# lukashermann/hulc

Hardware: AMD Instinct MI355X
Metric: trajectory-windows/sec (seq_len=32, bs=64/GPU) (higher is better)
Workload: dtype bf16; 1 GPU; HULC training step, vision goal only (use_clip_auxiliary_loss=false), B=64 windows/GPU, seq_len=32, 200x200 static + 84x84 gripper fp32 NCHW frames, fwd+loss+bwd+Adam, dropout 0.1; global_batch=64, seq_len=32, parallelism=dp1

## Files before the change

### hulc_amd/csrc/capi.hip

```cpp
#include <cstdarg>
#include <cstdio>
#include <cstring>
#include <cstdlib>
#include <cmath>
#include <algorithm>
#include <stdexcept>

#include "engine.h"
#include "sbert.h"
#include "store_gather.h"
#include "store_stage.h"

using namespace hulc_bf16;

static thread_local char g_err[1024] = "";
void hulc_set_error(const char* fmt, ...) {
    va_list ap;
    va_start(ap, fmt);
    vsnprintf(g_err, sizeof(g_err), fmt, ap);
    va_end(ap);
}

struct hulc_ctx {
    IEngine* e = nullptr;
// ... 241 lines not shown
    int r = -1, w = -1;
    if (ctx->e->comm->size(&r, &w)) return 1;
    if (rank) *rank = r;
    if (world) *world = w;
    return 0;
}
int hulc_comm_timeline(hulc_ctx* ctx, double* out, int32_t cap_buckets, double* backward_us) {
    if (!ctx || !ctx->e->comm || !out) { hulc_set_error("hulc_comm_timeline: no communicator / null buffer"); return -1; }
    return ctx->e->comm->timeline(out, cap_buckets, backward_us, ctx->e->st);
}
int hulc_allreduce_grads(hulc_ctx* ctx, int32_t bucket_dtype) {
    if (!ctx) { hulc_set_error("hulc_allreduce_grads: null context"); return 1; }
    return ctx->e->allreduce_grads(bucket_dtype);
}
int hulc_backward_allreduce(hulc_ctx* ctx, int32_t bucket_dtype) {
    if (!ctx) { hulc_set_error("hulc_backward_allreduce: null context"); return 1; }
    return ctx->e->backward_allreduce(bucket_dtype);
}
int hulc_scaler_enable(hulc_ctx* ctx, float init_scale, float growth_factor, float backoff_factor, int32_t growth_interval) {
    if (!ctx) { hulc_set_error("hulc_scaler_enable: null context"); return 1; }
    return ctx->e->scaler_enable(init_scale, growth_factor, backoff_factor, growth_interval);
}
int hulc_scaler_get(hulc_ctx* ctx, float* scale, int32_t* growth_tracker, int64_t* skipped_steps, int32_t* last_found_inf, int64_t* taken_steps) {
    if (!ctx) { hulc_set_error("hulc_scaler_get: null context"); return 1; }
    return ctx->e->scaler_get(scale, growth_tracker, skipped_steps, last_found_inf, taken_steps);
}
int hulc_scaler_set(hulc_ctx* ctx, float scale, int32_t growth_tracker, int64_t taken_steps) {
    if (!ctx) { hulc_set_error("hulc_scaler_set: null context"); return 1; }
    return ctx->e->scaler_set(scale, growth_tracker, taken_steps);
}
int hulc_grad_clip_set(hulc_ctx* ctx, int32_t algo, float limit, int32_t track) {
    if (!ctx) { hulc_set_error("hulc_grad_clip_set: null context"); return 1; }
    return ctx->e->grad_clip_set(algo, limit, track);
}
int hulc_grad_norm_get(hulc_ctx* ctx, float* total, float* coef, float* per_tensor_host, int64_t cap) {
    if (!ctx) { hulc_set_error("hulc_grad_norm_get: null context"); return 1; }
    return ctx->e->grad_norm_get(total, coef, per_tensor_host, cap);
}
int hulc_set_kl_beta(hulc_ctx* ctx, float b) { ctx->e->set_kl_beta(b); return 0; }
int hulc_set_dropout(hulc_ctx* ctx, float p) {
    if (!(p >= 0.f && p < 1.f)) { hulc_set_error("hulc_set_dropout: p must be in [0,1)"); return 1; }
    ctx->e->set_dropout(p);
    return 0;
}
int hulc_set_option(hulc_ctx* ctx, const char* name, int64_t value) {
    if (!ctx) { hulc_set_error("hulc_set_option: null context"); return 1; }
    return ctx->e->set_option(name, (long long)value);
}
int hulc_get_option(hulc_ctx* ctx, const char* name, int64_t* value) {
    if (!ctx || !value) { hulc_set_error("hulc_get_option: null argument"); return 1; }
    if (name && !strcmp(name, "stage_tickets")) { *value = HULC_STAGE_TICKETS; return 0; }
    long long v = 0;
    const int rc = ctx->e->get_option(name, &v);
    *value = (int64_t)v;
    return rc;
}
int hulc_timers_enable(hulc_ctx* ctx, int32_t on, const char* only_class) { ctx->e->set_timing(on != 0, only_class); return 0; }
int hulc_timers_read(hulc_ctx* ctx, char* json_out, int64_t cap, int32_t reset) { return ctx->e->timers_read(json_out, cap, reset != 0); }
int hulc_get_tensor(hulc_ctx* ctx, const char* name, float* out, int64_t cap, int64_t* n) { return ctx->e->get_tensor(name, out, cap, n); }
int hulc_get_plan_idx(hulc_ctx* ctx, int32_t* out, int64_t cap) { return ctx->e->get_plan_idx(out, cap); }

int hulc_k_gemm_nt(int32_t dtype, const void* A, const void* B, float* C, int32_t M, int32_t N, int32_t K, int64_t lda, int64_t ldb, int64_t ldc,
                   const float* bias, int32_t relu, void* stream) {
    if (dtype == HULC_DTYPE_F16) return hulc_f16::k_gemm_nt(0, A, B, C, M, N, K, lda, ldb, ldc, bias, relu, stream);
    return hulc_bf16::k_gemm_nt(dtype == HULC_DTYPE_F32, A, B, C, M, N, K, lda, ldb, ldc, bias, relu, stream);
}
#define HULC_K_16BIT(name, call)                                                                                          \
    if (dtype == HULC_DTYPE_F16) return hulc_f16::call;                                                                    \
    if (dtype == HULC_DTYPE_BF16) return hulc_bf16::call;                                                                  \
    hulc_set_error(name ": dtype %d is not a 16-bit type", (int)dtype);                                                    \
    return 1
int hulc_k_spatial_softmax64(int32_t dtype, const void* f, int32_t H, int32_t W, int32_t Nf, void* out, float* stats, const float* dout, void* df, void* stream) {
    HULC_K_16BIT("hulc_k_spatial_softmax64", k_spatial_softmax64(f, H, W, Nf, out, stats, dout, df, stream));
}
int hulc_k_enc_tail_fwd(int32_t dtype, int32_t Nf, int32_t ldemb, const hulc_enc_tail_job* a, const hulc_enc_tail_job* b, void* emb, const float* pos, int32_t S,
                        float drop_p, uint64_t seed, float* xf, void* xt, float* z0, float* z1, void* stream) {
    HULC_K_16BIT("hulc_k_enc_tail_fwd", k_enc_tail_fwd(Nf, ldemb, a, b, emb, pos, S, drop_p, (unsigned long long)seed, xf, xt, z0, z1, stream));
}
int hulc_k_enc_tail_bwd(int32_t dtype, int32_t Nf, int32_t ldemb, const hulc_enc_tail_bwd_job* a, const hulc_enc_tail_bwd_job* b, const float* demb, void* stream) {
    HULC_K_16BIT("hulc_k_enc_tail_bwd", k_enc_tail_bwd(Nf, ldemb, a, b, demb, stream));
}
int hulc_k_tr_layer_fwd(int32_t dtype, const hulc_tr_layer_job* job, int32_t B, int32_t S, int32_t ln_in, float dp, void* stream) {
    HULC_K_16BIT("hulc_k_tr_layer_fwd", k_tr_layer_fwd(job, B, S, ln_in, dp, stream));
}
int hulc_k_tr_ffn_bwd(int32_t dtype, const hulc_tr_ffn_bwd_job* job, int32_t B, int32_t S, int32_t bcast, float bdiv, float dp, void* stream) {
    HULC_K_16BIT("hulc_k_tr_ffn_bwd", k_tr_ffn_bwd(job, B, S, bcast, bdiv, dp, stream));
}
int hulc_k_tr_attn_bwd(int32_t dtype, const hulc_tr_attn_bwd_job* job, int32_t B, int32_t S, int32_t nparts, int64_t part_stride, float dp, void* stream) {
    HULC_K_16BIT("hulc_k_tr_attn_bwd", k_tr_attn_bwd(job, B, S, nparts, (long long)part_stride, dp, stream));
}
int hulc_k_gemm_multi(int32_t dtype, int32_t form, const hulc_gemm_epi_job* jobs, int32_t n, int32_t sh, int32_t* ran, void* stream) {
    HULC_K_16BIT("hulc_k_gemm_multi", k_gemm_multi(form, jobs, n, sh, ran, stream));
}
#undef HULC_K_16BIT
int hulc_k_gemm_epi(int32_t dtype, const hulc_gemm_epi_job* job, int32_t kernel, int32_t* ran, void* stream) {
    if (dtype == HULC_DTYPE_F16) return hulc_f16::k_gemm_epi(1, job, kernel, ran, stream);
    if (dtype != HULC_DTYPE_F32 && dtype != HULC_DTYPE_BF16) { hulc_set_error("hulc_k_gemm_epi: unknown dtype %d", (int)dtype); return 1; }
    return hulc_bf16::k_gemm_epi(dtype == HULC_DTYPE_BF16 ? 1 : 0, job, kernel, ran, stream);
}
int hulc_k_gemm_pick(int32_t dtype, int32_t M, int32_t N, int32_t K, int64_t lda, int64_t ldb, int32_t* pick, int32_t* bk) {
    if (dtype != HULC_DTYPE_F32 && dtype != HULC_DTYPE_BF16 && dtype != HULC_DTYPE_F16) { hulc_set_error("hulc_k_gemm_pick: unknown dtype %d", (int)dtype); return 1; }
    return hulc_bf16::k_gemm_pick(dtype != HULC_DTYPE_F32, M, N, K, (long long)lda, (long long)ldb, pick, bk);
}
int hulc_k_gemm_wgrad_nsplit(int32_t dtype, int32_t M, int32_t N, int32_t K, int32_t* nsplit, int32_t* big) {
    if (dtype != HULC_DTYPE_F32 && dtype != HULC_DTYPE_BF16 && dtype != HULC_DTYPE_F16) { hulc_set_error("hulc_k_gemm_wgrad_nsplit: unknown dtype %d", (int)dtype); return 1; }
    return hulc_bf16::k_gemm_wgrad_nsplit(dtype != HULC_DTYPE_F32, M, N, K, nsplit, big);
}
int hulc_k_logistic_loss(int32_t dtype, int32_t wide, const float* heads, int32_t ldh, const float* actions, const float* robot_obs, int32_t B, int32_t S,
                         int32_t n_mix, int32_t n_dim, int32_t num_classes, float log_scale_min, float gripper_alpha, int32_t gripper_control,
                         int32_t discrete_gripper, float grad_scale, const float* lscale, float* row_loss, float* a_tcp_out, void* dheads, void* stream) {
    if (dtype == HULC_DTYPE_F16)
        return hulc_f16::k_logistic_loss(1, wide, heads, ldh, actions, robot_obs, B, S, n_mix, n_dim, num_classes, log_scale_min, gripper_alpha, gripper_control,
                                         discrete_gripper, grad_scale, lscale, row_loss, a_tcp_out, dheads, stream);
    if (dtype != HULC_DTYPE_F32 && dtype != HULC_DTYPE_BF16) { hulc_set_error("hulc_k_logistic_loss: unknown dtype %d", (int)dtype); return 1; }
    return hulc_bf16::k_logistic_loss(dtype == HULC_DTYPE_BF16, wide, heads, ldh, actions, robot_obs, B, S, n_mix, n_dim, num_classes, log_scale_min, gripper_alpha,
                                      gripper_control, discrete_gripper, grad_scale, lscale, row_loss, a_tcp_out, dheads, stream);
}
#define HULC_K_ANY(name, fn, ...)                                                                                                     \
    if (dtype == HULC_DTYPE_F16) return hulc_f16::fn(1, __VA_ARGS__);                                                                  \
    if (dtype != HULC_DTYPE_F32 && dtype != HULC_DTYPE_BF16) { hulc_set_error(name ": unknown dtype %d", (int)dtype); return 1; }      \
    return hulc_bf16::fn(dtype == HULC_DTYPE_BF16 ? 1 : 0, __VA_ARGS__)
int hulc_k_plan_kl_sample(const float* pr_logits, const float* pp_logits, int32_t B, int32_t NCAT, int32_t NCLS, const int32_t* idx_in, int32_t* idx_out, float* probs,
                          float* kl_cat, float* dpp, float* dpr, float w_pp, float w_pr, uint64_t seed, const float* lscale, void* stream) {
    return hulc_bf16::k_plan_kl_sample(pr_logits, pp_logits, B, NCAT, NCLS, idx_in, idx_out, probs, kl_cat, dpp, dpr, w_pp, w_pr, (unsigned long long)seed, lscale, stream);
}
int hulc_k_st_softmax_bwd(int32_t dtype, const float* probs, const float* dplan, const float* dpr_kl, const float* dpp_kl, int32_t rows, int32_t NCLS, float* out, void* out_t,
                          void* dpp_t, void* stream) {
    HULC_K_ANY("hulc_k_st_softmax_bwd", k_st_softmax_bwd, probs, dplan, dpr_kl, dpp_kl, rows, NCLS, out, out_t, dpp_t, stream);
}
int hulc_k_plan_gather(int32_t dtype, const void* w_t, const int32_t* idx, int32_t B, int32_t NCAT, int32_t NCLS, int32_t H, const float* b1, const float* b2, float* out,
                       const void* emb, void* embg, int32_t S, int32_t W, const void* goal, int32_t G, int32_t grow0, void* cb, void* stream) {
    HULC_K_ANY("hulc_k_plan_gather", k_plan_gather, w_t, idx, B, NCAT, NCLS, H, b1, b2, out, emb, embg, S, W, goal, G, grow0, cb, stream);
}
int hulc_k_plan_scatter_grad(int32_t dtype, int32_t form, const void* dC, const int32_t* idx, int32_t B, int32_t NCAT, int32_t NCLS, int32_t H, int32_t KIN, float* dw,
                             int32_t store, void* stream) {
    HULC_K_ANY("hulc_k_plan_scatter_grad", k_plan_scatter_grad, form, dC, idx, B, NCAT, NCLS, H, KIN, dw, store, stream);
}
int hulc_k_normal_kl_sample(int32_t dtype, const float* pr_state, const float* pp_state, int32_t B, int32_t n, const float* eps_in, float* eps_out, float* plan_f, void* plan_t,
                            float* kl_elem, float* dpp, float* dpr, float w_pp, float w_pr, uint64_t seed, const float* lscale, void* stream) {
    HULC_K_ANY("hulc_k_normal_kl_sample", k_normal_kl_sample, pr_state, pp_state, B, n, eps_in, eps_out, plan_f, plan_t, kl_elem, dpp, dpr, w_pp, w_pr, (unsigned long long)seed, lscale, stream);
}
int hulc_k_normal_rsample_bwd(int32_t dtype, const float* dplan, const float* eps, const float* pr_state, const float* dpr_kl, int32_t B, int32_t n, void* out, void* stream) {
    HULC_K_ANY("hulc_k_normal_rsample_bwd", k_normal_rsample_bwd, dplan, eps, pr_state, dpr_kl, B, n, out, stream);
}
int hulc_k_det_head_loss(int32_t dtype, const void* H1, const void* W, const float* bias, const float* actions, const float* robot_obs, int32_t B, int32_t S,
                         int32_t criterion, int32_t frame, float grad_scale, const float* lscale, float* row_loss, float* pred, float* dpre, void* stream) {
    HULC_K_ANY("hulc_k_det_head_loss", k_det_head_loss, H1, W, bias, actions, robot_obs, B, S, criterion, frame, grad_scale, lscale, row_loss, pred, dpre, stream);
}
int hulc_k_det_head_bwd(int32_t dtype, const float* dpre, const void* W, const void* H1, int32_t B, int32_t S, void* dH1, void* dZ1, float* dW, float* db, void* stream) {
    HULC_K_ANY("hulc_k_det_head_bwd", k_det_head_bwd, dpre, W, H1, B, S, dH1, dZ1, dW, db, stream);
}
int hulc_k_det_head_act(int32_t dtype, const void* h1, const void* W, const float* bias, const float* robot_obs, int32_t n, float* out, void* stream) {
    HULC_K_ANY("hulc_k_det_head_act", k_det_head_act, h1, W, bias, robot_obs, n, out, stream);
}
int hulc_k_layernorm_fwd(int32_t dtype, const float* x, int64_t ldx, int32_t rows, int32_t n, const float* g, const float* b, void* out, int64_t ldo, float* out_f32, int64_t ldf,
                         float* stats, void* stream) {
    HULC_K_ANY("hulc_k_layernorm_fwd", k_layernorm_fwd, x, (long long)ldx, rows, n, g, b, out, (long long)ldo, out_f32, (long long)ldf, stats, stream);
}
int hulc_k_layernorm_bwd(int32_t dtype, const float* dy, int64_t lddy, const float* x, int64_t ldx, const float* stats, const float* g, int32_t rows, int32_t n, float* dx_f32,
                         int64_t ldd, int32_t accumulate, void* dx_t, int64_t ldt, float* dg, float* db, float drop_p, uint64_t seed, int32_t bcast_rows, float bcast_div,
                         int32_t dy_parts, int64_t dy_part_stride, float* scratch, void* stream) {
    HULC_K_ANY("hulc_k_layernorm_bwd", k_layernorm_bwd, dy, (long long)lddy, x, (long long)ldx, stats, g, rows, n, dx_f32, (long long)ldd, accumulate, dx_t, (long long)ldt, dg, db,
               drop_p, (unsigned long long)seed, bcast_rows, bcast_div, dy_parts, (long long)dy_part_stride, scratch, stream);
}
int hulc_k_layernorm_mean(int32_t dtype, const float* x, int32_t B, int32_t S, int32_t n, const float* g, const float* b, float* stats, void* out, float* yout, void* stream) {
    HULC_K_ANY("hulc_k_layernorm_mean", k_layernorm_mean, x, B, S, n, g, b, stats, out, yout, stream);
}
#undef HULC_K_ANY
int hulc_k_cast(int32_t dtype, const float* src, void* dst, int64_t n, void* stream) {
    hipStream_t st = (hipStream_t)stream;
    if (dtype == HULC_DTYPE_F32) hipLaunchKernelGGL((cast_kernel<float, float>), dim3(1024), dim3(256), 0, st, src, (float*)dst, (long long)n);
    else hipLaunchKernelGGL((cast_kernel<float, h16_t>), dim3(1024), dim3(256), 0, st, src, (h16_t*)dst, (long long)n);
    if (hipGetLastError() != hipSuccess) { hulc_set_error("hulc_k_cast: launch failed"); return 1; }
    return 0;
}
int hulc_k_window_compact(const int64_t* window_start, const int32_t* lens, const int32_t* off, int32_t off_base, int32_t B, int32_t S, int64_t store_frames,
                          const int32_t* shift_static, const int32_t* shift_gripper, int64_t* frame_out, int32_t* shift_static_out, int32_t* shift_gripper_out, void* stream) {
    if (!window_start || !lens || !off || !frame_out || B < 1 || S < 1 || store_frames < 1 || (shift_static && !shift_static_out) || (shift_gripper && !shift_gripper_out)) {
        hulc_set_error("hulc_k_window_compact: null argument or B=%d, S=%d, store_frames=%lld out of range", (int)B, (int)S, (long long)store_frames); return 1; }
    launch_window_compact((hipStream_t)stream, reinterpret_cast<const long long*>(window_start), lens, off, off_base, B, S, (long long)store_frames, shift_static, shift_gripper,
                          reinterpret_cast<long long*>(frame_out), shift_static_out, shift_gripper_out);
    if (hipGetLastError() != hipSuccess) { hulc_set_error("hulc_k_window_compact: launch failed"); return 1; }
    return 0;
}
int hulc_k_rows_expand(int32_t elem_bytes, const void* src, const int32_t* lens, const int32_t* off, int32_t B, int32_t S, int32_t n, void* dst, void* stream) {
    if (!src || !lens || !off || !dst || B < 1 || S < 1 || n < 1 || (elem_bytes != 2 && elem_bytes != 4) || (n * elem_bytes) % 16 || ((uintptr_t)src | (uintptr_t)dst) % 16) {
        hulc_set_error("hulc_k_rows_expand: null or misaligned argument, or B=%d, S=%d, n=%d, elem_bytes=%d unsupported", (int)B, (int)S, (int)n, (int)elem_bytes); return 1; }
    if (elem_bytes == 4) launch_rows_expand<float>((hipStream_t)stream, (const float*)src, lens, off, B, S, n, (float*)dst);
    else launch_rows_expand<h16_t>((hipStream_t)stream, (const h16_t*)src, lens, off, B, S, n, (h16_t*)dst);
    if (hipGetLastError() != hipSuccess) { hulc_set_error("hulc_k_rows_expand: launch failed"); return 1; }
    return 0;
}
int hulc_k_rows_reduce(const float* src, const int32_t* lens, const int32_t* off, int32_t B, int32_t S, int32_t n, float* dst, void* stream) {
    if (!src || !lens || !off || !dst || B < 1 || S < 1 || n < 4 || n % 4 || ((uintptr_t)src | (uintptr_t)dst) % 16) {
        hulc_set_error("hulc_k_rows_reduce: null or misaligned argument, or B=%d, S=%d, n=%d unsupported", (int)B, (int)S, (int)n); return 1; }
    launch_rows_reduce((hipStream_t)stream, src, lens, off, B, S, n, dst);
    if (hipGetLastError() != hipSuccess) { hulc_set_error("hulc_k_rows_reduce: launch failed"); return 1; }
    return 0;
}

static int k_clip_loss(bool wide, const float* img, const float* txt, int32_t n, const float* logit_scale, float w, float* loss_out, float* dimg, float* dtxt,
                       float* dlogit_scale, void* stream) {
    hipStream_t st = (hipStream_t)stream;
    if (n < 1 || !img || !txt || !logit_scale || !loss_out || !dimg || !dtxt || !dlogit_scale) { hulc_set_error("hulc_k_clip_loss: n=%d or a null argument", (int)n); return 1; }
    float* ws = nullptr;
    if (n > AUX_ROWS_SINGLE && hipMalloc((void**)&ws, sizeof(float) * (size_t)clip_rows_ws_floats(n)) != hipSuccess) { hulc_set_error("hulc_k_clip_loss: hipMalloc failed"); return 1; }
    const bool ok = launch_clip_loss(st, wide, img, txt, n, logit_scale, w, loss_out, dimg, dtxt, dlogit_scale, nullptr, ws);
    const hipError_t e1 = hipGetLastError(), e2 = hipStreamSynchronize(st);
    if (ws) hipFree(ws);
    if (!ok || e1 != hipSuccess || e2 != hipSuccess) { hulc_set_error("hulc_k_clip_loss: %s", !ok ? "not launched" : hipGetErrorString(e1 != hipSuccess ? e1 : e2)); return 1; }
    return 0;
}
int hulc_k_clip_loss(const float* img, const float* txt, int32_t n, const float* logit_scale, float w, float* loss_out, float* dimg, float* dtxt, float* dlogit_scale,
                     void* stream) { return k_clip_loss(true, img, txt, n, logit_scale, w, loss_out, dimg, dtxt, dlogit_scale, stream); }
int hulc_k_clip_loss_fp32(const float* img, const float* txt, int32_t n, const float* logit_scale, float w, float* loss_out, float* dimg, float* dtxt,
                          float* dlogit_scale, void* stream) { return k_clip_loss(false, img, txt, n, logit_scale, w, loss_out, dimg, dtxt, dlogit_scale, stream); }
int hulc_k_mia_head(const float* img, const float* txt, int32_t n, const float* W0, const float* b0, const float* W1, const float* b1, float w, float* loss_out,
                    float* dimg, float* dtxt, int32_t accum, float* dW0, float* db0, float* dW1, float* db1, void* stream) {
    hipStream_t st = (hipStream_t)stream;
    if (n < 1 || !img || !txt || !W0 || !b0 || !W1 || !b1 || !loss_out) { hulc_set_error("hulc_k_mia_head: n=%d or a null argument", (int)n); return 1; }
    if (dW0 && (!dimg || !dtxt || !db0 || !dW1 || !db1)) { hulc_set_error("hulc_k_mia_head: the backward needs every gradient pointer"); return 1; }
    float* ws = nullptr;
    if (n > AUX_ROWS_SINGLE && hipMalloc((void**)&ws, sizeof(float) * (size_t)mia_rows_ws_floats(n)) != hipSuccess) { hulc_set_error("hulc_k_mia_head: hipMalloc failed"); return 1; }
    const bool ok = launch_mia_head(st, img, txt, n, W0, b0, W1, b1, w, loss_out, dimg, dtxt, accum, dW0, db0, dW1, db1, nullptr, ws);
    const hipError_t e1 = hipGetLastError(), e2 = hipStreamSynchronize(st);
    if (ws) hipFree(ws);
    if (!ok || e1 != hipSuccess || e2 != hipSuccess) { hulc_set_error("hulc_k_mia_head: %s", !ok ? "not launched" : hipGetErrorString(e1 != hipSuccess ? e1 : e2)); return 1; }
    return 0;
}
int hulc_k_cosine_dist(const float* pred, const float* tgt, int32_t n, int32_t D, float w, float* loss_out, float* dpred, void* stream) {
    hipStream_t st = (hipStream_t)stream;
    if (n < 1 || D < 1 || !pred || !tgt || !loss_out) { hulc_set_error("hulc_k_cosine_dist: n=%d D=%d or a null argument", (int)n, (int)D); return 1; }
    hipLaunchKernelGGL(cosine_dist_loss_kernel, dim3(1), dim3(1024), 0, st, pred, tgt, n, D, w, loss_out, dpred, (const float*)nullptr);
    const hipError_t e1 = hipGetLastError(), e2 = hipStreamSynchronize(st);
    if (e1 != hipSuccess || e2 != hipSuccess) { hulc_set_error("hulc_k_cosine_dist: %s", hipGetErrorString(e1 != hipSuccess ? e1 : e2)); return 1; }
    return 0;
}

int hulc_k_attention(int32_t variant, const float* qkv, float* P, float* ao, const float* dao, float* dqkv, int32_t B, int32_t S, float drop_p,
                     uint64_t seed, void* stream) {
    hipStream_t st = (hipStream_t)stream;
    const int D = 128, NH = 8;
    if (S < 1 || S > 64 || (variant == 1 && S > 32)) { hulc_set_error("hulc_k_attention: S=%d not covered by variant %d", S, variant); return 1; }
    if (variant == 2) {
        if (!dao) hipLaunchKernelGGL((attention_fwd64_kernel<float>), dim3(B * NH), dim3(256), 0, st, qkv, B, S, D, NH, P, ao, drop_p, (unsigned long long)seed);
        else {
            hipFuncSetAttribute((const void*)attention_bwd64_kernel<float>, hipFuncAttributeMaxDynamicSharedMemorySize, (int)ATT_BWD64_LDS);
            hipLaunchKernelGGL((attention_bwd64_kernel<float>), dim3(B * NH), dim3(256), ATT_BWD64_LDS, st, qkv, P, dao, B, S, D, NH, dqkv, drop_p, (unsigned long long)seed);
        }
        if (hipGetLastError() != hipSuccess) { hulc_set_error("hulc_k_attention: launch failed"); return 1; }
        return 0;
    }
    const dim3 grid(B * NH), block(64);
    if (!dao) {
        if (variant == 1) hipLaunchKernelGGL((attention_fwd32_kernel<float>), grid, block, 0, st, qkv, B, S, D, NH, P, ao, drop_p, (unsigned long long)seed);
        else if (S <= 32) hipLaunchKernelGGL((attention_fwd_kernel<float, 32>), grid, block, 0, st, qkv, B, S, D, NH, P, ao, drop_p, (unsigned long long)seed);
        else hipLaunchKernelGGL((attention_fwd_kernel<float, 64>), grid, block, 0, st, qkv, B, S, D, NH, P, ao, drop_p, (unsigned long long)seed);
    } else {
        if (variant == 1) hipLaunchKernelGGL((attention_bwd32_kernel<float>), grid, block, 0, st, qkv, P, dao, B, S, D, NH, dqkv, drop_p, (unsigned long long)seed);
        else if (S <= 32) hipLaunchKernelGGL((attention_bwd_kernel<float, 32>), grid, block, 0, st, qkv, P, dao, B, S, D, NH, dqkv, drop_p, (unsigned long long)seed);
        else hipLaunchKernelGGL((attention_bwd_kernel<float, 64>), grid, block, 0, st, qkv, P, dao, B, S, D, NH, dqkv, drop_p, (unsigned long long)seed);
    }
    if (hipGetLastError() != hipSuccess) { hulc_set_error("hulc_k_attention: launch failed"); return 1; }
    return 0;
}

#define HULC_K_CONV_T(name, call)                                                                                          \
    if (dtype == HULC_DTYPE_F16) return hulc_f16::call;                                                                    \
    if (dtype == HULC_DTYPE_BF16) return hulc_bf16::call;                                                                  \
    hulc_set_error(name ": dtype %d is not a 16-bit type (HULC_DTYPE_BF16 or HULC_DTYPE_F16)", (int)dtype);                \
    return 1
int hulc_k_conv_wgrad(int32_t which, const void* X, const void* dY, float* out, int32_t Nf, int32_t IH, void* stream) {
    return hulc_bf16::k_conv_wgrad("hulc_k_conv_wgrad", 0, which, X, dY, out, nullptr, Nf, IH, nullptr, stream);
}
int hulc_k_conv_wgrad_t(int32_t dtype, int32_t which, const void* X, const void* dY, float* out, float* db_out, int32_t Nf, int32_t IH, int32_t* slabs, void* stream) {
    HULC_K_CONV_T("hulc_k_conv_wgrad_t", k_conv_wgrad("hulc_k_conv_wgrad_t", 1, which, X, dY, out, db_out, Nf, IH, slabs, stream));
}

int hulc_k_conv1_interior_groups(int32_t IW, int32_t pad, int32_t cap, int32_t* first, int32_t* count) {
    int cl = 0, wi = 0;
    conv1_interior_groups(IW, pad, cap, cl, wi);
    *first = cl; *count = wi;
    return 0;
}

int hulc_k_conv1_wgrad_u8(const void* X, const int32_t* shifts, int32_t pad, const void* dY, float* dw_out, float* db_out, int32_t Nf, int32_t IH, int32_t form, int32_t fold, void* stream) {
    return hulc_bf16::k_conv1_wgrad_u8("hulc_k_conv1_wgrad_u8", 0, X, shifts, pad, dY, dw_out, db_out, Nf, IH, form, fold, nullptr, stream);
}
int hulc_k_conv1_wgrad_u8_t(int32_t dtype, const void* X, const int32_t* shifts, int32_t pad, const void* dY, float* dw_out, float* db_out, int32_t Nf, int32_t IH, int32_t form,
                            int32_t fold, int32_t* slabs, void* stream) {
    HULC_K_CONV_T("hulc_k_conv1_wgrad_u8_t", k_conv1_wgrad_u8("hulc_k_conv1_wgrad_u8_t", 1, X, shifts, pad, dY, dw_out, db_out, Nf, IH, form, fold, slabs, stream));
}

int hulc_k_conv_tile(int32_t mode, const void* img, const void* w, const float* bias, const void* mask, void* out, int32_t Nf, int32_t IMH,
                     int32_t OUTH, int32_t relu, void* stream) {
    return hulc_bf16::k_conv_tile("hulc_k_conv_tile", 0, mode, img, w, bias, mask, out, nullptr, Nf, IMH, OUTH, relu, 0, stream);
}
int hulc_k_conv_tile_t(int32_t dtype, int32_t mode, const void* img, const void* w, const float* bias, const void* mask, void* out, uint32_t* bits1_out, int32_t Nf, int32_t IMH,
                       int32_t OUTH, int32_t relu, int32_t wgs, void* stream) {
    HULC_K_CONV_T("hulc_k_conv_tile_t", k_conv_tile("hulc_k_conv_tile_t", 1, mode, img, w, bias, mask, out, bits1_out, Nf, IMH, OUTH, relu, wgs, stream));
}
int hulc_k_conv_plan(int32_t form, int32_t frames, int32_t in_side, int32_t out_side, int32_t wgs, int32_t* nbands, int32_t* rows_per_band, int32_t* frames_per_band, int32_t* items) {
    return hulc_bf16::k_conv_plan(form, frames, in_side, out_side, wgs, nbands, rows_per_band, frames_per_band, items);
}

int hulc_k_camera_split(int32_t grid, double work_static, double work_gripper, int32_t* wg_static, int32_t* wg_gripper) {
    int a = 0, b = 0;
    camera_split(grid, work_static, work_gripper, a, b);
    *wg_static = a; *wg_gripper = b;
    return 0;
}

int hulc_k_conv_pair(int32_t stage, const hulc_conv_job* a, const hulc_conv_job* b, int32_t wg_a, int32_t wg_b, void* stream) {
    return hulc_bf16::k_conv_pair("hulc_k_conv_pair", 0, stage, a, b, wg_a, wg_b, nullptr, stream);
}
int hulc_k_conv_pair_t(int32_t dtype, int32_t stage, const hulc_conv_job* a, const hulc_conv_job* b, int32_t wg_a, int32_t wg_b, int32_t* slabs, void* stream) {
    HULC_K_CONV_T("hulc_k_conv_pair_t", k_conv_pair("hulc_k_conv_pair_t", 1, stage, a, b, wg_a, wg_b, slabs, stream));
}
#undef HULC_K_CONV_T

int hulc_k_skinny(const void* A, const void* W, void* out, int32_t M, int32_t N, int32_t K, int32_t variant, void* stream) {
    hipStream_t st = (hipStream_t)stream;
    EpiP ep; ep.out = out; ep.out_f32 = 0;
    const int NW = variant / 10, MT = variant % 10;
    dim3 grid(N / 16, MT > 0 ? (M + MT * 16 - 1) / (MT * 16) : 1);
    const h16_t* a = (const h16_t*)A; const h16_t* w = (const h16_t*)W;
#define SK(nw, mt) hipLaunchKernelGGL((skinny_gemm_kernel<nw, mt>), grid, dim3(nw * 64), 0, st, a, (long long)K, w, (long long)K, M, N, K, dense_out(N), ep)
    if (NW == 8 && MT == 2) SK(8, 2); else if (NW == 8 && MT == 4) SK(8, 4); else if (NW == 4 && MT == 2) SK(4, 2); else if (NW == 4 && MT == 4) SK(4, 4);
    else if (NW == 8 && MT == 1) SK(8, 1); else if (NW == 4 && MT == 1) SK(4, 1);
    else if (NW == 16 && MT == 2) SK(16, 2); else if (NW == 16 && MT == 4) SK(16, 4);
    else if (NW == 9 && MT == 2) hipLaunchKernelGGL((skinny_gemm_kernel<8, 2, 8>), grid, dim3(512), 0, st, a, (long long)K, w, (long long)K, M, N, K, dense_out(N), ep);
    else if (NW == 17 && MT == 2) hipLaunchKernelGGL((skinny_gemm_kernel<16, 2, 4>), grid, dim3(1024), 0, st, a, (long long)K, w, (long long)K, M, N, K, dense_out(N), ep);
    else if (NW == 20) { if (!launch_skinny_lds(st, a, (long long)K, w, (long long)K, M, N, K, MT, dense_out(N), ep)) { hulc_set_error("hulc_k_skinny: shape not covered by the LDS kernel"); return 1; } }
    else if (NW == 30) launch_skinny(st, a, (long long)K, w, (long long)K, M, N, K, dense_out(N), ep);
    else if (NW == 40) {
        EpiP ep2 = ep; ep2.out = (h16_t*)out + (long long)M * N;
        if (!launch_skinny_lds_dual(st, a, w, ep, a + (long long)M * K, w + (long long)N * K, ep2, (long long)K, (long long)K, M, N, K, dense_out(N))) {
            hulc_set_error("hulc_k_skinny: shape not covered by the dual launch"); return 1; }
    }
    else if (NW == 50 || NW == 51) {
        if ((N % 16) != 0 || (K % 128) != 0) { hulc_set_error("hulc_k_skinny: fragment order needs N %% 16 == 0 and K %% 128 == 0"); return 1; }
        h16_t* wf = (h16_t*)out;
        if (NW == 50 && hipMalloc((void**)&wf, (size_t)N * K * sizeof(h16_t)) != hipSuccess) { hulc_set_error("hulc_k_skinny: scratch allocation failed"); return 1; }
        FragPackBatch fb{};
        fb.src[0] = w; fb.dst[0] = wf; fb.N[0] = N; fb.K[0] = K; fb.blk0[0] = 0; fb.blk0[1] = frag_pack_blocks(N, K); fb.n = 1;
        hipLaunchKernelGGL(frag_pack_kernel, dim3(fb.blk0[1]), dim3(256), 0, st, fb);
        if (NW == 50) {
            const bool ok = launch_skinny_lds_kchunk(st, a, (long long)K, wf, 0ll, M, N, K, dense_out(N), ep);
            hipStreamSynchronize(st);
            hipFree(wf);
            if (!ok) { hulc_set_error("hulc_k_skinny: shape not covered by the K-chunked kernel"); return 1; }
        }
    }
    else { hulc_set_error("hulc_k_skinny: unsupported variant"); return 1; }
#undef SK
    return hipGetLastError() == hipSuccess ? 0 : 1;
}

int hulc_k_rnn_persist(void* X, const void* W, const void* res, const void* mask, int32_t B, int32_t S, int32_t q0, int32_t dq, int32_t act, uint32_t* flags,
                       uint32_t* err, uint32_t launch_index, void* stream) {
    RnnPersistP p{};
    p.X = (h16_t*)X; p.W = (const h16_t*)W; p.res = (const h16_t*)res; p.mask = (const h16_t*)mask; p.B = B; p.S = S; p.q0 = q0; p.dq = dq; p.act = act;
    p.flags = flags; p.base = launch_index << 12; p.parity = (int)(launch_index & 1u); p.err = err; p.stamps = nullptr;
    if (!launch_rnn_persist((hipStream_t)stream, p)) { hulc_set_error("hulc_k_rnn_persist: shape not covered (S >= 2, B <= 128)"); return 1; }
    return hipGetLastError() == hipSuccess ? 0 : 1;
}
int32_t hulc_k_rnn_persist_flag_words(void) { return RP_FLAG_WORDS; }

__global__ void trread_probe_kernel(const int* __restrict__ addr_in, unsigned short* __restrict__ out) {
    typedef short s16x4 __attribute__((ext_vector_type(4)));
    __shared__ __attribute__((aligned(16))) unsigned short lds[8192];
    for (int i = threadIdx.x; i < 8192; i += 64) lds[i] = (unsigned short)i;
    __syncthreads();
    const int a = addr_in[threadIdx.x];
    s16x4 v = __builtin_amdgcn_ds_read_tr16_b64_v4i16((__attribute__((address_space(3))) s16x4*)(lds + a));
#pragma unroll
    for (int j = 0; j < 4; ++j) out[threadIdx.x * 4 + j] = (unsigned short)v[j];
}
int hulc_k_trread_probe(const int32_t* addr, uint16_t* out, void* stream) {
    hipLaunchKernelGGL(trread_probe_kernel, dim3(1), dim3(64), 0, (hipStream_t)stream, (const int*)addr, (unsigned short*)out);
    if (hipGetLastError() != hipSuccess) { hulc_set_error("trread probe launch failed"); return 1; }
    return 0;
}

}
```

### hulc_amd/csrc/conv_wgrad.h

```cpp
#pragma once
#include "common.h"

namespace HULC_NS {

typedef short s16x4_t __attribute__((ext_vector_type(4)));
typedef unsigned int u32x4_t __attribute__((ext_vector_type(4)));
typedef __attribute__((address_space(3))) u32x4_t lds_u32x4;

typedef __attribute__((address_space(3))) char lds_char;
DEVI h16x8_t tr_read8(lds_char* p0, lds_char* p1) {
    const s16x4_t lo = __builtin_amdgcn_ds_read_tr16_b64_v4i16((__attribute__((address_space(3))) s16x4_t*)p0);
    const s16x4_t hi = __builtin_amdgcn_ds_read_tr16_b64_v4i16((__attribute__((address_space(3))) s16x4_t*)p1);
    typedef short s16x8_t __attribute__((ext_vector_type(8)));
    const s16x8_t v = __builtin_shufflevector(lo, hi, 0, 1, 2, 3, 4, 5, 6, 7);
    return __builtin_bit_cast(h16x8_t, v);
}

template <int CI, int CO, int KH, int KW, int S>
struct WgradCfg {
    static constexpr int XS = (S == 1) ? ((CI * 2 / 32) | 1) * 32 : CI * 2 + 16;
    static constexpr int DYS = ((CO * 2 / 32) | 1) * 32;
    static constexpr int CGN = CI / 16;
    static constexpr int NT = KH * KW * CGN;
    static constexpr int NTW = NT / 4;
    static constexpr int CT = CO / 16;
    static_assert(NT % 4 == 0, "n-tiles must split over 4 waves");
    static size_t lds_bytes(int R, int IW, int OW) {
        const int OWp = (OW + 7) / 8 * 8;
        const int XR = (R - 1) * S + KH;
        return (size_t)(XR * IW + 8 * S + KW) * XS + (size_t)(R * OWp + 8) * DYS;
    }
};

template <int CI, int CO, int KH, int KW, int S>
__global__ void __launch_bounds__(256, 2) conv_wgrad_tr_kernel(const h16_t* __restrict__ X, const h16_t* __restrict__ dY, float* __restrict__ part,
                                                            float* __restrict__ bias_part, int Nf, int IH, int IW, int OH, int OW, int R) {
    using C = WgradCfg<CI, CO, KH, KW, S>;
    extern __shared__ __attribute__((aligned(16))) char smem[];
    const int tid = threadIdx.x, lane = tid & 63, wave = tid >> 6;
    const int OWp = (OW + 7) & ~7, U = OWp >> 3;
    const int XR = (R - 1) * S + KH;
    const int xpix = XR * IW + 8 * S + KW;
    const int dypix = R * OWp + 8;
    lds_char* ximg = (lds_char*)smem;
    lds_char* dyimg = ximg + xpix * C::XS;
    for (int i = tid * 16; i < xpix * C::XS + dypix * C::DYS; i += 256 * 16) *(lds_u32x4*)((lds_char*)smem + i) = u32x4_t{0u, 0u, 0u, 0u};
    __syncthreads();

    f32x4 acc[C::NTW][C::CT];
#pragma unroll
    for (int j = 0; j < C::NTW; ++j)
#pragma unroll
        for (int c = 0; c < C::CT; ++c) acc[j][c] = f32x4{0.f, 0.f, 0.f, 0.f};

    const int g = lane >> 4, a = lane & 15;
    const int prow = a >> 2;
    const int ccol = (a & 3) * 8;
    const int nt0 = wave * C::NTW;
    float bsum[8] = {0.f, 0.f, 0.f, 0.f, 0.f, 0.f, 0.f, 0.f};

    for (int f = blockIdx.x; f < Nf; f += gridDim.x) {
        for (int oh0 = 0; oh0 < OH; oh0 += R) {
            __syncthreads();
            {
                constexpr int CH = CO / 8;
                for (int r = wave; r < R; r += 4) {
                    const bool in = oh0 + r < OH;
                    const h16_t* src = dY + ((long long)f * OH + min(oh0 + r, OH - 1)) * OW * CO;
                    for (int i = lane; i < OW * CH; i += 64) {
                        u32x4_t v = *reinterpret_cast<const u32x4_t*>(src + i * 8);
                        if (!in) v = u32x4_t{0u, 0u, 0u, 0u};
#pragma unroll
                        for (int e = 0; e < 4; ++e) { bsum[2 * e] += h2f_lo(v[e]); bsum[2 * e + 1] += h2f_hi(v[e]); }
                        *(lds_u32x4*)(dyimg + (r * OWp + i / CH) * C::DYS + (i % CH) * 16) = v;
                    }
                }
            }
            {
                constexpr int CH = CI / 8;
                const int ih0 = oh0 * S;
                const int rows = min(XR, IH - ih0);
                const int total = rows * IW * CH;
                const h16_t* src = X + ((long long)f * IH + ih0) * IW * CI;
                for (int i0 = tid; i0 < total; i0 += 256 * 8) {
                    u32x4_t v[8];
#pragma unroll
                    for (int u = 0; u < 8; ++u) {
                        const int i = min(i0 + u * 256, total - 1);
                        v[u] = *reinterpret_cast<const u32x4_t*>(src + (long long)(i / CH) * CI + (i % CH) * 8);
                    }
#pragma unroll
                    for (int u = 0; u < 8; ++u) {
                        const int i = i0 + u * 256;
                        if (i < total) *(lds_u32x4*)(ximg + (i / CH) * C::XS + (i % CH) * 16) = v[u];
                    }
                }
            }
            __syncthreads();
            const int units = R * U;
            for (int u0 = 0; u0 < units; u0 += 4) {
                const int u = u0 + g;
                const bool valid = u < units;
                const int r = valid ? u / U : 0, ow0 = valid ? (u % U) * 8 : 0;
                const int pixA = valid ? r * OWp + ow0 : R * OWp;
                lds_char* abase = dyimg + (pixA + prow) * C::DYS + ccol;
                h16x8_t af[C::CT];
#pragma unroll
                for (int c = 0; c < C::CT; ++c) af[c] = tr_read8(abase + c * 32, abase + 4 * C::DYS + c * 32);
                const int pixB0 = (r * S) * IW + ow0 * S;
#pragma unroll
                for (int j = 0; j < C::NTW; ++j) {
                    const int nt = nt0 + j;
                    const int tap = nt / C::CGN, cg = nt % C::CGN;
                    const int kh = tap / KW, kw = tap % KW;
                    lds_char* bbase = ximg + (pixB0 + kh * IW + kw + prow * S) * C::XS + cg * 32 + ccol;
                    const h16x8_t bf = tr_read8(bbase, bbase + 4 * S * C::XS);
#pragma unroll
                    for (int c = 0; c < C::CT; ++c) acc[j][c] = MFMA_16x16x32_H(af[c], bf, acc[j][c], 0, 0, 0);
                }
            }
        }
    }
    constexpr int KC = KH * KW * CI;
    float* out = part + (long long)blockIdx.x * CO * KC;
#pragma unroll
    for (int j = 0; j < C::NTW; ++j)
#pragma unroll
        for (int c = 0; c < C::CT; ++c)
#pragma unroll
            for (int r = 0; r < 4; ++r) out[(long long)(c * 16 + g * 4 + r) * KC + (nt0 + j) * 16 + a] = acc[j][c][r];
    __syncthreads();
    float* red = reinterpret_cast<float*>(smem);
#pragma unroll
    for (int e = 0; e < 8; ++e) red[tid * 8 + e] = bsum[e];
    __syncthreads();
    if (tid < CO) {
        constexpr int CH = CO / 8;
        const int cgrp = tid >> 3, e = tid & 7;
        float s = 0.f;
        for (int t = cgrp; t < 256; t += CH) s += red[t * 8 + e];
        if (bias_part) unsafeAtomicAdd(bias_part + tid, s);
    }
}

static inline void camera_split(int grid, double wA, double wB, int& nA, int& nB) {
    if (grid < 1) grid = 1;
    if (!(wB > 0.0)) { nA = grid; nB = 0; return; }
    if (!(wA > 0.0)) { nA = 0; nB = grid; return; }
    if (grid < 2) { nA = nB = 1; return; }
    int b = (int)(grid * (wB / (wA + wB)) + 0.5);
    b = std::min(std::max(b, 1), grid - 1);
    nA = grid - b; nB = b;
}

struct WgradJob {
    const h16_t* X; const h16_t* dY; float* part; float* bias_part; const h16_t* zeros;
    int Nf, IH, IW, OH, OW, R, nbands; int* work_ctr; int FPB;
};
template <int CI, int CO, int KH, int KW, int S, int NWV, int D = 3, int IWC = 0>
DEVI void conv_wgrad_tr8_body(const WgradJob& J, const int bid, const int nwg) {
    const h16_t* __restrict__ const X = J.X; const h16_t* __restrict__ const dY = J.dY; float* __restrict__ const part = J.part; float* __restrict__ const bias_part = J.bias_part;
    const int Nf = J.Nf, IH = J.IH, IW = J.IW, OH = J.OH, OW = J.OW, R = J.R, nbands = J.nbands, FPB = J.FPB;
    int* __restrict__ const work_ctr = J.work_ctr;
    using C = WgradCfg<CI, CO, KH, KW, S>;
    constexpr int NTH = NWV * 64, PF = 8192 / NTH, CTH = C::CT / (NWV / 4), CHY = CO / 8, CHX = CI / 8;
    extern __shared__ __attribute__((aligned(16))) char smem[];
    const int tid = threadIdx.x, lane = tid & 63, wave = tid >> 6;
    const int OWp = (OW + 7) & ~7, U = OWp >> 3;
    const int XR = (R - 1) * S + KH;
    const int xpix = XR * IW + 8 * S + KW;
    const int dypix = R * OWp + 8;
    lds_char* ximg = (lds_char*)smem;
    lds_char* dyimg = ximg + xpix * C::XS;
    for (int i = tid * 16; i < xpix * C::XS + dypix * C::DYS; i += NTH * 16) *(lds_u32x4*)((lds_char*)smem + i) = u32x4_t{0u, 0u, 0u, 0u};

    const bool stacked = FPB > 1;
    const int VP = IH / S;
    const int ndy = (stacked ? FPB * OH : R) * OW * CHY, nx = XR * IW * CHX, nch = ndy + nx;
    unsigned pk[PF];
#pragma unroll
    for (int k = 0; k < PF; ++k) {
        const int ci = min(tid + k * NTH, nch - 1);
        if (ci < ndy) {
            const int pix = ci / CHY, c = ci % CHY;
            int r = pix / OW;
            const int ow = pix % OW;
            if (stacked) r = (r / OH) * VP + r % OH;
            pk[k] = ((unsigned)((xpix * C::XS + (r * OWp + ow) * C::DYS + c * 16) >> 4) << 17) | (unsigned)ci;
        } else {
            const int cx = ci - ndy;
            const int pix = cx / CHX, c = cx % CHX;
            pk[k] = 0x80000000u | ((unsigned)((pix * C::XS + c * 16) >> 4) << 17) | (unsigned)cx;
        }
    }
    const int q = wave & 3, h = wave >> 2;
    f32x4 acc[C::NTW][CTH];
#pragma unroll
    for (int j = 0; j < C::NTW; ++j)
#pragma unroll
        for (int c = 0; c < CTH; ++c) acc[j][c] = f32x4{0.f, 0.f, 0.f, 0.f};
    const int g = lane >> 4, a = lane & 15;
    const int prow = a >> 2;
    const int ccol = (a & 3) * 8;
    constexpr int NTG = 4 / C::CGN, TPG = KH * KW / NTG;
    static_assert(C::CGN <= 4 && 4 % C::CGN == 0 && (KH * KW) % NTG == 0 && TPG == C::NTW && (NTG == 1 || TPG % KW == 0), "n-tile assignment");
    const int IWk = IWC ? IWC : IW;
    const int cgq = q % C::CGN, tg = q / C::CGN;
    const int qoff = ((tg * TPG / KW) * IWk) * C::XS + cgq * 32;
    int toff[C::NTW];
#pragma unroll
    for (int j = 0; j < C::NTW; ++j) toff[j] = ((j / KW) * IWk + j % KW) * C::XS;
    float bsum[8] = {0.f, 0.f, 0.f, 0.f, 0.f, 0.f, 0.f, 0.f};

    u32x4_t pf[PF];
    const int nitems = stacked ? (Nf + FPB - 1) / FPB : Nf * nbands;
    unsigned zmask = 0, zmask_cur = 0;
    auto prefetch = [&](int item) {
        zmask = 0;
        const int f = stacked ? item * FPB : item / nbands, oh0 = stacked ? 0 : (item % nbands) * R;
        const int nfr = stacked ? min(FPB, Nf - f) : 1;
        const h16_t* ybase = dY + ((long long)f * OH + oh0) * OW * CO;
        const h16_t* xbase = X + ((long long)f * IH + oh0 * S) * IW * CI;
        const int yrows = stacked ? nfr * OH : min(R, OH - oh0), xrows = stacked ? min(XR, nfr * IH) : min(XR, IH - oh0 * S);
        const int ylim = yrows * OW * CHY - 1, xlim = xrows * IW * CHX - 1;
#pragma unroll
        for (int k = 0; k < PF; ++k) {
            const bool isx = (pk[k] >> 31) != 0;
            const int go = (int)(pk[k] & 0x1ffffu);
            const h16_t* src = isx ? xbase + (long long)min(go, xlim) * 8 : ybase + (long long)min(go, ylim) * 8;
            pf[k] = *reinterpret_cast<const u32x4_t*>(src);
            if (!isx && go > ylim) zmask |= 1u << k;
        }
    };
    __shared__ int s_next[2];
    int item = bid, iter = 0;
    if (item < nitems) prefetch(item);
    while (item < nitems) {
        if (work_ctr && tid == 0) s_next[iter & 1] = nwg + atomicAdd(work_ctr, 1);
        __syncthreads();
        zmask_cur = zmask;
#pragma unroll
        for (int k = 0; k < PF; ++k) {
            if (tid + k * NTH < nch) {
                const u32x4_t v = ((zmask_cur >> k) & 1u) ? u32x4_t{0u, 0u, 0u, 0u} : pf[k];
                if (!(pk[k] >> 31)) {
#pragma unroll
                    for (int e = 0; e < 4; ++e) { bsum[2 * e] += h2f_lo(v[e]); bsum[2 * e + 1] += h2f_hi(v[e]); }
                }
                *(lds_u32x4*)((lds_char*)smem + (((pk[k] >> 17) & 0x3fffu) << 4)) = v;
            }
        }
        __syncthreads();
        item = work_ctr ? s_next[iter & 1] : item + nwg;
        ++iter;
        if (item < nitems) prefetch(item);
        const int units = R * U;
        const int px = (g & 1) * 4 + prow;
        const int q4 = 4 / U, r4 = 4 - q4 * U;
        const int step4 = (q4 * S * IW + r4 * 8 * S) * C::XS, wrapd = (S * IW - U * 8 * S) * C::XS;
        int uo[2], pbv[2];
#pragma unroll
        for (int hh = 0; hh < 2; ++hh) {
            const int u = hh * 2 + (g >> 1), r = u / U;
            uo[hh] = u - r * U;
            pbv[hh] = ((r * S) * IW + (uo[hh] * 8 + px) * S) * C::XS + ccol;
        }
        const int abase = px * C::DYS + ccol + h * CTH * 32, pb_idle = (px * S) * C::XS + ccol;
#pragma unroll 1
        for (int u0 = 0; u0 < units; u0 += 4) {
            lds_char* ab[2];
            int pb[2];
#pragma unroll
            for (int hh = 0; hh < 2; ++hh) {
                const int u = u0 + hh * 2 + (g >> 1);
                const bool valid = u < units;
                ab[hh] = dyimg + (valid ? u * 8 : R * OWp) * C::DYS + abase;
                pb[hh] = valid ? pbv[hh] : pb_idle;
                pbv[hh] += step4; uo[hh] += r4;
                if (uo[hh] >= U) { uo[hh] -= U; pbv[hh] += wrapd; }
            }
            auto bfrag = [&](int j) { return tr_read8(ximg + qoff + pb[0] + toff[j], ximg + qoff + pb[1] + toff[j]); };
            h16x8_t ring[D];
            h16x8_t af[CTH];
#pragma unroll
            for (int c = 0; c < CTH; ++c) af[c] = tr_read8(ab[0] + c * 32, ab[1] + c * 32);
#pragma unroll
            for (int j = 0; j < D && j < C::NTW; ++j) ring[j] = bfrag(j);
            __builtin_amdgcn_sched_barrier(0);
#pragma unroll
            for (int j = 0; j < C::NTW; ++j) {
                const h16x8_t bf = ring[j % D];
#pragma unroll
                for (int c = 0; c < CTH; ++c) acc[j][c] = MFMA_16x16x32_H(af[c], bf, acc[j][c], 0, 0, 0);
                if (j + D < C::NTW) ring[j % D] = bfrag(j + D);
                __builtin_amdgcn_sched_barrier(0);
            }
        }
    }
    constexpr int KC = KH * KW * CI;
    float* out = part + (long long)bid * CO * KC;
#pragma unroll
    for (int j = 0; j < C::NTW; ++j)
#pragma unroll
        for (int c = 0; c < CTH; ++c)
#pragma unroll
            for (int r = 0; r < 4; ++r) out[(long long)((h * CTH + c) * 16 + g * 4 + r) * KC + ((tg * TPG + j) * C::CGN + cgq) * 16 + a] = acc[j][c][r];
    __syncthreads();
    float* red = reinterpret_cast<float*>(smem);
#pragma unroll
    for (int e = 0; e < 8; ++e) red[tid * 8 + e] = bsum[e];
    __syncthreads();
    if (tid < CO) {
        const int cgrp = tid >> 3, e = tid & 7;
        float s = 0.f;
        for (int t = cgrp; t < NTH; t += CHY) s += red[t * 8 + e];
        if (bias_part) unsafeAtomicAdd(bias_part + tid, s);
    }
}
template <int CI, int CO, int KH, int KW, int S, int NWV, int D = 3, int IWC = 0>
__global__ void __launch_bounds__(NWV * 64) conv_wgrad_tr8_kernel(const h16_t* __restrict__ X, const h16_t* __restrict__ dY, float* __restrict__ part,
                                                            float* __restrict__ bias_part, int Nf, int IH, int IW, int OH, int OW, int R, int nbands,
                                                            int* __restrict__ work_ctr, int FPB) {
    const WgradJob J{X, dY, part, bias_part, nullptr, Nf, IH, IW, OH, OW, R, nbands, work_ctr, FPB};
    conv_wgrad_tr8_body<CI, CO, KH, KW, S, NWV, D, IWC>(J, (int)blockIdx.x, (int)gridDim.x);
}

DEVI int wg_fdiv(int x, float inv) { return (int)(((float)x + 0.5f) * inv); }
DEVI void wg_lds_dma16(const void* src, lds_char* dst) {
    const unsigned a = (unsigned)__builtin_amdgcn_readfirstlane((int)(unsigned)(size_t)dst);
    asm volatile("s_mov_b32 m0, %1\n\ts_nop 0\n\tglobal_load_lds_dwordx4 %0, off" : : "v"(src), "s"(a) : "memory", "m0");
}
template <int CI, int CO, int KH, int KW, int S, int IWC = 0>
DEVI void conv_wgrad_dma_body(const WgradJob& J, const int bid, const int nwg) {
    const h16_t* __restrict__ const X = J.X; const h16_t* __restrict__ const dY = J.dY; float* __restrict__ const part = J.part; float* __restrict__ const bias_part = J.bias_part;
    const h16_t* __restrict__ const zeros = J.zeros;
    const int Nf = J.Nf, IH = J.IH, IW = J.IW, OH = J.OH, OW = J.OW, R = J.R, nbands = J.nbands;
    int* __restrict__ const work_ctr = J.work_ctr;
    using C = WgradCfg<CI, CO, KH, KW, S>;
    constexpr int NWV = 8, NTH = NWV * 64, CTH = C::CT / (NWV / 4), CHY = CO / 8, CHX = CI / 8, XSS = C::XS / 16, YSS = C::DYS / 16;
    extern __shared__ __attribute__((aligned(16))) char smem[];
    const int tid = threadIdx.x, lane = tid & 63, wave = tid >> 6;
    const int OWp = (OW + 7) & ~7, U = OWp >> 3;
    const int XR = (R - 1) * S + KH;
    const int xpix = XR * IW + 8 * S + KW;
    const int dypix = R * OWp + 8;
    const int xslots = xpix * XSS, yslots = dypix * YSS;
    const int bbytes = ((xslots + yslots) * 16 + 1023) & ~1023;
    const int npieces = bbytes >> 10;
    lds_char* const lbase = (lds_char*)smem;
    const int nitems = Nf * nbands;
    const float invXSS = 1.f / (float)XSS, invYSS = 1.f / (float)YSS, invIW = 1.f / (float)IW, invOWp = 1.f / (float)OWp, invOW = 1.f / (float)OW;
    constexpr int PFM = 10;
    unsigned pk[PFM];
#pragma unroll
    for (int k = 0; k < PFM; ++k) {
        int q = (k * NWV + wave) * 64 + lane;
        unsigned v = 0;
        if (q < xslots) {
            const int px = wg_fdiv(q, invXSS), ch = q - px * XSS;
            const int r = wg_fdiv(px, invIW), c = px - r * IW;
            if (ch < CHX && r < XR) v = 0xC0000000u | ((unsigned)r << 24) | (unsigned)(((r * IW + c) * CI + ch * 8) >> 3);
        } else {
            q -= xslots;
            const int px = wg_fdiv(q, invYSS), ch = q - px * YSS;
            const int r = wg_fdiv(px, invOWp), c = px - r * OWp;
            if (ch < CHY && r < R && c < OW) v = 0x40000000u | ((unsigned)r << 24) | (unsigned)(((r * OW + c) * CO + ch * 8) >> 3);
        }
        pk[k] = v;
    }
    auto dma = [&](int item, int buf) {
        const int f = item / nbands, oh0 = (item - f * nbands) * R, ih0 = oh0 * S;
        const int yrows = min(R, OH - oh0), xrows = min(XR, IH - ih0);
        const h16_t* xsrc = X + ((long long)f * IH + ih0) * IW * CI;
        const h16_t* ysrc = dY + ((long long)f * OH + oh0) * OW * CO;
        lds_char* dst = lbase + buf * bbytes + wave * 1024;
#pragma unroll
        for (int k = 0; k < PFM; ++k) {
            if (k * NWV + wave >= npieces) break;
            const unsigned v = pk[k];
            const bool isx = (v >> 31) != 0;
            const int r = (int)((v >> 24) & 63u);
            const bool ok = ((v >> 30) & 1u) && r < (isx ? xrows : yrows);
            const h16_t* src = ok ? (isx ? xsrc : ysrc) + (long long)(v & 0xffffffu) * 8 : zeros;
            wg_lds_dma16(src, dst + k * NWV * 1024);
        }
    };
    const int q = wave & 3, h = wave >> 2;
    f32x4 acc[C::NTW][CTH];
#pragma unroll
    for (int j = 0; j < C::NTW; ++j)
#pragma unroll
        for (int c = 0; c < CTH; ++c) acc[j][c] = f32x4{0.f, 0.f, 0.f, 0.f};
    const int g = lane >> 4, a = lane & 15;
    const int prow = a >> 2;
    const int ccol = (a & 3) * 8;
    constexpr int NTG = 4 / C::CGN, TPG = KH * KW / NTG;
    static_assert(C::CGN <= 4 && 4 % C::CGN == 0 && (KH * KW) % NTG == 0 && TPG == C::NTW && (NTG == 1 || TPG % KW == 0), "n-tile assignment");
    const int IWk = IWC ? IWC : IW;
    const int cgq = q % C::CGN, tg = q / C::CGN;
    const int qoff = ((tg * TPG / KW) * IWk) * C::XS + cgq * 32;
    int toff[C::NTW];
#pragma unroll
    for (int j = 0; j < C::NTW; ++j) toff[j] = ((j / KW) * IWk + j % KW) * C::XS;
    float bsum[8] = {0.f, 0.f, 0.f, 0.f, 0.f, 0.f, 0.f, 0.f};
    __shared__ int s_next[2];
    int item = bid, iter = 0, nb = 0;
    if (item < nitems) dma(item, 0);
    asm volatile("s_waitcnt vmcnt(0)" ::: "memory");
    const int px = (g & 1) * 4 + prow;
    const int q4 = 4 / U, r4 = 4 - q4 * U;
    const int step4 = (q4 * S * IW + r4 * 8 * S) * C::XS, wrapd = (S * IW - U * 8 * S) * C::XS;
    while (item < nitems) {
        if (work_ctr && tid == 0) s_next[iter & 1] = nwg + atomicAdd(work_ctr, 1);
        __syncthreads();
        const int cur = item;
        item = work_ctr ? s_next[iter & 1] : item + nwg;
        ++iter;
        lds_char* const ximg0 = lbase + nb * bbytes;
        lds_char* const dyimg = ximg0 + xslots * 16;
        lds_char* const ximg = ximg0 + qoff;
        nb ^= 1;
        bool pend = item < nitems;
        if (pend && wave < 4) { dma(item, nb); pend = false; }
        {
            const int f = cur / nbands, oh0 = (cur - f * nbands) * R;
            const int nchunk = min(R, OH - oh0) * OW * CHY;
            for (int i = tid; i < nchunk; i += NTH) {
                const int pix = i / CHY, r = wg_fdiv(pix, invOW), c = pix - r * OW;
                const u32x4_t v = *(lds_u32x4*)(dyimg + (r * OWp + c) * C::DYS + (tid % CHY) * 16);
#pragma unroll
                for (int e = 0; e < 4; ++e) { bsum[2 * e] += h2f_lo(v[e]); bsum[2 * e + 1] += h2f_hi(v[e]); }
            }
        }
        const int units = R * U;
        int uo[2], pbv[2];
#pragma unroll
        for (int hh = 0; hh < 2; ++hh) {
            const int u = hh * 2 + (g >> 1), r = u / U;
            uo[hh] = u - r * U;
            pbv[hh] = ((r * S) * IW + (uo[hh] * 8 + px) * S) * C::XS + ccol;
        }
        const int abase = px * C::DYS + ccol + h * CTH * 32, pb_idle = (px * S) * C::XS + ccol;
        auto mstep = [&](const int u0) {
            lds_char* ab[2];
            int pb[2];
#pragma unroll
            for (int hh = 0; hh < 2; ++hh) {
                const int u = u0 + hh * 2 + (g >> 1);
                const bool valid = u < units;
                ab[hh] = dyimg + (valid ? u * 8 : R * OWp) * C::DYS + abase;
                pb[hh] = valid ? pbv[hh] : pb_idle;
                pbv[hh] += step4; uo[hh] += r4;
                if (uo[hh] >= U) { uo[hh] -= U; pbv[hh] += wrapd; }
            }
            auto bfrag = [&](int j) { return tr_read8(ximg + pb[0] + toff[j], ximg + pb[1] + toff[j]); };
            constexpr int D = 3;
            h16x8_t ring[D];
            h16x8_t af[CTH];
#pragma unroll
            for (int c = 0; c < CTH; ++c) af[c] = tr_read8(ab[0] + c * 32, ab[1] + c * 32);
#pragma unroll
            for (int j = 0; j < D && j < C::NTW; ++j) ring[j] = bfrag(j);
            __builtin_amdgcn_sched_barrier(0);
#pragma unroll
            for (int j = 0; j < C::NTW; ++j) {
                const h16x8_t bf = ring[j % D];
#pragma unroll
                for (int c = 0; c < CTH; ++c) acc[j][c] = MFMA_16x16x32_H(af[c], bf, acc[j][c], 0, 0, 0);
                if (j + D < C::NTW) ring[j % D] = bfrag(j + D);
                __builtin_amdgcn_sched_barrier(0);
            }
        };
        if (units > 0) mstep(0);
        if (pend) { dma(item, nb); pend = false; }
#pragma unroll 1
        for (int u0 = 4; u0 < units; u0 += 4) mstep(u0);
        if (pend) dma(item, nb);
        asm volatile("s_waitcnt vmcnt(0)" ::: "memory");
    }
    constexpr int KC = KH * KW * CI;
    float* out = part + (long long)bid * CO * KC;
#pragma unroll
    for (int j = 0; j < C::NTW; ++j)
#pragma unroll
        for (int c = 0; c < CTH; ++c)
#pragma unroll
            for (int r = 0; r < 4; ++r) out[(long long)((h * CTH + c) * 16 + g * 4 + r) * KC + ((tg * TPG + j) * C::CGN + cgq) * 16 + a] = acc[j][c][r];
    __syncthreads();
    float* red = reinterpret_cast<float*>(smem);
#pragma unroll
    for (int e = 0; e < 8; ++e) red[tid * 8 + e] = bsum[e];
    __syncthreads();
    if (tid < CO) {
        const int cgrp = tid >> 3, e = tid & 7;
        float s = 0.f;
        for (int t = cgrp; t < NTH; t += CHY) s += red[t * 8 + e];
        if (bias_part) unsafeAtomicAdd(bias_part + tid, s);
    }
}
template <int CI, int CO, int KH, int KW, int S, int IWC = 0>
__global__ void __launch_bounds__(512) conv_wgrad_dma_kernel(const h16_t* __restrict__ X, const h16_t* __restrict__ dY, float* __restrict__ part,
                                                             float* __restrict__ bias_part, const h16_t* __restrict__ zeros, int Nf, int IH, int IW, int OH, int OW,
                                                             int R, int nbands, int* __restrict__ work_ctr) {
    const WgradJob J{X, dY, part, bias_part, zeros, Nf, IH, IW, OH, OW, R, nbands, work_ctr, 1};
    conv_wgrad_dma_body<CI, CO, KH, KW, S, IWC>(J, (int)blockIdx.x, (int)gridDim.x);
}
template <int CI, int CO, int KH, int KW, int S, int IWS, int IWG>
__global__ void __launch_bounds__(512) conv_wgrad_pair_kernel(WgradJob A, WgradJob B, int wgA) {
    if ((int)blockIdx.x < wgA) conv_wgrad_dma_body<CI, CO, KH, KW, S, IWS>(A, (int)blockIdx.x, wgA);
    else conv_wgrad_tr8_body<CI, CO, KH, KW, S, 8, 3, IWG>(B, (int)blockIdx.x - wgA, (int)gridDim.x - wgA);
}
template <int CI, int CO, int KH, int KW, int S>
static inline int conv_wgrad_dma_rows(int IH, int IW, int OH, int OW, int* nbands_out, size_t* lds_out) {
    using C = WgradCfg<CI, CO, KH, KW, S>;
    const int OWp = (OW + 7) / 8 * 8, U = OWp / 8;
    int bestR = 0, bestc = 1 << 30;
    for (int R = OH; R >= 1; --R) {
        const int XR = (R - 1) * S + KH;
        const size_t band = (((size_t)(XR * IW + 8 * S + KW) * C::XS + (size_t)(R * OWp + 8) * C::DYS) + 1023) / 1024 * 1024;
        const size_t lds = std::max<size_t>(2 * band, 512 * 8 * sizeof(float));
        if (lds > 160 * 1024 - 128 || band > 80 * 1024 || R > 63) continue;
        const int nb = (OH + R - 1) / R, last = OH - (nb - 1) * R;
        const int cost = (nb - 1) * ((R * U + 3) / 4 + 1) + (last * U + 3) / 4 + 1;
        if (cost < bestc) { bestc = cost; bestR = R; *nbands_out = nb; *lds_out = lds; }
    }
    return bestR;
}

template <int CI, int KH> struct WgradCamW {
    static constexpr int fixed = (CI == 64 && KH == 3) ? 1 : ((CI == 32 && KH == 4) ? 2 : 0);
    static constexpr int stat = fixed == 1 ? 23 : (fixed == 2 ? 49 : 0), gripper = fixed == 1 ? 9 : (fixed == 2 ? 20 : 0);
};
template <int CI, int CO, int KH, int KW, int S>
static inline bool conv_wgrad_tr8_plan(int Nf, int IH, int IW, int OH, int OW, int wgs, int& R_out, int& nb_out, int& fpb_out, size_t& lds_out) {
    using C = WgradCfg<CI, CO, KH, KW, S>;
    constexpr int NWV = 8;
    for (int nb = 1; nb <= OH; ++nb) {
        int R = (OH + nb - 1) / nb, XR = (R - 1) * S + KH;
        long long chunks = (long long)R * OW * (CO / 8) + (long long)XR * IW * (CI / 8);
        size_t lds = std::max<size_t>(C::lds_bytes(R, IW, OW), NWV * 64 * 8 * sizeof(float));
        if (chunks > 16 * 512 || lds > 160 * 1024 - 64 || (long long)XR * IW * CI >= (1 << 20)) continue;
        int fpb = 1;
        if (nb == 1 && IH % S == 0) {
            for (int f = 2; f <= 16; ++f) {
                const int Rf = (f - 1) * (IH / S) + OH, XRf = (Rf - 1) * S + KH;
                const long long ch = (long long)f * OH * OW * (CO / 8) + (long long)XRf * IW * (CI / 8);
                const size_t l = std::max<size_t>(C::lds_bytes(Rf, IW, OW), NWV * 64 * 8 * sizeof(float));
                if (ch > 16 * 512 || l > 160 * 1024 - 64 || (long long)XRf * IW * CI >= (1 << 20)) break;
                if ((Nf + f - 1) / f < 2 * wgs) break;
                fpb = f; R = Rf; XR = XRf; chunks = ch; lds = l;
            }
        }
        R_out = R; nb_out = nb; fpb_out = fpb; lds_out = lds;
        return true;
    }
    return false;
}

template <int CI, int CO, int KH, int KW, int S>
static inline int launch_conv_wgrad_tr(hipStream_t st, const h16_t* X, const h16_t* dY, float* part, float* bias_part, int Nf, int IH, int IW, int OH,
                                       int OW, int max_blocks, int* work_ctr = nullptr, const h16_t* zeros = nullptr) {
    using C = WgradCfg<CI, CO, KH, KW, S>;
    if (zeros && OH * OW >= 256 && Nf >= 2) {
        int nb = 0; size_t lds = 0;
        const int R = conv_wgrad_dma_rows<CI, CO, KH, KW, S>(IH, IW, OH, OW, &nb, &lds);
        if (R > 0 && (long long)Nf * IH * IW * CI < (1ll << 31)) {
            constexpr int IWS = WgradCamW<CI, KH>::stat;
            static bool attr3 = false;
            if (!attr3) {
                hipFuncSetAttribute((const void*)conv_wgrad_dma_kernel<CI, CO, KH, KW, S, 0>, hipFuncAttributeMaxDynamicSharedMemorySize, 160 * 1024 - 64);
                hipFuncSetAttribute((const void*)conv_wgrad_dma_kernel<CI, CO, KH, KW, S, IWS>, hipFuncAttributeMaxDynamicSharedMemorySize, 160 * 1024 - 64);
                attr3 = true;
            }
            const int grid = std::min(std::min(Nf * nb, 256), max_blocks);
            if (IWS && IW == IWS) hipLaunchKernelGGL((conv_wgrad_dma_kernel<CI, CO, KH, KW, S, IWS>), dim3(grid), dim3(512), lds, st, X, dY, part, bias_part, zeros, Nf, IH, IW, OH, OW, R, nb, work_ctr);
            else hipLaunchKernelGGL((conv_wgrad_dma_kernel<CI, CO, KH, KW, S, 0>), dim3(grid), dim3(512), lds, st, X, dY, part, bias_part, zeros, Nf, IH, IW, OH, OW, R, nb, work_ctr);
            return grid;
        }
    }
    constexpr int NWV = 8;
    {
        int R = 0, nb = 0, fpb = 1; size_t lds = 0;
        if (conv_wgrad_tr8_plan<CI, CO, KH, KW, S>(Nf, IH, IW, OH, OW, std::min(256, max_blocks), R, nb, fpb, lds)) {
        static bool attr8 = false;
        if (!attr8) {
            hipFuncSetAttribute((const void*)conv_wgrad_tr8_kernel<CI, CO, KH, KW, S, NWV>, hipFuncAttributeMaxDynamicSharedMemorySize, 160 * 1024 - 64);
            attr8 = true;
        }
        const int items = fpb > 1 ? (Nf + fpb - 1) / fpb : Nf * nb;
        const int grid = std::min(std::min(items, 256), max_blocks);
        {
            constexpr int IWG = WgradCamW<CI, KH>::gripper;
            if (IWG && IW == IWG) {
                static bool ag = false;
                if (!ag) { hipFuncSetAttribute((const void*)conv_wgrad_tr8_kernel<CI, CO, KH, KW, S, NWV, 3, IWG>, hipFuncAttributeMaxDynamicSharedMemorySize, 160 * 1024 - 64); ag = true; }
                hipLaunchKernelGGL((conv_wgrad_tr8_kernel<CI, CO, KH, KW, S, NWV, 3, IWG>), dim3(grid), dim3(NWV * 64), lds, st, X, dY, part, bias_part, Nf, IH, IW, OH, OW, R, nb, work_ctr, fpb);
                return grid;
            }
        }
        hipLaunchKernelGGL((conv_wgrad_tr8_kernel<CI, CO, KH, KW, S, NWV>), dim3(grid), dim3(NWV * 64), lds, st, X, dY, part, bias_part, Nf, IH, IW, OH, OW, R, nb, work_ctr, fpb);
        return grid;
        }
    }
    int R = OH;
    while (R > 1 && C::lds_bytes(R, IW, OW) > 78 * 1024) --R;
    const int nbands = (OH + R - 1) / R;
    R = (OH + nbands - 1) / nbands;
    const size_t lds = C::lds_bytes(R, IW, OW);
    static bool attr_set = false;
    if (!attr_set) {
        hipFuncSetAttribute((const void*)conv_wgrad_tr_kernel<CI, CO, KH, KW, S>, hipFuncAttributeMaxDynamicSharedMemorySize, 160 * 1024);
        attr_set = true;
    }
    const int grid = Nf < max_blocks ? Nf : max_blocks;
    hipLaunchKernelGGL((conv_wgrad_tr_kernel<CI, CO, KH, KW, S>), dim3(grid), dim3(256), lds, st, X, dY, part, bias_part, Nf, IH, IW, OH, OW, R);
    return grid;
}

template <int CI, int CO, int KH, int KW, int S>
static inline bool launch_conv_wgrad_pair(hipStream_t st, WgradJob A, WgradJob B, int max_blocks, const int* wg, int ns[2]) {
    using W = WgradCamW<CI, KH>;
    if constexpr (W::fixed == 0) return false;
    else {
        constexpr int IWS = W::stat, IWG = W::gripper;
        if (A.IW != IWS || A.IH != IWS || B.IW != IWG || B.IH != IWG || !A.zeros || A.OH * A.OW < 256 || A.Nf < 1 || B.Nf < 1) return false;
        if ((long long)A.Nf * A.IH * A.IW * CI >= (1ll << 31)) return false;
        int nbA = 0; size_t ldsA = 0;
        A.R = conv_wgrad_dma_rows<CI, CO, KH, KW, S>(A.IH, A.IW, A.OH, A.OW, &nbA, &ldsA);
        if (A.R <= 0) return false;
        A.nbands = nbA; A.FPB = 1;
        const int grid = std::min(256, max_blocks);
        if (grid < 2) return false;
        auto steps = [](int rows, int OW) { return (rows * ((OW + 7) / 8) + 3) / 4 + 1; };
        const int itemsA = A.Nf * nbA;
        const double wA = (double)A.Nf * ((nbA - 1) * steps(A.R, A.OW) + steps(A.OH - (nbA - 1) * A.R, A.OW));
        size_t ldsB = 0; int itemsB = 0;
        auto planB = [&](int wgs) {
            if (!conv_wgrad_tr8_plan<CI, CO, KH, KW, S>(B.Nf, B.IH, B.IW, B.OH, B.OW, wgs, B.R, B.nbands, B.FPB, ldsB)) return false;
            itemsB = B.FPB > 1 ? (B.Nf + B.FPB - 1) / B.FPB : B.Nf * B.nbands;
            return true;
        };
        int nA, nB;
        if (wg) { nA = std::max(wg[0], 1); nB = std::max(wg[1], 1); if (!planB(nB)) return false; }
        else {
            if (!planB(grid)) return false;
            if (itemsA + itemsB <= grid) { nA = itemsA; nB = itemsB; }
            else {
                camera_split(grid, wA, (double)itemsB * steps(B.R, B.OW), nA, nB);
                if (nA > itemsA) { nB = std::min(itemsB, nB + nA - itemsA); nA = itemsA; }
                if (nB > itemsB) { nA = std::min(itemsA, nA + nB - itemsB); nB = itemsB; }
                if (!planB(nB)) return false;
            }
        }
        nA = std::min(nA, itemsA); nB = std::min(nB, itemsB);
        B.part = A.part + (long long)nA * CO * (KH * KW * CI);
        static bool attrp = false;
        if (!attrp) { hipFuncSetAttribute((const void*)conv_wgrad_pair_kernel<CI, CO, KH, KW, S, IWS, IWG>, hipFuncAttributeMaxDynamicSharedMemorySize, 160 * 1024 - 64); attrp = true; }
        hipLaunchKernelGGL((conv_wgrad_pair_kernel<CI, CO, KH, KW, S, IWS, IWG>), dim3(nA + nB), dim3(512), std::max(ldsA, ldsB), st, A, B, nA);
        ns[0] = nA; ns[1] = nB;
        return true;
    }
}

#define CONV1_RAW_MARGIN 16
static inline __host__ __device__ int conv1_raw_pitch16(int IW) { return (((IW + 2 * CONV1_RAW_MARGIN) * 3 + 8 + 7) & ~7) + 15 & ~15; }
static inline __host__ __device__ int conv1_raw_pitch(int IW) { return ((IW + 2 * CONV1_RAW_MARGIN) * 3 + 8 + 7) & ~7; }
struct Conv1Src {
    const void* X;
    const int* shift;
    int u8, pad;
    int fold;
    const long long* wstart = nullptr;
    int S = 1;
    long long nstore = 0;
    DEVI long long frame(int f) const {
        if (!wstart) return f;
        const int b = f / S;
        const long long s0 = min(max(wstart[b], 0ll), nstore - (long long)S);
        return s0 + (f - b * S);
    }
    DEVI long long frames_total(int Nf) const { return wstart ? nstore : (long long)Nf; }
    DEVI void offsets(int f, int& dx, int& dy) const {
        dx = dy = 0;
        if (shift) { dx = min(max(shift[2 * f] - pad, -pad), pad); dy = shift[2 * f + 1] - pad; }
    }
};
#define CONV1_FOLD_SCALE (2.f / 255.f)
__global__ void __launch_bounds__(64) conv1_bias_fold_kernel(const h16_t* __restrict__ W, const float* __restrict__ b, float* __restrict__ out) {
    const int o = blockIdx.x, lane = threadIdx.x;
    float s = 0.f;
    for (int k = lane; k < 192; k += 64) s += h2f(W[o * 192 + k]);
#pragma unroll
    for (int m = 32; m > 0; m >>= 1) s += __shfl_xor(s, m);
    if (lane == 0) out[o] = b[o] - s;
}
DEVI float u8_to_unit(unsigned char b) { return ((float)b / 255.f - 0.5f) / 0.5f; }
struct RowCol { int r, c; };
struct Step256 {
    int n, dq, dr;
    DEVI explicit Step256(int n_) : n(n_), dq(256 / n_), dr(256 % n_) {}
    DEVI void adv(RowCol& p) const { p.c += dr; p.r += dq; if (p.c >= n) { p.c -= n; ++p.r; } }
};
DEVI int conv1_window_off(int c, int dx, int IW, int RB) {
    const int qp = min(max(c * 4 + dx, 0), IW - 4);
    return min((qp * 3) & ~3, RB - 16);
}
template <bool FOLD>
DEVI void conv1_window_group(const u32x4_t& w, int c, int dx, int IW, int RB, unsigned (&lo)[3], unsigned (&hi)[3]) {
    const float sc = 2.f / 255.f, of = -1.f;
    const int p0 = c * 4 + dx, qp = min(max(p0, 0), IW - 4);
    const int a0 = min((qp * 3) & ~3, RB - 16), sh = qp * 3 - a0;
    const bool s4 = sh == 4;
    const unsigned w0 = s4 ? w[1] : w[0], w1 = s4 ? w[2] : w[1], w2 = s4 ? w[3] : w[2], w3 = w[3];
    const unsigned d0 = __builtin_amdgcn_alignbyte(w1, w0, sh & 3), d1 = __builtin_amdgcn_alignbyte(w2, w1, sh & 3), d2 = __builtin_amdgcn_alignbyte(w3, w2, sh & 3);
    const unsigned P[4] = {d0, __builtin_amdgcn_alignbyte(d1, d0, 3), __builtin_amdgcn_alignbyte(d2, d1, 2), d2 >> 8};
    float v[12];
#pragma unroll
    for (int kk = 0; kk < 4; ++kk) {
        const int si = min(max(p0 + kk, 0), IW - 1) - qp;
        const unsigned pw = si == 0 ? P[0] : (si == 1 ? P[1] : (si == 2 ? P[2] : P[3]));
#pragma unroll
        for (int ch = 0; ch < 3; ++ch) { const float x = (float)((pw >> (8 * ch)) & 0xffu); v[kk * 3 + ch] = FOLD ? x : fmaf(x, sc, of); }
    }
#pragma unroll
    for (int ch = 0; ch < 3; ++ch) { lo[ch] = pack2h(v[ch], v[3 + ch]); hi[ch] = pack2h(v[6 + ch], v[9 + ch]); }
}
template <bool FOLD>
DEVI void conv1_window_group_interior(const u32x4_t& w, int sh, unsigned (&lo)[3], unsigned (&hi)[3]) {
    const float sc = 2.f / 255.f, of = -1.f;
    const unsigned d[3] = {__builtin_amdgcn_alignbyte(w[1], w[0], sh), __builtin_amdgcn_alignbyte(w[2], w[1], sh), __builtin_amdgcn_alignbyte(w[3], w[2], sh)};
    float v[12];
#pragma unroll
    for (int i = 0; i < 12; ++i) { const float x = (float)((d[i >> 2] >> (8 * (i & 3))) & 0xffu); v[i] = FOLD ? x : fmaf(x, sc, of); }
#pragma unroll
    for (int ch = 0; ch < 3; ++ch) { lo[ch] = pack2h(v[ch], v[3 + ch]); hi[ch] = pack2h(v[6 + ch], v[9 + ch]); }
}
static inline __host__ __device__ void conv1_interior_groups(int IW, int pad, int cap, int& cl, int& wi) {
    const int lo = (pad + 3) >> 2, hi = (IW - 6 - pad) >= 0 ? (IW - 6 - pad) / 4 + 1 : 0;
    wi = hi - lo < cap ? hi - lo : cap;
    cl = wi > 0 ? lo + (hi - lo - wi) / 2 : 0;
    if (wi < 0) wi = 0;
}
template <bool REGCONV = false>
DEVI void conv1_stage_band(const Conv1Src& s, int f, int ih0, int rows, int IH, int IW, lds_char* ximg, int XR, int XRS, int tid, lds_char* raw) {
    typedef unsigned int u32x2_t __attribute__((ext_vector_type(2)));
    const int W4 = IW >> 2;
    const Step256 sq(W4);
    const RowCol q0{tid / W4, tid % W4};
    if (!s.u8) {
        const float* X = reinterpret_cast<const float*>(s.X);
        const float* src0 = X + ((long long)f * 3 * IH + ih0) * IW;
        const int per = rows * W4, tot = 3 * per;
        const float inv_per = 1.f / (float)per, inv_w4 = 1.f / (float)W4;
        constexpr int NU = 6;
        for (int e0 = tid; e0 < tot; e0 += 256 * NU) {
            float4 v[NU];
            int pk[NU];
#pragma unroll
            for (int u = 0; u < NU; ++u) {
                const int e = min(e0 + u * 256, tot - 1);
                const int c = (int)(((float)e + 0.5f) * inv_per), rem = e - c * per;
                const int r = (int)(((float)rem + 0.5f) * inv_w4), q4 = rem - r * W4;
                pk[u] = (c << 20) | (r << 8) | q4;
                v[u] = *reinterpret_cast<const float4*>(src0 + ((long long)c * IH + r) * IW + q4 * 4);
            }
#pragma unroll
            for (int u = 0; u < NU; ++u) {
                if (e0 + u * 256 < tot) {
                    const int c = pk[u] >> 20, r = (pk[u] >> 8) & 0xfff, q4 = pk[u] & 0xff;
                    u32x2_t o;
                    o[0] = pack2h(v[u].x, v[u].y);
                    o[1] = pack2h(v[u].z, v[u].w);
                    *(__attribute__((address_space(3))) u32x2_t*)(ximg + (c * XR + r) * XRS + q4 * 8) = o;
                }
            }
        }
        return;
    }
    const unsigned char* base = reinterpret_cast<const unsigned char*>(s.X) + s.frame(f) * IH * IW * 3;
    int dx = 0, dy = 0;
    s.offsets(f, dx, dy);
    const int RB = IW * 3;
    if constexpr (REGCONV) {
        constexpr int NU = 6;
        int cl, WI;
        conv1_interior_groups(IW, s.pad, W4, cl, WI);
        if (WI > 0 && dx >= -s.pad && dx <= s.pad) {
            const Step256 si(WI);
            const int shu = (3 * dx) & 3, off0 = 12 * cl + 3 * dx;
            RowCol p{tid / WI, tid % WI};
            while (p.r < rows) {
                RowCol e[NU];
                u32x4_t w[NU];
#pragma unroll
                for (int u = 0; u < NU; ++u) {
                    e[u] = p; si.adv(p);
                    const bool in = e[u].r < rows;
                    w[u] = *reinterpret_cast<const u32x4_t*>(base + (long long)min(max(ih0 + (in ? e[u].r : rows - 1) + dy, 0), IH - 1) * RB + ((off0 + 12 * (in ? e[u].c : 0)) & ~3));
                }
#pragma unroll
                for (int u = 0; u < NU; ++u)
                    if (e[u].r < rows) {
                        unsigned lo[3], hi[3];
                        if (s.fold) conv1_window_group_interior<true>(w[u], shu, lo, hi); else conv1_window_group_interior<false>(w[u], shu, lo, hi);
#pragma unroll
                        for (int ch = 0; ch < 3; ++ch) *(__attribute__((address_space(3))) u32x2_t*)(ximg + (ch * XR + e[u].r) * XRS + (cl + e[u].c) * 8) = u32x2_t{lo[ch], hi[ch]};
                    }
            }
            const int WE = W4 - WI;
            for (int i = tid; i < rows * WE; i += 256) {
                const int r = i / WE, ce = i - r * WE, c = ce < cl ? ce : ce + WI;
                const u32x4_t w = *reinterpret_cast<const u32x4_t*>(base + (long long)min(max(ih0 + r + dy, 0), IH - 1) * RB + conv1_window_off(c, dx, IW, RB));
                unsigned lo[3], hi[3];
                if (s.fold) conv1_window_group<true>(w, c, dx, IW, RB, lo, hi); else conv1_window_group<false>(w, c, dx, IW, RB, lo, hi);
#pragma unroll
                for (int ch = 0; ch < 3; ++ch) *(__attribute__((address_space(3))) u32x2_t*)(ximg + (ch * XR + r) * XRS + c * 8) = u32x2_t{lo[ch], hi[ch]};
            }
            return;
        }
        RowCol p = q0;
        while (p.r < rows) {
            RowCol e[NU];
            u32x4_t w[NU];
#pragma unroll
            for (int u = 0; u < NU; ++u) {
                e[u] = p; sq.adv(p);
                const bool in = e[u].r < rows;
                w[u] = *reinterpret_cast<const u32x4_t*>(base + (long long)min(max(ih0 + (in ? e[u].r : rows - 1) + dy, 0), IH - 1) * RB + conv1_window_off(in ? e[u].c : 0, dx, IW, RB));
            }
#pragma unroll
            for (int u = 0; u < NU; ++u)
                if (e[u].r < rows) {
                    unsigned lo[3], hi[3];
                    if (s.fold) conv1_window_group<true>(w[u], e[u].c, dx, IW, RB, lo, hi); else conv1_window_group<false>(w[u], e[u].c, dx, IW, RB, lo, hi);
#pragma unroll
                    for (int ch = 0; ch < 3; ++ch) *(__attribute__((address_space(3))) u32x2_t*)(ximg + (ch * XR + e[u].r) * XRS + e[u].c * 8) = u32x2_t{lo[ch], hi[ch]};
                }
        }
        return;
    }
    const int RP = conv1_raw_pitch(IW);
    constexpr int LM = CONV1_RAW_MARGIN * 3;
    if ((RB & 7) == 0 && ((uintptr_t)base & 7) == 0) {
        typedef unsigned int u32x2v __attribute__((ext_vector_type(2)));
        constexpr int NU = 10;
        const int n8 = RB >> 3;
        const Step256 s8(n8);
        RowCol p{tid / n8, tid % n8};
        while (p.r < rows) {
            RowCol e[NU];
            u32x2v v[NU];
#pragma unroll
            for (int u = 0; u < NU; ++u) {
                e[u] = p; s8.adv(p);
                const bool in = e[u].r < rows;
                v[u] = *reinterpret_cast<const u32x2v*>(base + (long long)min(max(ih0 + (in ? e[u].r : rows - 1) + dy, 0), IH - 1) * RB + (in ? e[u].c : 0) * 8);
            }
#pragma unroll
            for (int u = 0; u < NU; ++u)
                if (e[u].r < rows) *(__attribute__((address_space(3))) u32x2v*)(raw + e[u].r * RP + LM + e[u].c * 8) = v[u];
        }
    } else {
        constexpr int NU = 8;
        const int n4 = RB >> 2;
        const Step256 s4(n4);
        RowCol p{tid / n4, tid % n4};
        while (p.r < rows) {
            RowCol e[NU];
            unsigned v[NU];
#pragma unroll
            for (int u = 0; u < NU; ++u) {
                e[u] = p; s4.adv(p);
                const bool in = e[u].r < rows;
                v[u] = *reinterpret_cast<const unsigned*>(base + (long long)min(max(ih0 + (in ? e[u].r : rows - 1) + dy, 0), IH - 1) * RB + (in ? e[u].c : 0) * 4);
            }
#pragma unroll
            for (int u = 0; u < NU; ++u)
                if (e[u].r < rows) *(__attribute__((address_space(3))) unsigned*)(raw + e[u].r * RP + LM + e[u].c * 4) = v[u];
        }
    }
    if (dx != 0) {
        for (int i = tid; i < rows * 2; i += 256) {
            const int rr = i >> 1, side = i & 1;
            const unsigned char* rp = base + (long long)min(max(ih0 + rr + dy, 0), IH - 1) * RB;
            const unsigned w = *reinterpret_cast<const unsigned*>(rp + (side ? RB - 4 : 0));
            const unsigned px = side ? (w >> 8) : (w & 0xffffffu);
            lds_char* dst = raw + rr * RP + (side ? LM + RB : 0);
            for (int k = 0; k < CONV1_RAW_MARGIN; ++k) {
                dst[k * 3 + 0] = (char)(px & 0xff); dst[k * 3 + 1] = (char)((px >> 8) & 0xff); dst[k * 3 + 2] = (char)((px >> 16) & 0xff);
            }
        }
    }
    __syncthreads();
    const float sc = s.fold ? 1.f : 2.f / 255.f, of = s.fold ? 0.f : -1.f;
    for (RowCol p = q0; p.r < rows; sq.adv(p)) {
        const int o = p.r * RP + LM + (p.c * 4 + dx) * 3;
        const int sh = o & 3;
        const __attribute__((address_space(3))) unsigned* wp = (const __attribute__((address_space(3))) unsigned*)(raw + (o & ~3));
        const unsigned w0 = wp[0], w1 = wp[1], w2 = wp[2], w3 = wp[3];
        const unsigned d[3] = {__builtin_amdgcn_alignbyte(w1, w0, sh), __builtin_amdgcn_alignbyte(w2, w1, sh), __builtin_amdgcn_alignbyte(w3, w2, sh)};
        float v[12];
#pragma unroll
        for (int k = 0; k < 12; ++k) v[k] = fmaf((float)((d[k >> 2] >> (8 * (k & 3))) & 0xffu), sc, of);
#pragma unroll
        for (int c = 0; c < 3; ++c) {
            u32x2_t ov;
            ov[0] = pack2h(v[c], v[3 + c]);
            ov[1] = pack2h(v[6 + c], v[9 + c]);
            *(__attribute__((address_space(3))) u32x2_t*)(ximg + (c * XR + p.r) * XRS + p.c * 8) = ov;
        }
    }
}
__global__ void ingest_u8_kernel(const unsigned char* __restrict__ in, const int* __restrict__ shift, int pad, int Nf, int IH, int IW, float* __restrict__ out, Conv1Src src = Conv1Src{}) {
    const long long idx = (long long)blockIdx.x * blockDim.x + threadIdx.x;
    if (idx >= (long long)Nf * 3 * IH * IW) return;
    const int x = (int)(idx % IW), y = (int)((idx / IW) % IH), c = (int)((idx / ((long long)IW * IH)) % 3), f = (int)(idx / ((long long)3 * IW * IH));
    int dx = 0, dy = 0;
    if (shift) { dx = min(max(shift[2 * f] - pad, -pad), pad); dy = shift[2 * f + 1] - pad; }
    const int sy = min(max(y + dy, 0), IH - 1), sx = min(max(x + dx, 0), IW - 1);
    out[idx] = u8_to_unit(in[((src.frame(f) * IH + sy) * IW + sx) * 3 + c]);
}

__global__ void __launch_bounds__(256) window_expand_kernel(const long long* __restrict__ wstart, const int* __restrict__ wlen, int B, int S, long long nstore,
                                                            const int* __restrict__ sh_s, const int* __restrict__ sh_g, long long* __restrict__ frame_out,
                                                            int* __restrict__ sh_s_out, int* __restrict__ sh_g_out) {
    const int idx = blockIdx.x * 256 + threadIdx.x;
    if (idx >= B * S) return;
    const int b = idx / S, t = idx - b * S;
    const int L = min(max(wlen[b], 1), (int)min((long long)S, nstore));
    const long long s0 = min(max(wstart[b], 0ll), nstore - (long long)L);
    const int te = min(t, L - 1), fe = b * S + te;
    frame_out[idx] = s0 + te;
    if (sh_s) { sh_s_out[2 * idx] = sh_s[2 * fe]; sh_s_out[2 * idx + 1] = sh_s[2 * fe + 1]; }
    if (sh_g) { sh_g_out[2 * idx] = sh_g[2 * fe]; sh_g_out[2 * idx + 1] = sh_g[2 * fe + 1]; }
}
__global__ void __launch_bounds__(256) window_compact_kernel(const long long* __restrict__ wstart, const int* __restrict__ lens, const int* __restrict__ off, int off_base,
                                                             int B, int S, long long nstore, const int* __restrict__ sh_s, const int* __restrict__ sh_g,
                                                             long long* __restrict__ frame_out, int* __restrict__ sh_s_out, int* __restrict__ sh_g_out) {
    const int idx = blockIdx.x * 256 + threadIdx.x;
    if (idx >= B * S) return;
    const int b = idx / S, t = idx - b * S, L = lens[b];
    if (t >= L) return;
    const long long s0 = min(max(wstart[b], 0ll), nstore - (long long)L);
    const int r = off[b] - off_base + t;
    frame_out[r] = s0 + t;
    if (sh_s) { sh_s_out[2 * r] = sh_s[2 * idx]; sh_s_out[2 * r + 1] = sh_s[2 * idx + 1]; }
    if (sh_g) { sh_g_out[2 * r] = sh_g[2 * idx]; sh_g_out[2 * r + 1] = sh_g[2 * idx + 1]; }
}
template <typename T>
__global__ void __launch_bounds__(256) rows_expand_kernel(const T* __restrict__ src, const int* __restrict__ lens, const int* __restrict__ off, int B, int S, int n,
                                                          T* __restrict__ dst) {
// ... 822 lines not shown
```

### hulc_amd/csrc/k_entries.h

```cpp
#pragma once
#include "iengine.h"
#include "kernels.h"
#include "enc_tail.h"
#include "plan_ln_launch.h"
#include "gemm.h"
#include "tr_fused.h"
#include "det_head.h"
#include <vector>

namespace HULC_NS {

static inline bool k_misaligned16(const void* p) { return (reinterpret_cast<uintptr_t>(p) & 15) != 0; }
static inline int k_launched(const char* who) {
    const hipError_t e = hipGetLastError();
    if (e != hipSuccess) { hulc_set_error("%s: launch failed: %s", who, hipGetErrorString(e)); return 1; }
    return 0;
}

int k_spatial_softmax64(const void* f, int H, int W, int Nf, void* out, float* stats, const float* dout, void* df, void* stream) {
    hipStream_t st = (hipStream_t)stream;
    if (Nf < 1 || H < 2 || W < 2 || (long long)H * W > (1 << 20)) { hulc_set_error("hulc_k_spatial_softmax64: Nf=%d H=%d W=%d (need Nf >= 1, H, W >= 2)", Nf, H, W); return 1; }
    if (!f || !stats || (dout ? !df : !out)) { hulc_set_error("hulc_k_spatial_softmax64: null argument"); return 1; }
    if (k_misaligned16(f) || k_misaligned16(stats) || k_misaligned16(dout) || k_misaligned16(df)) { hulc_set_error("hulc_k_spatial_softmax64: f, stats, dout, df must be 16-byte aligned"); return 1; }
    if (!dout) hipLaunchKernelGGL(spatial_softmax_fwd64_kernel, dim3(Nf), dim3(256), 0, st, (const h16_t*)f, H, W, (h16_t*)out, stats);
// ... 545 lines not shown
    if (!ran) ran = &dummy;
    *ran = HULC_GEMM_RAN_NONE;
    if (!jobs) { hulc_set_error("%s: null jobs", who); return 1; }
    if (form < 0 || form > 2 || n < 2 || n > (form == 0 ? 3 : 2)) { hulc_set_error("%s: form=%d n=%d (form 0: n = 2 or 3; forms 1, 2: n = 2)", who, form, n); return 1; }
    DenseLoader<h16_t> a[3], b[3]; DenseOut om[3]; EpiP ep[3];
    for (int i = 0; i < n; ++i) {
        const hulc_gemm_epi_job& j = jobs[i];
        if (k_gemm_job_bad(who, i, &j, 2)) return 1;
        if (j.nsplit != 1 || j.z_stride != 0 || j.atomic || j.wfrag) { hulc_set_error("%s: job %d: nsplit = 1, z_stride = 0, no atomic, no wfrag", who, i); return 1; }
        a[i] = dense<h16_t>((const h16_t*)j.A, j.M, j.lda); b[i] = dense<h16_t>((const h16_t*)j.B, j.N, j.ldb); om[i] = k_gemm_job_om(j); ep[i] = k_gemm_job_epi(j);
    }
    const hulc_gemm_epi_job &j0 = jobs[0], &j1 = jobs[1];
    if (form == 0) {
        GemmGroupP g{};
        g.n = n;
        for (int i = 0; i < n; ++i) {
            if (!gemm_glds_ok(a[i], b[i], ep[i], jobs[i].M, jobs[i].N, jobs[i].K)) { hulc_set_error("%s: job %d: gemm_glds_ok refuses (K >= 64, K %% 32 == 0, rows 16-byte aligned)", who, i); return 1; }
            g.a[i] = a[i]; g.b[i] = b[i]; g.om[i] = om[i]; g.ep[i] = ep[i]; g.M[i] = jobs[i].M; g.N[i] = jobs[i].N; g.K[i] = jobs[i].K;
        }
        launch_gemm_glds_group(st, g);
        *ran = HULC_GEMM_RAN_GROUP;
        return k_launched(who);
    }
    if (j0.M != j1.M || j0.N != j1.N || j0.K != j1.K || j0.lda != j1.lda || j0.ldb != j1.ldb || j0.ldc != j1.ldc || j0.out_R1 != j1.out_R1 || j0.out_s0 != j1.out_s0) {
        hulc_set_error("%s: forms 1 and 2: the two jobs share M, N, K, the leading dimensions and the output map", who); return 1;
    }
    if (form == 1) {
        if (j0.A != j1.A) { hulc_set_error("%s: form 1: the two jobs share A", who); return 1; }
        if (!gemm_glds_pair_ok(a[0], b[0], b[1], ep[0], ep[1], j0.M, j0.N, j0.K, sh)) {
            hulc_set_error("%s: form 1: gemm_glds_pair_ok refuses (K >= 192, K, sh multiples of 64, 0 < sh < K, M, N multiples of 128, plain fp32 epilogues, 16-byte aligned)", who); return 1;
        }
        launch_gemm_glds_pair(st, a[0], b[0], b[1], om[0], ep[0], ep[1], j0.M, j0.N, j0.K, sh);
        *ran = HULC_GEMM_RAN_PAIR;
        return k_launched(who);
    }
    if (!skinny_use_lds || !skinny_lds_dual_ok(a[0].p, b[0].p, a[1].p, b[1].p, j0.lda, j0.ldb, j0.M, j0.N, j0.K)) {
        hulc_set_error("%s: form 2: shape not covered by the dual launch (32 < M <= 64, K = 2048, N %% 16 == 0, lda %% 64 == 0, A 128-byte aligned, W 16-byte aligned)", who); return 1;
    }
    if (!launch_skinny_lds_dual(st, a[0].p, b[0].p, ep[0], a[1].p, b[1].p, ep[1], j0.lda, j0.ldb, j0.M, j0.N, j0.K, om[0])) { hulc_set_error("%s: form 2: the launcher refused", who); return 1; }
    *ran = HULC_GEMM_RAN_DUAL;
    return k_launched(who);
}
int k_gemm_pick(int t16, int M, int N, int K, long long lda, long long ldb, int* pick, int* bk) {
    if (!pick || !bk || M < 1 || N < 1 || K < 1 || lda < K || ldb < K) { hulc_set_error("hulc_k_gemm_pick: null argument or bad shape"); return 1; }
    EpiP ep;
    GemmPick p;
    const void* al = (const void*)(uintptr_t)0x10000;
    if (t16) p = gemm_pick<h16_t>(dense<h16_t>((const h16_t*)al, M, lda), dense<h16_t>((const h16_t*)al, N, ldb), ep, M, N, K, gemm_use_glds);
    else p = gemm_pick<float>(dense<float>((const float*)al, M, lda), dense<float>((const float*)al, N, ldb), ep, M, N, K, gemm_use_glds);
    *pick = p == GEMM_PICK_SKINNY ? HULC_GEMM_RAN_SKINNY_ROUTER : p == GEMM_PICK_GLDS ? HULC_GEMM_RAN_GLDS : gemm_pick_tile(p) == 128 ? HULC_GEMM_RAN_128 : gemm_pick_tile(p) == 64 ? HULC_GEMM_RAN_64 : HULC_GEMM_RAN_32;
    *bk = (p == GEMM_PICK_SKINNY || p == GEMM_PICK_GLDS) ? 0 : (p == GEMM_PICK_64_BK128 || p == GEMM_PICK_32_BK128) ? 128 : p == GEMM_PICK_128_BK64 ? 64 : 32;
    return 0;
}
int k_gemm_wgrad_nsplit(int t16, int M, int N, int K, int* nsplit, int* big) {
    if (!nsplit || !big || M < 1 || N < 1 || K < 1) { hulc_set_error("hulc_k_gemm_wgrad_nsplit: null argument or bad shape"); return 1; }
    bool b = false;
    *nsplit = t16 ? gemm_wgrad_nsplit<h16_t>(M, N, K, &b) : gemm_wgrad_nsplit<float>(M, N, K, &b);
    *big = b ? 1 : 0;
    return 0;
}

static inline int k_conv_fwd_side(int in_side, int K, int S) { return in_side < K ? -1 : (in_side - K) / S + 1; }
static inline bool k_conv_mode_bench_only(int mode) { return mode == 12 || mode == 13 || mode == 18 || mode == 19; }
int k_conv_wgrad(const char* who, int typed, int which, const void* X, const void* dY, float* out, float* db_out, int Nf, int IH, int* slabs, void* stream) {
    hipStream_t st = (hipStream_t)stream;
    if (slabs) *slabs = 0;
    if (typed) {
        if (which < 1 || which > 3) { hulc_set_error("%s: which must be 1, 2 or 3", who); return 1; }
        const int KH = which == 3 ? 3 : (which == 2 ? 4 : 8);
        if (!X || !dY || !out || Nf < 1 || IH < KH || IH > 4096 || (long long)Nf * IH * IH * 64 >= (1ll << 31)) { hulc_set_error("%s: null argument, or Nf=%d, IH=%d out of range", who, Nf, IH); return 1; }
    }
    float* part = nullptr;
    static float* bias_tmp = nullptr;
    if (!bias_tmp && hipMalloc(&bias_tmp, sizeof(float) * 512 * 64) != hipSuccess) { hulc_set_error("%s: hipMalloc failed", who); return 1; }
    const int KC = which == 3 ? 576 : (which == 2 ? 512 : 192);
    const int CO = which == 1 ? 32 : 64;
    if (hipMalloc(&part, sizeof(float) * 512ll * 64 * KC) != hipSuccess) { hulc_set_error("%s: hipMalloc failed", who); return 1; }
    int ns;
    static h16_t* zp = nullptr;
    if (!zp) { if (hipMalloc(&zp, 256) != hipSuccess) { hulc_set_error("%s: hipMalloc failed", who); return 1; } hipMemset(zp, 0, 256); }
    if (db_out) hipMemsetAsync(bias_tmp, 0, sizeof(float) * 64, st);
    if (which == 3) { const int OH = IH - 2; ns = launch_conv_wgrad_tr<64, 64, 3, 3, 1>(st, (const h16_t*)X, (const h16_t*)dY, part, bias_tmp, Nf, IH, IH, OH, OH, 512, nullptr, zp); }
    else if (which == 2) { const int OH = (IH - 4) / 2 + 1; ns = launch_conv_wgrad_tr<32, 64, 4, 4, 2>(st, (const h16_t*)X, (const h16_t*)dY, part, bias_tmp, Nf, IH, IH, OH, OH, 512, nullptr, zp); }
    else if (which == 1) { const int OH = (IH - 8) / 4 + 1; ns = launch_conv1_wgrad_tr(st, Conv1Src{X, nullptr, 0, 0}, (const h16_t*)dY, part, bias_tmp, Nf, IH, IH, OH, OH, 512); }
    else { hipFree(part); hulc_set_error("%s: which must be 1, 2 or 3", who); return 1; }
    hipMemsetAsync(out, 0, sizeof(float) * CO * KC, st);
    hipLaunchKernelGGL(unpack_conv_wgrad_kernel, dim3((CO * KC + 1023) / 1024), dim3(256), 0, st, part, ns, (long long)CO * KC, out, CO, KC, 1, 1, 0);
    if (db_out) hipMemcpyAsync(db_out, bias_tmp, sizeof(float) * CO, hipMemcpyDeviceToDevice, st);
    hipError_t e = hipStreamSynchronize(st);
    hipFree(part);
    if (e != hipSuccess) { hulc_set_error("%s: %s", who, hipGetErrorString(e)); return 1; }
    if (slabs) *slabs = ns;
    return 0;
}

int k_conv1_wgrad_u8(const char* who, int typed, const void* X, const int* shifts, int pad, const void* dY, float* dw_out, float* db_out, int Nf, int IH, int form, int fold, int* slabs,
                     void* stream) {
    hipStream_t st = (hipStream_t)stream;
    if (slabs) *slabs = 0;
    if (form != 1 && form != 2) { hulc_set_error("%s: form must be 1 or 2 (got %d)", who, form); return 1; }
    if (typed) {
        if (form != 2) { hulc_set_error("%s: form %d is a bench-only form (the engine runs form 2)", who, form); return 1; }
        if (!X || !dY || !dw_out || !db_out || Nf < 1 || IH < 8 || IH > 4096 || pad < 0 || pad > CONV1_RAW_MARGIN) { hulc_set_error("%s: null argument, or Nf=%d, IH=%d, pad=%d out of range", who, Nf, IH, pad); return 1; }
    }
    float *part = nullptr, *bias = nullptr;
    if (hipMalloc(&part, sizeof(float) * 512ll * 32 * 192) != hipSuccess || hipMalloc(&bias, sizeof(float) * 64) != hipSuccess) { hulc_set_error("%s: hipMalloc failed", who); return 1; }
    hipMemsetAsync(bias, 0, sizeof(float) * 64, st);
    Conv1Src src{}; src.X = X; src.shift = shifts; src.u8 = 1; src.pad = pad; src.fold = fold != 0;
    const int OH = (IH - 8) / 4 + 1;
    const int keep = g_conv1_wgrad_u8reg;
    g_conv1_wgrad_u8reg = form;
    const int ns = launch_conv1_wgrad_tr(st, src, (const h16_t*)dY, part, bias, Nf, IH, IH, OH, OH, 512);
    g_conv1_wgrad_u8reg = keep;
    hipMemsetAsync(dw_out, 0, sizeof(float) * 32 * 192, st);
    hipLaunchKernelGGL(unpack_conv_wgrad_kernel, dim3((32 * 192 + 1023) / 1024), dim3(256), 0, st, part, ns, (long long)32 * 192, dw_out, 32, 192, 1, 1, 0);
    hipMemcpyAsync(db_out, bias, sizeof(float) * 32, hipMemcpyDeviceToDevice, st);
    hipError_t e = hipStreamSynchronize(st);
    hipFree(part); hipFree(bias);
    if (e != hipSuccess) { hulc_set_error("%s: %s", who, hipGetErrorString(e)); return 1; }
    if (slabs) *slabs = ns;
    return 0;
}

int k_conv_tile(const char* who, int typed, int mode, const void* img, const void* w, const float* bias, const void* mask, void* out, unsigned* bits1_out, int Nf, int IMH, int OUTH,
                int relu, int wgs, void* stream) {
    hipStream_t st = (hipStream_t)stream;
    if (mode < 0 || mode > 29 || (mode >= 14 && mode <= 16) || (mode >= 24 && mode <= 26)) { hulc_set_error("%s: unsupported mode %d", who, mode); return 1; }
    if ((relu & ~(1 | 32 | 256)) || ((relu & 256) && mode != 5 && mode != 6)) { hulc_set_error("%s: unknown bits in relu (%d) for mode %d", who, relu, mode); return 1; }
#ifdef HULC_HALF_F16
    if (k_conv_mode_bench_only(mode)) { hulc_set_error("%s: mode %d is a bench-only form: bf16 only", who, mode); return 1; }
#endif
    if (typed) {
        if (k_conv_mode_bench_only(mode) || (relu & 256)) { hulc_set_error("%s: mode %d, relu %d is a bench-only form no launch site of the engine names", who, mode, relu); return 1; }
        const int m10 = mode % 10;
        const bool c1 = mode >= 4 && mode <= 6, dg = !c1 && (m10 == 2 || m10 == 3 || m10 == 8 || m10 == 9), k3 = !c1 && (m10 == 0 || m10 == 2 || m10 == 8);
        if (!img || !w || !out || (!dg && !bias) || Nf < 1 || IMH < 1 || OUTH < 1 || IMH > 4096 || OUTH > 4096) { hulc_set_error("%s: null argument, or Nf=%d, IMH=%d, OUTH=%d out of range", who, Nf, IMH, OUTH); return 1; }
        const int want = c1 ? k_conv_fwd_side(IMH, 8, 4) : (k3 ? k_conv_fwd_side(dg ? OUTH : IMH, 3, 1) : k_conv_fwd_side(dg ? OUTH : IMH, 4, 2));
        if (want < 1 || want != (dg ? IMH : OUTH)) { hulc_set_error("%s: mode %d: out_side %d does not belong to in_side %d", who, mode, OUTH, IMH); return 1; }
        if (dg && !mask) { hulc_set_error("%s: mode %d is a data-gradient form and needs its mask", who, mode); return 1; }
        if (mode == 6 && !mask) { hulc_set_error("%s: mode 6 needs the shifts in mask", who); return 1; }
        if (!c1 && !dg && !(relu & 1)) { hulc_set_error("%s: mode %d: the forward forms run with ReLU (relu bit 0)", who, mode); return 1; }
        if (wgs < 0 || wgs > 512 || (wgs && mode < 10)) { hulc_set_error("%s: wgs=%d (0 .. 512; the weights-in-registers modes 10 .. 29 only)", who, wgs); return 1; }
        if (bits1_out && !c1) { hulc_set_error("%s: bits1_out goes with the conv1 forward (modes 4 .. 6); the conv2 forms emit their bit words into mask", who); return 1; }
    }
    ConvTileP p{}; p.img = (const h16_t*)img; p.IMH = p.IMW = IMH; p.w = (const h16_t*)w; p.out = (h16_t*)out; p.OUTH = p.OUTW = OUTH;
    p.bias = bias; p.mask = (const h16_t*)mask; p.relu = relu & 1; p.Nf = Nf;
    if (mode == 7) { p.mask = nullptr; p.bits_out = (unsigned*)mask; mode = 1; }
    else if (mode == 8 || mode == 9) { p.mask = nullptr; p.maskbits = (const unsigned*)mask; mode -= 6; }
    if (relu & 32) {
        static int* ctr = nullptr;
        if (!ctr && hipMalloc(&ctr, 256) != hipSuccess) { hulc_set_error("%s: hipMalloc failed", who); return 1; }
        hipMemsetAsync(ctr, 0, 256, st);
        p.work_ctr = ctr;
    }
    {
        static void* dp = nullptr;
        if (!dp && hipMalloc(&dp, 8192) != hipSuccess) { hulc_set_error("%s: hipMalloc failed", who); return 1; }
        p.dump = (h16_t*)dp;
    }
    bool ok = false;
    const int* const wgp = (typed && wgs > 0) ? &wgs : nullptr;
    if (mode == 17) { p.mask = nullptr; p.bits_out = (unsigned*)mask; mode = 11; }
    if (mode == 18) { p.mask = nullptr; p.maskbits = (const unsigned*)mask; mode = 12; }
    if (mode == 19) { p.mask = nullptr; p.maskbits = (const unsigned*)mask; mode = 13; }
    if (mode == 27) { p.mask = nullptr; p.bits_out = (unsigned*)mask; mode = 21; }
    if (mode == 28) { p.mask = nullptr; p.maskbits = (const unsigned*)mask; mode = 22; }
    if (mode == 29) { p.mask = nullptr; p.maskbits = (const unsigned*)mask; mode = 23; }
    if (mode == 12 || mode == 13 || mode == 22 || mode == 23) {
        static void* zp = nullptr;
        if (!zp) { if (hipMalloc(&zp, 256) != hipSuccess) { hulc_set_error("%s: hipMalloc failed", who); return 1; } hipMemset(zp, 0, 256); }
        p.zeros = (const h16_t*)zp;
    }
    if (mode == 20) ok = launch_conv_reg_jobs<64, 3, 3, 1, false, 1, 4>(st, &p, 1, wgp);
    else if (mode == 21) ok = launch_conv_reg_jobs<32, 4, 4, 2, false, 1, 4, true>(st, &p, 1, wgp);
    else if (mode == 22) ok = launch_conv_reg_jobs<64, 3, 3, 1, true, 1, 4, true, 1>(st, &p, 1, wgp);
    else if (mode == 23) ok = launch_conv_reg_jobs<64, 2, 2, 1, true, 2, 4, true, 1>(st, &p, 1, wgp);
    else if (mode == 10) ok = launch_conv_reg_fwd_jobs<64, 3, 3, 1>(st, &p, 1, wgp);
    else if (mode == 11) ok = launch_conv_reg_fwd_jobs<32, 4, 4, 2>(st, &p, 1, wgp);
#ifndef HULC_HALF_F16
    else if (mode == 12) ok = launch_conv_reg<64, 3, 3, 1, true>(st, p);
    else if (mode == 13) ok = launch_conv_reg<64, 2, 2, 1, true, 2>(st, p);
#endif
    else if (mode == 0) ok = launch_conv_tile<64, 64, 3, 3, 1, 1, false>(st, p);
    else if (mode == 1) ok = launch_conv_tile<32, 64, 4, 4, 2, 1, false>(st, p);
    else if (mode == 2) ok = launch_conv_tile<64, 64, 3, 3, 1, 1, true>(st, p);
    else if (mode == 3) ok = launch_conv_tile<64, 32, 2, 2, 1, 2, true>(st, p);
    else if (mode == 4) { launch_conv1_fwd(st, Conv1Src{img, nullptr, 0, 0}, (const h16_t*)w, bias, (h16_t*)out, Nf, IMH, IMH, OUTH, OUTH, false, bits1_out); ok = true; }
    else if (mode == 5 || mode == 6) {
        launch_conv1_fwd(st, Conv1Src{img, mode == 6 ? (const int*)mask : nullptr, 1, IMH >= 100 ? 10 : 4}, (const h16_t*)w, bias, (h16_t*)out, Nf, IMH, IMH, OUTH,
                         OUTH, (relu & 256) != 0, bits1_out);
        ok = true;
    }
    if (!ok) { hulc_set_error("%s: unsupported mode/shape", who); return 1; }
    if (hipGetLastError() != hipSuccess) { hulc_set_error("%s: launch failed", who); return 1; }
    return 0;
}

int k_conv_pair(const char* who, int typed, int stage, const hulc_conv_job* a, const hulc_conv_job* b, int wg_a, int wg_b, int* slabs, void* stream) {
    hipStream_t st = (hipStream_t)stream;
    const bool fwd = stage == HULC_PAIR_CONV2_FWD || stage == HULC_PAIR_CONV3_FWD, dgr = stage == HULC_PAIR_CONV3_DGRAD || stage == HULC_PAIR_CONV2_DGRAD;
    const bool wgr = stage == HULC_PAIR_CONV3_WGRAD || stage == HULC_PAIR_CONV2_WGRAD || stage == HULC_PAIR_CONV1_WGRAD;
    if (slabs) slabs[0] = slabs[1] = 0;
    if (!fwd && !dgr && !wgr) { hulc_set_error("%s: unknown stage %d", who, stage); return 1; }
    if (!a) { hulc_set_error("%s: job a is required", who); return 1; }
    if (wg_a < 1 || (b && wg_b < 1)) { hulc_set_error("%s: every job needs at least one workgroup", who); return 1; }
    if (wgr && !b) { hulc_set_error("%s: the weight-gradient stages need both jobs", who); return 1; }
    {
        const hulc_conv_job* src[2] = {a, b};
        for (int k = 0; k < (b ? 2 : 1); ++k)
            if (!src[k]->in || !src[k]->w || !src[k]->out || src[k]->frames < 1 || src[k]->in_side < 1 || src[k]->out_side < 1 || (wgr && !src[k]->bits)) { hulc_set_error("%s: incomplete job", who); return 1; }
    }
    if (wgr) {
        const int KH = stage == HULC_PAIR_CONV1_WGRAD ? 8 : (stage == HULC_PAIR_CONV3_WGRAD ? 3 : 4), S = stage == HULC_PAIR_CONV1_WGRAD ? 4 : (stage == HULC_PAIR_CONV3_WGRAD ? 1 : 2);
        if (a->in_side < KH || b->in_side < KH || a->out_side != (a->in_side - KH) / S + 1 || b->out_side != (b->in_side - KH) / S + 1) { hulc_set_error("%s: out_side does not belong to in_side", who); return 1; }
    } else if (typed) {
        const bool k3 = stage == HULC_PAIR_CONV3_FWD || stage == HULC_PAIR_CONV3_DGRAD;
        const hulc_conv_job* src[2] = {a, b};
        for (int k = 0; k < (b ? 2 : 1); ++k) {
            const int big = dgr ? src[k]->out_side : src[k]->in_side, small = dgr ? src[k]->in_side : src[k]->out_side;
            if (big > 4096 || k_conv_fwd_side(big, k3 ? 3 : 4, k3 ? 1 : 2) != small) { hulc_set_error("%s: out_side does not belong to in_side", who); return 1; }
            if (dgr && !src[k]->bits) { hulc_set_error("%s: a data-gradient job needs its mask (the ReLU bit words in bits)", who); return 1; }
            if (fwd && !src[k]->bias) { hulc_set_error("%s: a forward job needs its bias", who); return 1; }
        }
    }
    static void *dp = nullptr, *zp = nullptr;
    static int* ctr = nullptr;
    if (!dp && hipMalloc(&dp, 8192) != hipSuccess) { hulc_set_error("%s: hipMalloc failed", who); return 1; }
    if (!zp) { if (hipMalloc(&zp, 256) != hipSuccess) { hulc_set_error("%s: hipMalloc failed", who); return 1; } hipMemset(zp, 0, 256); }
    if (!ctr && hipMalloc(&ctr, 256) != hipSuccess) { hulc_set_error("%s: hipMalloc failed", who); return 1; }
    hipMemsetAsync(ctr, 0, 256, st);
    if (wgr) {
        const bool c1 = stage == HULC_PAIR_CONV1_WGRAD, c3 = stage == HULC_PAIR_CONV3_WGRAD;
        const int KC = c1 ? 192 : (c3 ? 576 : 512), CO = c1 ? 32 : 64;
        float* part = nullptr;
        if (hipMalloc(&part, sizeof(float) * (size_t)(wg_a + wg_b) * CO * KC) != hipSuccess) { hulc_set_error("%s: hipMalloc failed", who); return 1; }
        const hulc_conv_job* src[2] = {a, b};
        const int wg[2] = {wg_a, wg_b};
        int ns[2] = {0, 0};
        bool okw = false;
        if (c1) {
            Wgrad1Job J[2];
            for (int k = 0; k < 2; ++k) {
                Wgrad1Job q{}; q.S = Conv1Src{src[k]->in, nullptr, 0, 0}; q.work_ctr = ctr + 16 * k; q.dY = (const h16_t*)src[k]->w; q.bias_part = (float*)src[k]->bits;
                q.Nf = src[k]->frames; q.IH = q.IW = src[k]->in_side; q.OH = q.OW = src[k]->out_side;
                J[k] = q;
            }
            J[0].part = part;
            size_t l0 = 0, l1 = 0; int r, nb;
            okw = conv1_wgrad_plan(J[0].S, J[0].IH, J[0].IW, J[0].OH, J[0].OW, r, nb, l0) == conv1_wgrad_plan(J[1].S, J[1].IH, J[1].IW, J[1].OH, J[1].OW, r, nb, l1);
            if (okw) {
                for (int k = 0; k < 2; ++k) { hipMemsetAsync(src[k]->bits, 0, sizeof(float) * CO, st); hipMemsetAsync(src[k]->out, 0, sizeof(float) * CO * KC, st); }
                okw = launch_conv1_wgrad_jobs(st, J, 2, 1024, wg, ns);
            }
        } else {
            WgradJob J[2];
            for (int k = 0; k < 2; ++k) {
                WgradJob q{}; q.X = (const h16_t*)src[k]->in; q.dY = (const h16_t*)src[k]->w; q.bias_part = (float*)src[k]->bits; q.zeros = (const h16_t*)zp; q.work_ctr = ctr + 16 * k;
                q.Nf = src[k]->frames; q.IH = q.IW = src[k]->in_side; q.OH = q.OW = src[k]->out_side; q.FPB = 1;
                J[k] = q;
            }
            J[0].part = part;
            using W3 = WgradCamW<64, 3>; using W2 = WgradCamW<32, 4>;
            okw = c3 ? (a->in_side == W3::stat && b->in_side == W3::gripper) : (a->in_side == W2::stat && b->in_side == W2::gripper);
            if (okw) {
                for (int k = 0; k < 2; ++k) { hipMemsetAsync(src[k]->bits, 0, sizeof(float) * CO, st); hipMemsetAsync(src[k]->out, 0, sizeof(float) * CO * KC, st); }
                okw = c3 ? launch_conv_wgrad_pair<64, 64, 3, 3, 1>(st, J[0], J[1], 512, wg, ns) : launch_conv_wgrad_pair<32, 64, 4, 4, 2>(st, J[0], J[1], 512, wg, ns);
            }
        }
        if (okw) {
            hipLaunchKernelGGL(unpack_conv_wgrad_kernel, dim3((CO * KC + 1023) / 1024), dim3(256), 0, st, part, ns[0], (long long)CO * KC, (float*)a->out, CO, KC, 1, 1, 0);
            hipLaunchKernelGGL(unpack_conv_wgrad_kernel, dim3((CO * KC + 1023) / 1024), dim3(256), 0, st, part + (long long)ns[0] * CO * KC, ns[1], (long long)CO * KC, (float*)b->out, CO, KC, 1, 1, 0);
        }
        const hipError_t e = hipStreamSynchronize(st);
        hipFree(part);
        if (!okw) { hulc_set_error("%s: unsupported shape (the two cameras' maps only)", who); return 1; }
        if (e != hipSuccess) { hulc_set_error("%s: %s", who, hipGetErrorString(e)); return 1; }
        if (slabs) { slabs[0] = ns[0]; slabs[1] = ns[1]; }
        return 0;
    }
    ConvTileP j[2]; int wg[2] = {wg_a, wg_b};
    const hulc_conv_job* src[2] = {a, b};
    const int n = b ? 2 : 1;
    for (int k = 0; k < n; ++k) {
        ConvTileP p{}; p.img = (const h16_t*)src[k]->in; p.IMH = p.IMW = src[k]->in_side; p.w = (const h16_t*)src[k]->w; p.out = (h16_t*)src[k]->out; p.OUTH = p.OUTW = src[k]->out_side;
        p.Nf = src[k]->frames; p.dump = (h16_t*)dp;
        if (fwd) { p.bias = src[k]->bias; p.relu = 1; p.bits_out = (unsigned*)src[k]->bits; }
        else { p.maskbits = (const unsigned*)src[k]->bits; p.zeros = (const h16_t*)zp; }
        p.work_ctr = ctr + 16 * k;
        j[k] = p;
    }
    bool ok = false;
    if (stage == HULC_PAIR_CONV2_FWD) ok = launch_conv_reg_fwd_jobs<32, 4, 4, 2>(st, j, n, wg);
    else if (stage == HULC_PAIR_CONV3_FWD) ok = launch_conv_reg_fwd_jobs<64, 3, 3, 1>(st, j, n, wg);
    else if (stage == HULC_PAIR_CONV3_DGRAD) ok = launch_conv_reg_jobs<64, 3, 3, 1, true, 1, 4, true, 1>(st, j, n, wg);
    else ok = launch_conv_reg_jobs<64, 2, 2, 1, true, 2, 4, true, 1>(st, j, n, wg);
    if (!ok) { hulc_set_error("%s: unsupported shape", who); return 1; }
    if (hipGetLastError() != hipSuccess) { hulc_set_error("%s: launch failed", who); return 1; }
    return 0;
}

int k_conv_plan(int form, int frames, int in_side, int out_side, int wgs, int* nbands, int* rows_per_band, int* frames_per_band, int* items) {
    static const char* who = "hulc_k_conv_plan";
    if (!nbands || !rows_per_band || !frames_per_band || !items || frames < 1 || in_side < 1 || out_side < 1 || in_side > 4096 || out_side > 4096) { hulc_set_error("%s: null argument or frames=%d, in_side=%d, out_side=%d out of range", who, frames, in_side, out_side); return 1; }
    const int m10 = form % 10;
    const bool known = (form >= 10 && form <= 13) || (form >= 17 && form <= 23) || (form >= 27 && form <= 29);
    if (!known) { hulc_set_error("%s: form %d is not a weights-in-registers form", who, form); return 1; }
    const bool dg = m10 == 2 || m10 == 3 || m10 == 8 || m10 == 9, k3 = m10 == 0 || m10 == 2 || m10 == 8, bitsf = m10 == 8 || m10 == 9;
    if (k_conv_fwd_side(dg ? out_side : in_side, k3 ? 3 : 4, k3 ? 1 : 2) != (dg ? in_side : out_side)) { hulc_set_error("%s: form %d: out_side %d does not belong to in_side %d", who, form, out_side, in_side); return 1; }
    const h16_t* al = reinterpret_cast<const h16_t*>((uintptr_t)0x10000);
    ConvTileP p{}; p.IMH = p.IMW = in_side; p.OUTH = p.OUTW = out_side; p.Nf = frames;
    if (!dg) p.relu = 1;
    else { p.zeros = al; if (bitsf) p.maskbits = reinterpret_cast<const unsigned*>(al); else p.mask = al; }
    size_t lds = 0; int it = 0; double work = 0;
    bool ok = false;
    const int w8 = wgs > 0 ? wgs : 256, w4 = wgs > 0 ? wgs : 512;
    if (form == 10) ok = plan_conv_reg<64, 3, 3, 1, false, 1, 8, true>(p, w8, lds, it, work);
    else if (form == 11 || form == 17) ok = plan_conv_reg<32, 4, 4, 2, false, 1, 8, true>(p, w8, lds, it, work);
    else if (form == 20) ok = plan_conv_reg<64, 3, 3, 1, false, 1, 4>(p, w4, lds, it, work);
    else if (form == 21 || form == 27) ok = plan_conv_reg<32, 4, 4, 2, false, 1, 4, true>(p, w4, lds, it, work);
    else if (form == 22 || form == 28) ok = plan_conv_reg<64, 3, 3, 1, true, 1, 4, true, 1>(p, w4, lds, it, work);
    else if (form == 23 || form == 29) ok = plan_conv_reg<64, 2, 2, 1, true, 2, 4, true, 1>(p, w4, lds, it, work);
    else if (form == 12 || form == 18) ok = plan_conv_reg<64, 3, 3, 1, true>(p, w8, lds, it, work);
    else ok = plan_conv_reg<64, 2, 2, 1, true, 2>(p, w8, lds, it, work);
    if (!ok) { hulc_set_error("%s: form %d does not take frames=%d, in_side=%d, out_side=%d", who, form, frames, in_side, out_side); return 1; }
    *nbands = p.FPB > 1 ? 1 : p.nbands; *rows_per_band = p.RB; *frames_per_band = p.FPB; *items = it;
    return 0;
}

}
```

### hulc_amd/lib.py

```python
from __future__ import annotations

import ctypes as C
import os

_HERE = os.path.dirname(os.path.abspath(__file__))
LIB_PATH = os.path.join(_HERE, "csrc", "libhulc_hip.so")

KIND = {"hulc": 0, "gcbc": 1, "mcil": 2, "mcil_gru": 3}
DTYPE = {"fp32": 0, "bf16": 1, "fp16": 2}


class HulcConfig(C.Structure):
    _fields_ = [("kind", C.c_int32), ("dtype", C.c_int32), ("max_batch", C.c_int32), ("max_seq", C.c_int32),
                ("max_window", C.c_int32), ("use_clip", C.c_int32), ("kl_beta", C.c_float),
                ("kl_balancing_mix", C.c_float), ("dropout_p", C.c_float), ("num_classes", C.c_int32),
                ("gripper_alpha", C.c_float), ("log_scale_min", C.c_float), ("seed", C.c_uint64)]


class HulcBatch(C.Structure):
    _fields_ = [("B", C.c_int32), ("S", C.c_int32), ("is_lang", C.c_int32), ("rgb_static", C.c_void_p),
                ("rgb_gripper", C.c_void_p), ("actions", C.c_void_p), ("robot_obs", C.c_void_p), ("lang", C.c_void_p),
                ("plan_idx", C.c_void_p), ("aux_rows", C.c_void_p), ("n_aux", C.c_int32), ("step", C.c_uint64),
                ("frames_u8", C.c_int32), ("pad_static", C.c_int32), ("pad_gripper", C.c_int32), ("shift_static", C.c_void_p),
                ("shift_gripper", C.c_void_p), ("plan_eps", C.c_void_p), ("actions_absolute", C.c_int32), ("max_rel_pos", C.c_float),
                ("max_rel_orn", C.c_float), ("window_start", C.c_void_p), ("store_frames", C.c_int64), ("window_len", C.c_void_p),
                ("window_len_host", C.c_void_p)]


class HulcStoreTables(C.Structure):
    _fields_ = [("actions", C.c_void_p), ("robot_obs", C.c_void_p), ("lang", C.c_void_p), ("store_frames", C.c_int64), ("lang_rows", C.c_int32), ("absolute", C.c_int32)]


class HulcStageCopy(C.Structure):
    _fields_ = [("src", C.c_void_p), ("dst", C.c_void_p), ("bytes", C.c_int64)]


class HulcValNoise(C.Structure):
    _fields_ = [("plan_idx_pp", C.c_void_p), ("plan_idx_pr", C.c_void_p), ("u_mix_pp", C.c_void_p), ("u_act_pp", C.c_void_p),
                ("u_mix_pr", C.c_void_p), ("u_act_pr", C.c_void_p)]


class HulcRolloutObs(C.Structure):
    _fields_ = [("rgb_static", C.c_void_p), ("rgb_gripper", C.c_void_p), ("robot_obs_raw", C.c_void_p)]


class HulcRolloutEnvsObs(C.Structure):
    _fields_ = [("n", C.c_int32), ("slots", C.c_void_p), ("rgb_static", C.c_void_p), ("rgb_gripper", C.c_void_p), ("robot_obs_raw", C.c_void_p)]


class HulcOptim(C.Structure):
    _fields_ = [("kind", C.c_int32), ("lr", C.c_float), ("beta1", C.c_float), ("beta2", C.c_float), ("eps", C.c_float), ("weight_decay", C.c_float),
                ("momentum", C.c_float), ("dampening", C.c_float), ("nesterov", C.c_int32), ("step", C.c_int64), ("grad_scale", C.c_float)]


DECODER = {"logistic": 0, "deterministic": 1}
CRITERION = {"HuberLoss": 0, "MSELoss": 1}
BODY = {"rnn": 0, "mlp": 1}
OPTIM = {"adam": 0, "adamw": 1, "sgd": 2}
CLIP = {"off": 0, "norm": 1, "value": 2}


class HulcSbertConfig(C.Structure):
    _fields_ = [("layers", C.c_int32), ("hidden", C.c_int32), ("heads", C.c_int32), ("intermediate", C.c_int32), ("vocab", C.c_int32),
                ("max_position", C.c_int32), ("max_sentences", C.c_int32), ("max_tokens", C.c_int32), ("normalize", C.c_int32), ("ln_eps", C.c_float)]


class HulcConvJob(C.Structure):
    _fields_ = [("input", C.c_void_p), ("w", C.c_void_p), ("bias", C.c_void_p), ("out", C.c_void_p), ("bits", C.c_void_p),
                ("frames", C.c_int32), ("in_side", C.c_int32), ("out_side", C.c_int32)]


class HulcEncTailJob(C.Structure):
    _fields_ = [("x", C.c_void_p), ("W1", C.c_void_p), ("W2", C.c_void_p), ("b1", C.c_void_p), ("b2", C.c_void_p), ("lng", C.c_void_p), ("lnb", C.c_void_p),
                ("f1", C.c_void_p), ("f2", C.c_void_p), ("lnst", C.c_void_p), ("col0", C.c_int32)]


class HulcEncTailBwdJob(C.Structure):
    _fields_ = [("f2", C.c_void_p), ("lnst", C.c_void_p), ("lng", C.c_void_p), ("f1", C.c_void_p), ("W2t", C.c_void_p), ("W1t", C.c_void_p), ("xmask", C.c_void_p),
                ("dlng", C.c_void_p), ("dlnb", C.c_void_p), ("d_f2", C.c_void_p), ("d_f1", C.c_void_p), ("dx_f32", C.c_void_p), ("dx_t", C.c_void_p), ("col0", C.c_int32)]


class HulcTrLayerJob(C.Structure):
    _fields_ = [(n, C.c_void_p) for n in ("xin", "ln_g", "ln_b", "xf_out", "xt_out", "st_out", "Wqkv", "Wo", "W1", "W2", "bqkv", "bo", "b1", "b2", "n1g", "n1b",
                                          "qkv", "Pat", "ao", "y1", "st1", "x1t", "x1f", "hff", "y2")] + \
               [(n, C.c_uint64) for n in ("seed_att", "seed_o", "seed_h", "seed_y")]


class HulcTrFfnBwdJob(C.Structure):
    _fields_ = [(n, C.c_void_p) for n in ("dx", "y2", "st2", "n2g", "dg2", "db2", "W2t", "W1t", "hff", "dt_c", "dt_a", "part")] + [("seed_y", C.c_uint64)]


class HulcTrAttnBwdJob(C.Structure):
    _fields_ = [(n, C.c_void_p) for n in ("parts", "y1", "st1", "n1g", "dg1", "db1", "Wot", "Wint", "qkv", "Pat", "b_d", "b_b", "dy_f", "dx")] + \
               [("seed_o", C.c_uint64), ("seed_att", C.c_uint64)]


class HulcGemmEpiJob(C.Structure):
    _fields_ = [("A", C.c_void_p), ("B", C.c_void_p), ("M", C.c_int32), ("N", C.c_int32), ("K", C.c_int32), ("lda", C.c_int64), ("ldb", C.c_int64),
                ("ldc", C.c_int64), ("out_R1", C.c_int32), ("out_s0", C.c_int64), ("nsplit", C.c_int32), ("wfrag", C.c_int32),
                ("out", C.c_void_p), ("out_f32", C.c_int32), ("accumulate", C.c_int32), ("atomic", C.c_int32), ("z_stride", C.c_int64),
                ("bias", C.c_void_p), ("bias2", C.c_void_p), ("res", C.c_void_p), ("res_f32", C.c_int32), ("res_ld", C.c_int64), ("res_rowmod", C.c_int32),
                ("res_late", C.c_int32), ("mask", C.c_void_p), ("mask_tanh", C.c_int32), ("relu", C.c_int32), ("alpha", C.c_float), ("drop_p", C.c_float),
                ("drop_seed", C.c_uint64), ("out2", C.c_void_p), ("out2_lo", C.c_int64), ("out2_hi", C.c_int64), ("out2_mask", C.c_void_p),
                ("out2_relu", C.c_int32), ("generic_only", C.c_int32)]


GEMM_RAN = {"none": 0, "32": 1, "64": 2, "128": 3, "glds": 4, "skinny_router": 5, "skinny_reg": 6, "kchunk": 7, "splitk_64": 8, "splitk_128": 9, "group": 10, "pair": 11,
            "dual": 12}

EXPORTS = ["hulc_last_error", "hulc_ctx_create", "hulc_ctx_destroy", "hulc_set_stream", "hulc_workspace_bytes",
           "hulc_bind_params", "hulc_prepare_weights", "hulc_zero_grads", "hulc_flush_grads", "hulc_forward_loss", "hulc_forward_loss_pair", "hulc_backward", "hulc_backward_part",
           "hulc_adam_step", "hulc_optimizer_step", "hulc_comm_unique_id", "hulc_comm_prepare", "hulc_comm_init", "hulc_comm_destroy", "hulc_comm_buckets", "hulc_comm_stats", "hulc_comm_size", "hulc_comm_timeline", "hulc_allreduce_grads", "hulc_backward_allreduce", "hulc_scaler_enable", "hulc_scaler_get", "hulc_scaler_set", "hulc_grad_clip_set", "hulc_grad_norm_get", "hulc_validate", "hulc_store_gather", "hulc_store_stage", "hulc_store_stage_join", "hulc_store_stage_stats", "hulc_clip_gt_encode", "hulc_clip_gt_scores", "hulc_aux_heads_enable", "hulc_decoder_select", "hulc_aux_weights_set", "hulc_aux_losses_get", "hulc_rollout_reset", "hulc_rollout_plan", "hulc_rollout_act", "hulc_rollout_get_goal", "hulc_rollout_set_state", "hulc_rollout_envs_init", "hulc_rollout_envs_reset", "hulc_rollout_envs_plan", "hulc_rollout_envs_act", "hulc_rollout_envs_get_state", "hulc_rollout_envs_set_state", "hulc_sbert_create", "hulc_sbert_destroy", "hulc_sbert_set_stream", "hulc_sbert_bind", "hulc_sbert_encode", "hulc_set_kl_beta", "hulc_set_dropout", "hulc_set_option", "hulc_get_option", "hulc_timers_enable", "hulc_timers_read", "hulc_get_tensor", "hulc_get_plan_idx", "hulc_k_gemm_nt", "hulc_k_cast", "hulc_k_trread_probe", "hulc_k_conv_wgrad", "hulc_k_conv1_wgrad_u8", "hulc_k_conv1_interior_groups", "hulc_k_conv_tile", "hulc_k_camera_split", "hulc_k_conv_pair", "hulc_k_skinny", "hulc_k_attention", "hulc_k_rnn_persist", "hulc_k_rnn_persist_flag_words", "hulc_k_clip_loss", "hulc_k_clip_loss_fp32", "hulc_k_mia_head", "hulc_k_cosine_dist", "hulc_k_spatial_softmax64", "hulc_k_enc_tail_fwd", "hulc_k_enc_tail_bwd", "hulc_k_logistic_loss",
           "hulc_k_plan_kl_sample", "hulc_k_st_softmax_bwd", "hulc_k_plan_gather", "hulc_k_plan_scatter_grad", "hulc_k_normal_kl_sample", "hulc_k_normal_rsample_bwd",
           "hulc_k_layernorm_fwd", "hulc_k_layernorm_bwd", "hulc_k_layernorm_mean", "hulc_k_tr_layer_fwd", "hulc_k_tr_ffn_bwd", "hulc_k_tr_attn_bwd",
           "hulc_k_window_compact", "hulc_k_rows_expand", "hulc_k_rows_reduce", "hulc_k_gemm_epi", "hulc_k_gemm_multi", "hulc_k_gemm_pick", "hulc_k_gemm_wgrad_nsplit",
           "hulc_k_det_head_loss", "hulc_k_det_head_bwd", "hulc_k_det_head_act",
           "hulc_k_conv_wgrad_t", "hulc_k_conv1_wgrad_u8_t", "hulc_k_conv_tile_t", "hulc_k_conv_pair_t", "hulc_k_conv_plan",
           "hulc_decoder_body_select"]

_lib = None


def load():
    global _lib
    if _lib is not None:
        return _lib
    path = os.environ.get("HULC_LIB_PATH") or LIB_PATH
    if not os.path.exists(path):
        raise RuntimeError(f"hulc_amd: {path} not built — run `python -c 'import __graft_entry__ as g; g.build()'`; "
                           "there is no CPU fallback for the product path")
    import torch
    lib = C.CDLL(path)
    lib.hulc_last_error.restype = C.c_char_p
    lib.hulc_workspace_bytes.restype = C.c_int64
    lib.hulc_ctx_create.argtypes = [C.POINTER(HulcConfig), C.POINTER(C.c_void_p)]
    lib.hulc_ctx_destroy.argtypes = [C.c_void_p]
    lib.hulc_set_stream.argtypes = [C.c_void_p, C.c_void_p]
    lib.hulc_workspace_bytes.argtypes = [C.c_void_p]
    lib.hulc_bind_params.argtypes = [C.c_void_p, C.c_void_p, C.c_void_p, C.c_void_p, C.c_void_p, C.c_int64, C.c_int32,
                                     C.POINTER(C.c_char_p), C.POINTER(C.c_int64), C.POINTER(C.c_int64)]
    lib.hulc_prepare_weights.argtypes = [C.c_void_p]
    lib.hulc_zero_grads.argtypes = [C.c_void_p]
    if os.environ.get("HULC_LIB_PATH") and not hasattr(lib, "hulc_flush_grads"):
        lib.hulc_zero_grads.argtypes = [C.c_void_p]
    else:
        lib.hulc_flush_grads.argtypes = [C.c_void_p]
    lib.hulc_forward_loss.argtypes = [C.c_void_p, C.POINTER(HulcBatch), C.c_float, C.c_float, C.c_void_p, C.c_int32]
    lib.hulc_forward_loss_pair.argtypes = [C.c_void_p, C.POINTER(HulcBatch), C.POINTER(HulcBatch), C.c_float, C.c_float, C.c_void_p, C.c_int32]
    lib.hulc_backward.argtypes = [C.c_void_p]
    lib.hulc_backward_part.argtypes = [C.c_void_p, C.c_int32]
    lib.hulc_adam_step.argtypes = [C.c_void_p, C.c_float, C.c_float, C.c_float, C.c_float, C.c_int64, C.c_float]
    lib.hulc_optimizer_step.argtypes = [C.c_void_p, C.POINTER(HulcOptim)]
    lib.hulc_comm_unique_id.argtypes = [C.c_void_p, C.c_int64]
    lib.hulc_comm_prepare.argtypes = [C.c_void_p]
    lib.hulc_comm_init.argtypes = [C.c_void_p, C.c_void_p, C.c_int32, C.c_int32]
    lib.hulc_comm_destroy.argtypes = [C.c_void_p]
    lib.hulc_comm_buckets.argtypes = [C.c_void_p, C.POINTER(C.c_int64), C.POINTER(C.c_int64), C.c_int32]
    lib.hulc_comm_stats.argtypes = [C.c_void_p, C.POINTER(C.c_int64), C.POINTER(C.c_double)]
    if hasattr(lib, "hulc_comm_size") or not os.environ.get("HULC_LIB_PATH"):
        lib.hulc_comm_size.argtypes = [C.c_void_p, C.POINTER(C.c_int32), C.POINTER(C.c_int32)]
    lib.hulc_comm_timeline.argtypes = [C.c_void_p, C.POINTER(C.c_double), C.c_int32, C.POINTER(C.c_double)]
    lib.hulc_allreduce_grads.argtypes = [C.c_void_p, C.c_int32]
    lib.hulc_backward_allreduce.argtypes = [C.c_void_p, C.c_int32]
    lib.hulc_scaler_enable.argtypes = [C.c_void_p, C.c_float, C.c_float, C.c_float, C.c_int32]
    lib.hulc_scaler_get.argtypes = [C.c_void_p, C.POINTER(C.c_float), C.POINTER(C.c_int32), C.POINTER(C.c_int64), C.POINTER(C.c_int32), C.POINTER(C.c_int64)]
    lib.hulc_scaler_set.argtypes = [C.c_void_p, C.c_float, C.c_int32, C.c_int64]
    if hasattr(lib, "hulc_grad_clip_set") or not os.environ.get("HULC_LIB_PATH"):
        lib.hulc_grad_clip_set.argtypes = [C.c_void_p, C.c_int32, C.c_float, C.c_int32]
        lib.hulc_grad_norm_get.argtypes = [C.c_void_p, C.POINTER(C.c_float), C.POINTER(C.c_float), C.c_void_p, C.c_int64]
    lib.hulc_clip_gt_encode.argtypes = [C.c_void_p, C.c_void_p, C.c_int32, C.c_int32]
    lib.hulc_clip_gt_scores.argtypes = [C.c_void_p, C.c_int32, C.c_void_p, C.c_int64, C.POINTER(C.c_int32), C.POINTER(C.c_int32)]
    if hasattr(lib, "hulc_aux_heads_enable") or not os.environ.get("HULC_LIB_PATH"):
        lib.hulc_aux_heads_enable.argtypes = [C.c_void_p, C.c_int32, C.c_int32]
        lib.hulc_aux_weights_set.argtypes = [C.c_void_p, C.c_float, C.c_float]
        lib.hulc_aux_losses_get.argtypes = [C.c_void_p, C.c_void_p]
    lib.hulc_validate.argtypes = [C.c_void_p, C.POINTER(HulcBatch), C.POINTER(HulcValNoise), C.c_void_p, C.c_void_p, C.c_void_p, C.c_void_p, C.c_void_p]
    if hasattr(lib, "hulc_store_gather") or not os.environ.get("HULC_LIB_PATH"):
        lib.hulc_store_gather.argtypes = [C.c_void_p, C.POINTER(HulcStoreTables), C.c_void_p, C.c_void_p, C.c_void_p, C.c_int32, C.c_int32, C.c_void_p, C.c_void_p, C.c_void_p]
    if hasattr(lib, "hulc_store_stage") or not os.environ.get("HULC_LIB_PATH"):
        lib.hulc_store_stage.restype = C.c_int64
        lib.hulc_store_stage.argtypes = [C.c_void_p, C.POINTER(HulcStageCopy), C.c_int32]
        lib.hulc_store_stage_join.argtypes = [C.c_void_p, C.c_int64]
        lib.hulc_store_stage_stats.argtypes = [C.c_void_p, C.POINTER(C.c_int64), C.POINTER(C.c_int64), C.POINTER(C.c_int64)]
    lib.hulc_rollout_reset.argtypes = [C.c_void_p]
    lib.hulc_rollout_plan.argtypes = [C.c_void_p, C.POINTER(HulcRolloutObs), C.c_void_p, C.c_void_p, C.c_void_p, C.c_void_p, C.c_void_p]
    lib.hulc_rollout_act.argtypes = [C.c_void_p, C.POINTER(HulcRolloutObs), C.c_void_p, C.c_void_p, C.c_void_p]
    lib.hulc_rollout_get_goal.argtypes = [C.c_void_p, C.c_void_p]
    lib.hulc_rollout_set_state.argtypes = [C.c_void_p, C.c_void_p, C.c_void_p]
    if hasattr(lib, "hulc_rollout_envs_init") or not os.environ.get("HULC_LIB_PATH"):
        lib.hulc_rollout_envs_init.argtypes = [C.c_void_p, C.c_int32]
        lib.hulc_rollout_envs_reset.argtypes = [C.c_void_p, C.c_int32, C.c_void_p, C.c_int32]
        lib.hulc_rollout_envs_plan.argtypes = [C.c_void_p, C.POINTER(HulcRolloutEnvsObs), C.c_void_p, C.c_void_p, C.c_void_p, C.c_void_p, C.c_void_p, C.c_void_p]
        lib.hulc_rollout_envs_act.argtypes = [C.c_void_p, C.POINTER(HulcRolloutEnvsObs), C.c_void_p, C.c_void_p, C.c_void_p]
        lib.hulc_rollout_envs_get_state.argtypes = [C.c_void_p, C.c_int32, C.c_void_p, C.c_void_p, C.c_void_p]
        lib.hulc_rollout_envs_set_state.argtypes = [C.c_void_p, C.c_int32, C.c_void_p, C.c_void_p, C.c_void_p]
    lib.hulc_sbert_create.argtypes = [C.POINTER(HulcSbertConfig), C.POINTER(C.c_void_p)]
    lib.hulc_sbert_destroy.argtypes = [C.c_void_p]
    lib.hulc_sbert_set_stream.argtypes = [C.c_void_p, C.c_void_p]
    lib.hulc_sbert_bind.argtypes = [C.c_void_p, C.c_void_p, C.c_int64, C.c_int32, C.POINTER(C.c_char_p), C.POINTER(C.c_int64), C.POINTER(C.c_int64)]
    lib.hulc_sbert_encode.argtypes = [C.c_void_p, C.c_void_p, C.c_void_p, C.c_int32, C.c_int32, C.c_void_p]
    lib.hulc_set_kl_beta.argtypes = [C.c_void_p, C.c_float]
    lib.hulc_set_dropout.argtypes = [C.c_void_p, C.c_float]
    lib.hulc_timers_enable.argtypes = [C.c_void_p, C.c_int32, C.c_char_p]
    lib.hulc_set_option.argtypes = [C.c_void_p, C.c_char_p, C.c_int64]
    lib.hulc_get_option.argtypes = [C.c_void_p, C.c_char_p, C.POINTER(C.c_int64)]
    lib.hulc_k_rnn_persist.argtypes = [C.c_void_p, C.c_void_p, C.c_void_p, C.c_void_p, C.c_int32, C.c_int32, C.c_int32, C.c_int32, C.c_int32, C.c_void_p, C.c_void_p, C.c_uint32, C.c_void_p]
    lib.hulc_k_rnn_persist_flag_words.restype = C.c_int32
    lib.hulc_timers_read.argtypes = [C.c_void_p, C.c_char_p, C.c_int64, C.c_int32]
    lib.hulc_get_tensor.argtypes = [C.c_void_p, C.c_char_p, C.c_void_p, C.c_int64, C.POINTER(C.c_int64)]
    lib.hulc_get_plan_idx.argtypes = [C.c_void_p, C.c_void_p, C.c_int64]
    lib.hulc_k_gemm_nt.argtypes = [C.c_int32, C.c_void_p, C.c_void_p, C.c_void_p, C.c_int32, C.c_int32, C.c_int32, C.c_int64,
                                   C.c_int64, C.c_int64, C.c_void_p, C.c_int32, C.c_void_p]
    lib.hulc_k_conv_wgrad.argtypes = [C.c_int32, C.c_void_p, C.c_void_p, C.c_void_p, C.c_int32, C.c_int32, C.c_void_p]
    if hasattr(lib, "hulc_k_conv1_wgrad_u8") or not os.environ.get("HULC_LIB_PATH"):
        lib.hulc_k_conv1_interior_groups.argtypes = [C.c_int32, C.c_int32, C.c_int32, C.POINTER(C.c_int32), C.POINTER(C.c_int32)]
        lib.hulc_k_conv1_wgrad_u8.argtypes = [C.c_void_p, C.c_void_p, C.c_int32, C.c_void_p, C.c_void_p, C.c_void_p, C.c_int32, C.c_int32, C.c_int32, C.c_int32, C.c_void_p]
    lib.hulc_k_conv_tile.argtypes = [C.c_int32, C.c_void_p, C.c_void_p, C.c_void_p, C.c_void_p, C.c_void_p, C.c_int32, C.c_int32, C.c_int32,
                                     C.c_int32, C.c_void_p]
    if hasattr(lib, "hulc_k_conv_pair") or not os.environ.get("HULC_LIB_PATH"):
        lib.hulc_k_camera_split.argtypes = [C.c_int32, C.c_double, C.c_double, C.POINTER(C.c_int32), C.POINTER(C.c_int32)]
        lib.hulc_k_conv_pair.argtypes = [C.c_int32, C.POINTER(HulcConvJob), C.POINTER(HulcConvJob), C.c_int32, C.c_int32, C.c_void_p]
    lib.hulc_k_skinny.argtypes = [C.c_void_p, C.c_void_p, C.c_void_p, C.c_int32, C.c_int32, C.c_int32, C.c_int32, C.c_void_p]
    lib.hulc_k_trread_probe.argtypes = [C.c_void_p, C.c_void_p, C.c_void_p]
    lib.hulc_k_cast.argtypes = [C.c_int32, C.c_void_p, C.c_void_p, C.c_int64, C.c_void_p]
    if hasattr(lib, "hulc_k_clip_loss") or not os.environ.get("HULC_LIB_PATH"):
        for f in (lib.hulc_k_clip_loss, lib.hulc_k_clip_loss_fp32):
            f.argtypes = [C.c_void_p, C.c_void_p, C.c_int32, C.c_void_p, C.c_float, C.c_void_p, C.c_void_p, C.c_void_p, C.c_void_p, C.c_void_p]
        lib.hulc_k_mia_head.argtypes = [C.c_void_p, C.c_void_p, C.c_int32, C.c_void_p, C.c_void_p, C.c_void_p, C.c_void_p, C.c_float, C.c_void_p, C.c_void_p, C.c_void_p,
                                        C.c_int32, C.c_void_p, C.c_void_p, C.c_void_p, C.c_void_p, C.c_void_p]
        lib.hulc_k_cosine_dist.argtypes = [C.c_void_p, C.c_void_p, C.c_int32, C.c_int32, C.c_float, C.c_void_p, C.c_void_p, C.c_void_p]
    lib.hulc_k_attention.argtypes = [C.c_int32, C.c_void_p, C.c_void_p, C.c_void_p, C.c_void_p, C.c_void_p, C.c_int32, C.c_int32, C.c_float, C.c_uint64, C.c_void_p]
    if hasattr(lib, "hulc_k_enc_tail_fwd") or not os.environ.get("HULC_LIB_PATH"):
        lib.hulc_k_spatial_softmax64.argtypes = [C.c_int32, C.c_void_p, C.c_int32, C.c_int32, C.c_int32, C.c_void_p, C.c_void_p, C.c_void_p, C.c_void_p, C.c_void_p]
        lib.hulc_k_enc_tail_fwd.argtypes = [C.c_int32, C.c_int32, C.c_int32, C.POINTER(HulcEncTailJob), C.POINTER(HulcEncTailJob), C.c_void_p, C.c_void_p, C.c_int32,
                                            C.c_float, C.c_uint64, C.c_void_p, C.c_void_p, C.c_void_p, C.c_void_p, C.c_void_p]
        lib.hulc_k_enc_tail_bwd.argtypes = [C.c_int32, C.c_int32, C.c_int32, C.POINTER(HulcEncTailBwdJob), C.POINTER(HulcEncTailBwdJob), C.c_void_p, C.c_void_p]
        lib.hulc_k_logistic_loss.argtypes = [C.c_int32, C.c_int32, C.c_void_p, C.c_int32, C.c_void_p, C.c_void_p, C.c_int32, C.c_int32, C.c_int32, C.c_int32, C.c_int32,
                                             C.c_float, C.c_float, C.c_int32, C.c_int32, C.c_float, C.c_void_p, C.c_void_p, C.c_void_p, C.c_void_p, C.c_void_p]
    if hasattr(lib, "hulc_k_layernorm_bwd") or not os.environ.get("HULC_LIB_PATH"):
        P, I, F, U, Q = C.c_void_p, C.c_int32, C.c_float, C.c_uint64, C.c_int64
        lib.hulc_k_plan_kl_sample.argtypes = [P, P, I, I, I, P, P, P, P, P, P, F, F, U, P, P]
        lib.hulc_k_st_softmax_bwd.argtypes = [I, P, P, P, P, I, I, P, P, P, P]
        lib.hulc_k_plan_gather.argtypes = [I, P, P, I, I, I, I, P, P, P, P, P, I, I, P, I, I, P, P]
        lib.hulc_k_plan_scatter_grad.argtypes = [I, I, P, P, I, I, I, I, I, P, I, P]
        lib.hulc_k_normal_kl_sample.argtypes = [I, P, P, I, I, P, P, P, P, P, P, P, F, F, U, P, P]
        lib.hulc_k_normal_rsample_bwd.argtypes = [I, P, P, P, P, I, I, P, P]
        lib.hulc_k_layernorm_fwd.argtypes = [I, P, Q, I, I, P, P, P, Q, P, Q, P, P]
        lib.hulc_k_layernorm_bwd.argtypes = [I, P, Q, P, Q, P, P, I, I, P, Q, I, P, Q, P, P, F, U, I, F, I, Q, P, P]
        lib.hulc_k_layernorm_mean.argtypes = [I, P, I, I, I, P, P, P, P, P, P]
    if hasattr(lib, "hulc_k_tr_layer_fwd") or not os.environ.get("HULC_LIB_PATH"):
        lib.hulc_k_tr_layer_fwd.argtypes = [C.c_int32, C.POINTER(HulcTrLayerJob), C.c_int32, C.c_int32, C.c_int32, C.c_float, C.c_void_p]
        lib.hulc_k_tr_ffn_bwd.argtypes = [C.c_int32, C.POINTER(HulcTrFfnBwdJob), C.c_int32, C.c_int32, C.c_int32, C.c_float, C.c_float, C.c_void_p]
        lib.hulc_k_tr_attn_bwd.argtypes = [C.c_int32, C.POINTER(HulcTrAttnBwdJob), C.c_int32, C.c_int32, C.c_int32, C.c_int64, C.c_float, C.c_void_p]
    if hasattr(lib, "hulc_k_rows_reduce") or not os.environ.get("HULC_LIB_PATH"):
        P, I, Q = C.c_void_p, C.c_int32, C.c_int64
        lib.hulc_k_window_compact.argtypes = [P, P, P, I, I, I, Q, P, P, P, P, P, P]
        lib.hulc_k_rows_expand.argtypes = [I, P, P, P, I, I, I, P, P]
        lib.hulc_k_rows_reduce.argtypes = [P, P, P, I, I, I, P, P]
    if hasattr(lib, "hulc_k_gemm_epi") or not os.environ.get("HULC_LIB_PATH"):
        I, Q, PI = C.c_int32, C.c_int64, C.POINTER(C.c_int32)
        lib.hulc_k_gemm_epi.argtypes = [I, C.POINTER(HulcGemmEpiJob), I, PI, C.c_void_p]
        lib.hulc_k_gemm_multi.argtypes = [I, I, C.POINTER(HulcGemmEpiJob), I, I, PI, C.c_void_p]
        lib.hulc_k_gemm_pick.argtypes = [I, I, I, I, Q, Q, PI, PI]
        lib.hulc_k_gemm_wgrad_nsplit.argtypes = [I, I, I, I, PI, PI]
    if hasattr(lib, "hulc_decoder_select") or not os.environ.get("HULC_LIB_PATH"):
        P, I, F = C.c_void_p, C.c_int32, C.c_float
        lib.hulc_decoder_select.argtypes = [P, I, I]
        lib.hulc_k_det_head_loss.argtypes = [I, P, P, P, P, P, I, I, I, I, F, P, P, P, P, P]
        lib.hulc_k_det_head_bwd.argtypes = [I, P, P, P, I, I, P, P, P, P, P]
        lib.hulc_k_det_head_act.argtypes = [I, P, P, P, P, I, P, P]
    if hasattr(lib, "hulc_decoder_body_select") or not os.environ.get("HULC_LIB_PATH"):
        lib.hulc_decoder_body_select.argtypes = [C.c_void_p, C.c_int32]
    if hasattr(lib, "hulc_k_conv_plan") or not os.environ.get("HULC_LIB_PATH"):
        P, I, PI = C.c_void_p, C.c_int32, C.POINTER(C.c_int32)
        lib.hulc_k_conv_wgrad_t.argtypes = [I, I, P, P, P, P, I, I, PI, P]
        lib.hulc_k_conv1_wgrad_u8_t.argtypes = [I, P, P, I, P, P, P, I, I, I, I, PI, P]
        lib.hulc_k_conv_tile_t.argtypes = [I, I, P, P, P, P, P, P, I, I, I, I, I, P]
        lib.hulc_k_conv_pair_t.argtypes = [I, I, C.POINTER(HulcConvJob), C.POINTER(HulcConvJob), I, I, PI, P]
        lib.hulc_k_conv_plan.argtypes = [I, I, I, I, I, PI, PI, PI, PI]
    _lib = lib
    return lib


def check(rc: int):
    if rc != 0:
        raise RuntimeError("libhulc_hip: " + load().hulc_last_error().decode("utf-8", "replace"))
```

### include/hulc_hip.h

```cpp
#ifndef HULC_HIP_H
#define HULC_HIP_H
#include <stdint.h>

#ifdef __cplusplus
extern "C" {
#endif

typedef struct hulc_ctx hulc_ctx;

enum { HULC_KIND_HULC = 0, HULC_KIND_GCBC = 1, HULC_KIND_MCIL = 2, HULC_KIND_MCIL_GRU = 3 };
enum { HULC_DTYPE_F32 = 0, HULC_DTYPE_BF16 = 1, HULC_DTYPE_F16 = 2 };

typedef struct hulc_config {
    int32_t kind;
    int32_t dtype;
    int32_t max_batch;
    int32_t max_seq;
    int32_t max_window;
    int32_t use_clip;
    float kl_beta;
    float kl_balancing_mix;
    float dropout_p;
    int32_t num_classes;
    float gripper_alpha;
    float log_scale_min;
    uint64_t seed;
} hulc_config;

typedef struct hulc_batch {
    int32_t B, S;
    int32_t is_lang;
    const void* rgb_static;
    const void* rgb_gripper;
    const float* actions;
    const float* robot_obs;
    const float* lang;
    const int32_t* plan_idx;
    const int32_t* aux_rows;
    int32_t n_aux;
    uint64_t step;
    int32_t frames_u8;
    int32_t pad_static, pad_gripper;
    const int32_t* shift_static;
    const int32_t* shift_gripper;
    const float* plan_eps;
    int32_t actions_absolute;
    float max_rel_pos, max_rel_orn;
    const int64_t* window_start;
    int64_t store_frames;
    const int32_t* window_len;
    const int32_t* window_len_host;
} hulc_batch;

#define HULC_N_LOSSES 4

const char* hulc_last_error(void);
int hulc_ctx_create(const hulc_config* cfg, hulc_ctx** out);
int hulc_ctx_destroy(hulc_ctx* ctx);
int hulc_set_stream(hulc_ctx* ctx, void* hip_stream);
int64_t hulc_workspace_bytes(const hulc_ctx* ctx);

int hulc_bind_params(hulc_ctx* ctx, float* params, float* grads, float* adam_m, float* adam_v, int64_t numel,
                     int32_t n_tensors, const char* const* names, const int64_t* offsets, const int64_t* numels);
int hulc_prepare_weights(hulc_ctx* ctx);
int hulc_zero_grads(hulc_ctx* ctx);
int hulc_flush_grads(hulc_ctx* ctx);

int hulc_forward_loss(hulc_ctx* ctx, const hulc_batch* batch, float loss_weight, float clip_weight, float* out_losses,
                      int32_t losses_on_host);
int hulc_forward_loss_pair(hulc_ctx* ctx, const hulc_batch* vis, const hulc_batch* lang, float loss_weight, float clip_weight, float* out_losses,
                           int32_t losses_on_host);
int hulc_backward(hulc_ctx* ctx);
int hulc_backward_part(hulc_ctx* ctx, int32_t part);
int hulc_adam_step(hulc_ctx* ctx, float lr, float beta1, float beta2, float eps, int64_t step, float grad_scale);
enum { HULC_OPT_ADAM = 0, HULC_OPT_ADAMW = 1, HULC_OPT_SGD = 2 };
typedef struct hulc_optim {
    int32_t kind;
    float lr, beta1, beta2, eps, weight_decay;
    float momentum, dampening;
    int32_t nesterov;
    int64_t step;
    float grad_scale;
} hulc_optim;
int hulc_optimizer_step(hulc_ctx* ctx, const hulc_optim* opt);

int hulc_comm_unique_id(void* out_host , int64_t cap);
int hulc_comm_prepare(hulc_ctx* ctx);
int hulc_comm_init(hulc_ctx* ctx, const void* unique_id_host, int32_t rank, int32_t world);
int hulc_comm_destroy(hulc_ctx* ctx);
int hulc_comm_buckets(hulc_ctx* ctx, int64_t* lo, int64_t* hi, int32_t cap);
int hulc_comm_stats(hulc_ctx* ctx, int64_t* n_collectives, double* bytes_on_wire_per_rank);
int hulc_comm_size(hulc_ctx* ctx, int32_t* rank, int32_t* world);
int hulc_comm_timeline(hulc_ctx* ctx, double* out, int32_t cap_buckets, double* backward_us);
int hulc_allreduce_grads(hulc_ctx* ctx, int32_t bucket_dtype);
int hulc_backward_allreduce(hulc_ctx* ctx, int32_t bucket_dtype);

int hulc_scaler_enable(hulc_ctx* ctx, float init_scale, float growth_factor, float backoff_factor, int32_t growth_interval);
int hulc_scaler_get(hulc_ctx* ctx, float* scale, int32_t* growth_tracker, int64_t* skipped_steps, int32_t* last_found_inf,
                    int64_t* taken_steps );
int hulc_scaler_set(hulc_ctx* ctx, float scale, int32_t growth_tracker, int64_t taken_steps);

enum { HULC_CLIP_OFF = 0, HULC_CLIP_NORM = 1, HULC_CLIP_VALUE = 2 };
int hulc_grad_clip_set(hulc_ctx* ctx, int32_t algo, float limit, int32_t track);
int hulc_grad_norm_get(hulc_ctx* ctx, float* total, float* coef, float* per_tensor_host, int64_t cap);

typedef struct hulc_val_noise {
    const int32_t* plan_idx_pp;
    const int32_t* plan_idx_pr;
    const float* u_mix_pp;
    const float* u_act_pp;
    const float* u_mix_pr;
    const float* u_act_pr;
} hulc_val_noise;
#define HULC_N_VAL 18
int hulc_validate(hulc_ctx* ctx, const hulc_batch* batch, const hulc_val_noise* noise, float* out_host, int32_t* plan_idx_pp_out,
                  int32_t* plan_idx_pr_out, float* pred_pp_out, float* pred_pr_out);

typedef struct hulc_store_tables {
    const float* actions;
    const float* robot_obs;
    const float* lang;
    int64_t store_frames;
    int32_t lang_rows;
    int32_t absolute;
} hulc_store_tables;
int hulc_store_gather(hulc_ctx* ctx, const hulc_store_tables* tables, const int64_t* window_start , const int32_t* window_len ,
                      const int32_t* lang_row , int32_t B, int32_t S, float* actions_out ,
                      float* robot_obs_out , float* lang_out );

#define HULC_STAGE_TICKETS 32
typedef struct hulc_stage_copy { const void* src; void* dst; int64_t bytes; } hulc_stage_copy;
int64_t hulc_store_stage(hulc_ctx* ctx, const hulc_stage_copy* copies, int32_t n);
int hulc_store_stage_join(hulc_ctx* ctx, int64_t ticket);
int hulc_store_stage_stats(hulc_ctx* ctx, int64_t* calls, int64_t* copies, int64_t* bytes);

#define HULC_GT_TRAIN 0
#define HULC_GT_VAL 1
int hulc_clip_gt_encode(hulc_ctx* ctx, const float* lang_emb, int32_t m, int32_t slot);
int hulc_clip_gt_scores(hulc_ctx* ctx, int32_t slot, float* scores_host, int64_t cap_floats, int32_t* n_out, int32_t* m_out);

int hulc_aux_heads_enable(hulc_ctx* ctx, int32_t bc_z, int32_t mia);
int hulc_aux_weights_set(hulc_ctx* ctx, float bc_z_weight, float mia_weight);
int hulc_aux_losses_get(hulc_ctx* ctx, float* out_host );

#define HULC_DECODER_LOGISTIC 0
#define HULC_DECODER_DETERMINISTIC 1
#define HULC_CRIT_HUBER 0
#define HULC_CRIT_MSE 1
int hulc_decoder_select(hulc_ctx* ctx, int32_t decoder, int32_t criterion);

#define HULC_BODY_RNN 0
#define HULC_BODY_MLP 1
int hulc_decoder_body_select(hulc_ctx* ctx, int32_t body);

typedef struct hulc_rollout_obs {
    const float* rgb_static;
    const float* rgb_gripper;
    const float* robot_obs_raw;
} hulc_rollout_obs;
int hulc_rollout_reset(hulc_ctx* ctx);
int hulc_rollout_plan(hulc_ctx* ctx, const hulc_rollout_obs* obs, const float* goal_rgb_static, const float* goal_rgb_gripper,
                      const float* goal_lang ,
                      const int32_t* plan_idx_inject , int32_t* plan_idx_out );
int hulc_rollout_act(hulc_ctx* ctx, const hulc_rollout_obs* obs, const float* u_mix ,
                     const float* u_act , float* action_out_host );
int hulc_rollout_get_goal(hulc_ctx* ctx, float* latent_goal_out );
int hulc_rollout_set_state(hulc_ctx* ctx, const void* plan, const float* latent_goal );

typedef struct hulc_rollout_envs_obs {
    int32_t n;
    const int32_t* slots;
    const float* rgb_static;
    const float* rgb_gripper;
    const float* robot_obs_raw;
} hulc_rollout_envs_obs;
int hulc_rollout_envs_init(hulc_ctx* ctx, int32_t max_envs);
int hulc_rollout_envs_reset(hulc_ctx* ctx, int32_t n, const int32_t* slots , int32_t clear_hidden);
int hulc_rollout_envs_plan(hulc_ctx* ctx, const hulc_rollout_envs_obs* obs, const float* goal_rgb_static , const float* goal_rgb_gripper,
                           const float* goal_lang , const void* plan_inject, void* plan_out, float* latent_goal_out);
int hulc_rollout_envs_act(hulc_ctx* ctx, const hulc_rollout_envs_obs* obs, const float* u_mix, const float* u_act, float* actions_out_host );
int hulc_rollout_envs_get_state(hulc_ctx* ctx, int32_t n, const int32_t* slots, void* plan_out, float* latent_goal_out);
int hulc_rollout_envs_set_state(hulc_ctx* ctx, int32_t n, const int32_t* slots, const void* plan, const float* latent_goal);

typedef struct hulc_sbert_config {
    int32_t layers, hidden, heads, intermediate, vocab, max_position;
    int32_t max_sentences, max_tokens;
    int32_t normalize;
    float ln_eps;
} hulc_sbert_config;
typedef struct hulc_sbert hulc_sbert;
int hulc_sbert_create(const hulc_sbert_config* cfg, hulc_sbert** out);
int hulc_sbert_destroy(hulc_sbert* ctx);
int hulc_sbert_set_stream(hulc_sbert* ctx, void* hip_stream);
int hulc_sbert_bind(hulc_sbert* ctx, const float* flat_params, int64_t numel, int32_t n_tensors, const char* const* names,
                    const int64_t* offsets, const int64_t* numels);
int hulc_sbert_encode(hulc_sbert* ctx, const int32_t* token_ids, const int32_t* attention_mask, int32_t B, int32_t L, float* out);

int hulc_set_kl_beta(hulc_ctx* ctx, float kl_beta);
int hulc_set_dropout(hulc_ctx* ctx, float p);

int hulc_set_option(hulc_ctx* ctx, const char* name, int64_t value);
int hulc_get_option(hulc_ctx* ctx, const char* name, int64_t* value);

int hulc_timers_enable(hulc_ctx* ctx, int32_t on, const char* only_class );
int hulc_timers_read(hulc_ctx* ctx, char* json_out, int64_t cap, int32_t reset);

int hulc_get_tensor(hulc_ctx* ctx, const char* name, float* host_out, int64_t cap, int64_t* n);
int hulc_get_plan_idx(hulc_ctx* ctx, int32_t* host_out, int64_t cap);

int hulc_k_gemm_nt(int32_t dtype, const void* A, const void* B, float* C, int32_t M, int32_t N, int32_t K, int64_t lda,
                   int64_t ldb, int64_t ldc, const float* bias, int32_t relu, void* hip_stream);
int hulc_k_conv_wgrad(int32_t which, const void* X, const void* dY, float* out, int32_t Nf, int32_t IH, void* hip_stream);
int hulc_k_conv1_interior_groups(int32_t IW, int32_t pad, int32_t cap, int32_t* first, int32_t* count);
int hulc_k_conv1_wgrad_u8(const void* X, const int32_t* shifts, int32_t pad, const void* dY, float* dw_out, float* db_out, int32_t Nf, int32_t IH, int32_t form, int32_t fold, void* hip_stream);
int hulc_k_conv_tile(int32_t mode, const void* img, const void* w, const float* bias, const void* mask, void* out, int32_t Nf, int32_t IMH,
                     int32_t OUTH, int32_t relu, void* hip_stream);
int hulc_k_camera_split(int32_t grid, double work_static, double work_gripper, int32_t* wg_static, int32_t* wg_gripper);
typedef struct hulc_conv_job {
    const void* in; const void* w; const float* bias; void* out; void* bits;
    int32_t frames, in_side, out_side;
} hulc_conv_job;
enum { HULC_PAIR_CONV2_FWD = 2, HULC_PAIR_CONV3_FWD = 3, HULC_PAIR_CONV2_DGRAD = 12, HULC_PAIR_CONV3_DGRAD = 13, HULC_PAIR_CONV1_WGRAD = 21, HULC_PAIR_CONV2_WGRAD = 22, HULC_PAIR_CONV3_WGRAD = 23 };
int hulc_k_conv_pair(int32_t stage, const hulc_conv_job* a, const hulc_conv_job* b, int32_t wg_a, int32_t wg_b, void* hip_stream);
int hulc_k_conv_wgrad_t(int32_t dtype, int32_t which, const void* X, const void* dY, float* out, float* db_out, int32_t Nf, int32_t IH, int32_t* slabs, void* hip_stream);
int hulc_k_conv1_wgrad_u8_t(int32_t dtype, const void* X, const int32_t* shifts, int32_t pad, const void* dY, float* dw_out, float* db_out, int32_t Nf, int32_t IH, int32_t form,
                            int32_t fold, int32_t* slabs, void* hip_stream);
int hulc_k_conv_tile_t(int32_t dtype, int32_t mode, const void* img, const void* w, const float* bias, const void* mask, void* out, uint32_t* bits1_out, int32_t Nf, int32_t IMH,
                       int32_t OUTH, int32_t relu, int32_t wgs, void* hip_stream);
int hulc_k_conv_pair_t(int32_t dtype, int32_t stage, const hulc_conv_job* a, const hulc_conv_job* b, int32_t wg_a, int32_t wg_b, int32_t* slabs, void* hip_stream);
int hulc_k_conv_plan(int32_t form, int32_t frames, int32_t in_side, int32_t out_side, int32_t wgs, int32_t* nbands, int32_t* rows_per_band, int32_t* frames_per_band, int32_t* items);
int hulc_k_skinny(const void* A, const void* W, void* out, int32_t M, int32_t N, int32_t K, int32_t variant, void* hip_stream);
int hulc_k_rnn_persist(void* X, const void* W, const void* res, const void* mask, int32_t B, int32_t S, int32_t q0, int32_t dq, int32_t act,
                       uint32_t* flags, uint32_t* err, uint32_t launch_index, void* hip_stream);
int32_t hulc_k_rnn_persist_flag_words(void);
int hulc_k_trread_probe(const int32_t* elem_index_per_lane , uint16_t* out , void* hip_stream);
int hulc_k_cast(int32_t dtype, const float* src, void* dst, int64_t n, void* hip_stream);
int hulc_k_attention(int32_t variant, const float* qkv, float* P, float* ao, const float* dao, float* dqkv, int32_t B, int32_t S,
                     float drop_p, uint64_t seed, void* hip_stream);

int hulc_k_clip_loss(const float* img, const float* txt, int32_t n, const float* logit_scale, float w, float* loss_out, float* dimg, float* dtxt,
                     float* dlogit_scale, void* hip_stream);
int hulc_k_clip_loss_fp32(const float* img, const float* txt, int32_t n, const float* logit_scale, float w, float* loss_out, float* dimg, float* dtxt,
                          float* dlogit_scale, void* hip_stream);
int hulc_k_mia_head(const float* img, const float* txt, int32_t n, const float* W0, const float* b0, const float* W1, const float* b1, float w, float* loss_out,
                    float* dimg, float* dtxt, int32_t accum, float* dW0, float* db0, float* dW1, float* db1, void* hip_stream);
int hulc_k_cosine_dist(const float* pred, const float* tgt, int32_t n, int32_t D, float w, float* loss_out, float* dpred, void* hip_stream);

int hulc_k_spatial_softmax64(int32_t dtype, const void* f, int32_t H, int32_t W, int32_t Nf, void* out, float* stats, const float* dout, void* df, void* hip_stream);
typedef struct hulc_enc_tail_job {
    const void* x; const void* W1; const void* W2; const float* b1; const float* b2; const float* lng; const float* lnb;
    void* f1; float* f2; float* lnst;
    int32_t col0;
} hulc_enc_tail_job;
int hulc_k_enc_tail_fwd(int32_t dtype, int32_t Nf, int32_t ldemb, const hulc_enc_tail_job* a, const hulc_enc_tail_job* b, void* emb, const float* pos, int32_t S,
                        float drop_p, uint64_t seed, float* xf, void* xt, float* z0, float* z1, void* hip_stream);
typedef struct hulc_enc_tail_bwd_job {
    const float* f2; const float* lnst; const float* lng; const void* f1; const void* W2t; const void* W1t; const void* xmask;
    float* dlng; float* dlnb; void* d_f2; void* d_f1; float* dx_f32; void* dx_t;
    int32_t col0;
} hulc_enc_tail_bwd_job;
int hulc_k_enc_tail_bwd(int32_t dtype, int32_t Nf, int32_t ldemb, const hulc_enc_tail_bwd_job* a, const hulc_enc_tail_bwd_job* b, const float* demb, void* hip_stream);
int hulc_k_logistic_loss(int32_t dtype, int32_t wide, const float* heads, int32_t ldh, const float* actions, const float* robot_obs, int32_t B, int32_t S,
                         int32_t n_mix, int32_t n_dim, int32_t num_classes, float log_scale_min, float gripper_alpha, int32_t gripper_control,
                         int32_t discrete_gripper, float grad_scale, const float* lscale, float* row_loss, float* a_tcp_out, void* dheads, void* hip_stream);

int hulc_k_det_head_loss(int32_t dtype, const void* H1, const void* W, const float* bias, const float* actions, const float* robot_obs, int32_t B, int32_t S,
                         int32_t criterion, int32_t frame, float grad_scale, const float* lscale, float* row_loss, float* pred, float* dpre, void* hip_stream);
int hulc_k_det_head_bwd(int32_t dtype, const float* dpre, const void* W, const void* H1, int32_t B, int32_t S, void* dH1, void* dZ1, float* dW, float* db,
                        void* hip_stream);
int hulc_k_det_head_act(int32_t dtype, const void* h1, const void* W, const float* bias, const float* robot_obs, int32_t n, float* out, void* hip_stream);

int hulc_k_plan_kl_sample(const float* pr_logits, const float* pp_logits, int32_t B, int32_t NCAT, int32_t NCLS, const int32_t* idx_in, int32_t* idx_out, float* probs,
                          float* kl_cat, float* dpp, float* dpr, float w_pp, float w_pr, uint64_t seed, const float* lscale, void* hip_stream);
int hulc_k_st_softmax_bwd(int32_t dtype, const float* probs, const float* dplan, const float* dpr_kl, const float* dpp_kl, int32_t rows, int32_t NCLS, float* out,
                          void* out_t, void* dpp_t, void* hip_stream);
int hulc_k_plan_gather(int32_t dtype, const void* w_t, const int32_t* idx, int32_t B, int32_t NCAT, int32_t NCLS, int32_t H, const float* b1, const float* b2, float* out,
                       const void* emb, void* embg, int32_t S, int32_t W, const void* goal, int32_t G, int32_t grow0, void* cb, void* hip_stream);
int hulc_k_plan_scatter_grad(int32_t dtype, int32_t form, const void* dC, const int32_t* idx, int32_t B, int32_t NCAT, int32_t NCLS, int32_t H, int32_t KIN, float* dw,
                             int32_t store, void* hip_stream);
int hulc_k_normal_kl_sample(int32_t dtype, const float* pr_state, const float* pp_state, int32_t B, int32_t n, const float* eps_in, float* eps_out, float* plan_f, void* plan_t,
                            float* kl_elem, float* dpp, float* dpr, float w_pp, float w_pr, uint64_t seed, const float* lscale, void* hip_stream);
int hulc_k_normal_rsample_bwd(int32_t dtype, const float* dplan, const float* eps, const float* pr_state, const float* dpr_kl, int32_t B, int32_t n, void* out,
                              void* hip_stream);
int hulc_k_layernorm_fwd(int32_t dtype, const float* x, int64_t ldx, int32_t rows, int32_t n, const float* g, const float* b, void* out, int64_t ldo, float* out_f32,
                         int64_t ldf, float* stats, void* hip_stream);
int hulc_k_layernorm_bwd(int32_t dtype, const float* dy, int64_t lddy, const float* x, int64_t ldx, const float* stats, const float* g, int32_t rows, int32_t n, float* dx_f32,
                         int64_t ldd, int32_t accumulate, void* dx_t, int64_t ldt, float* dg, float* db, float drop_p, uint64_t seed, int32_t bcast_rows, float bcast_div,
                         int32_t dy_parts, int64_t dy_part_stride, float* scratch, void* hip_stream);
int hulc_k_layernorm_mean(int32_t dtype, const float* x, int32_t B, int32_t S, int32_t n, const float* g, const float* b, float* stats, void* out, float* yout,
                          void* hip_stream);
int hulc_k_window_compact(const int64_t* window_start, const int32_t* lens, const int32_t* off, int32_t off_base, int32_t B, int32_t S, int64_t store_frames,
                          const int32_t* shift_static, const int32_t* shift_gripper, int64_t* frame_out, int32_t* shift_static_out, int32_t* shift_gripper_out,
                          void* hip_stream);
int hulc_k_rows_expand(int32_t elem_bytes, const void* src, const int32_t* lens, const int32_t* off, int32_t B, int32_t S, int32_t n, void* dst, void* hip_stream);
int hulc_k_rows_reduce(const float* src, const int32_t* lens, const int32_t* off, int32_t B, int32_t S, int32_t n, float* dst, void* hip_stream);

typedef struct hulc_tr_layer_job {
    const float* xin; const float* ln_g; const float* ln_b; float* xf_out; void* xt_out; float* st_out;
    const void* Wqkv; const void* Wo; const void* W1; const void* W2;
    const float* bqkv; const float* bo; const float* b1; const float* b2; const float* n1g; const float* n1b;
    void* qkv; float* Pat; void* ao; float* y1; float* st1; void* x1t; float* x1f; void* hff; float* y2;
    uint64_t seed_att, seed_o, seed_h, seed_y;
} hulc_tr_layer_job;
int hulc_k_tr_layer_fwd(int32_t dtype, const hulc_tr_layer_job* job, int32_t B, int32_t S, int32_t ln_in, float dp, void* hip_stream);
typedef struct hulc_tr_ffn_bwd_job {
    const float* dx; const float* y2; const float* st2; const float* n2g; float* dg2; float* db2;
    const void* W2t; const void* W1t; const void* hff; void* dt_c; void* dt_a; float* part;
    uint64_t seed_y;
} hulc_tr_ffn_bwd_job;
int hulc_k_tr_ffn_bwd(int32_t dtype, const hulc_tr_ffn_bwd_job* job, int32_t B, int32_t S, int32_t bcast, float bdiv, float dp, void* hip_stream);
typedef struct hulc_tr_attn_bwd_job {
    const float* parts; const float* y1; const float* st1; const float* n1g; float* dg1; float* db1;
    const void* Wot; const void* Wint; const void* qkv; const float* Pat; void* b_d; void* b_b; float* dy_f; float* dx;
    uint64_t seed_o, seed_att;
} hulc_tr_attn_bwd_job;
int hulc_k_tr_attn_bwd(int32_t dtype, const hulc_tr_attn_bwd_job* job, int32_t B, int32_t S, int32_t nparts, int64_t part_stride, float dp, void* hip_stream);

typedef struct hulc_gemm_epi_job {
    const void* A; const void* B; int32_t M, N, K; int64_t lda, ldb;
    int64_t ldc; int32_t out_R1; int64_t out_s0;
    int32_t nsplit, wfrag;
    void* out; int32_t out_f32, accumulate, atomic; int64_t z_stride;
    const float* bias; const float* bias2;
    const void* res; int32_t res_f32; int64_t res_ld; int32_t res_rowmod, res_late;
    const void* mask; int32_t mask_tanh, relu; float alpha, drop_p; uint64_t drop_seed;
    void* out2; int64_t out2_lo, out2_hi; const void* out2_mask; int32_t out2_relu, generic_only;
} hulc_gemm_epi_job;
enum { HULC_GEMM_RAN_NONE = 0, HULC_GEMM_RAN_32 = 1, HULC_GEMM_RAN_64 = 2, HULC_GEMM_RAN_128 = 3, HULC_GEMM_RAN_GLDS = 4, HULC_GEMM_RAN_SKINNY_ROUTER = 5, HULC_GEMM_RAN_SKINNY_REG = 6,
       HULC_GEMM_RAN_KCHUNK = 7, HULC_GEMM_RAN_SPLITK_64 = 8, HULC_GEMM_RAN_SPLITK_128 = 9, HULC_GEMM_RAN_GROUP = 10, HULC_GEMM_RAN_PAIR = 11, HULC_GEMM_RAN_DUAL = 12 };
int hulc_k_gemm_epi(int32_t dtype, const hulc_gemm_epi_job* job, int32_t kernel, int32_t* ran, void* hip_stream);
int hulc_k_gemm_multi(int32_t dtype, int32_t form, const hulc_gemm_epi_job* jobs, int32_t n, int32_t sh, int32_t* ran, void* hip_stream);
int hulc_k_gemm_pick(int32_t dtype, int32_t M, int32_t N, int32_t K, int64_t lda, int64_t ldb, int32_t* pick, int32_t* bk);
int hulc_k_gemm_wgrad_nsplit(int32_t dtype, int32_t M, int32_t N, int32_t K, int32_t* nsplit, int32_t* big);

#ifdef __cplusplus
}
#endif
#endif
```

Measured before the change: 21790 windows/s.

## Pack stride-1 wgrad dY rows densely and let the DMA body use eight n-tile quarters

```diff
diff --git a/hulc_amd/csrc/capi.hip b/hulc_amd/csrc/capi.hip
--- a/hulc_amd/csrc/capi.hip
+++ b/hulc_amd/csrc/capi.hip
@@ -567,6 +567,14 @@
 }
 int hulc_k_conv_plan(int32_t form, int32_t frames, int32_t in_side, int32_t out_side, int32_t wgs, int32_t* nbands, int32_t* rows_per_band, int32_t* frames_per_band, int32_t* items) {
     return hulc_bf16::k_conv_plan(form, frames, in_side, out_side, wgs, nbands, rows_per_band, frames_per_band, items);
+}
+
+int hulc_k_conv_slab_sum(const float* slabs, int32_t nsplit, int32_t O, int32_t I, int32_t KH, int32_t KW, int32_t nhwc, int32_t yparts, float* grad, void* stream) {
+    return hulc_bf16::k_conv_slab_sum(slabs, nsplit, O, I, KH, KW, nhwc, yparts, grad, stream);
+}
+int hulc_k_conv_wgrad_run_map(int32_t form, int32_t in_side, int32_t out_side, int32_t rows_per_band, int32_t real_rows, int32_t frames_per_band, int32_t capacity, int32_t* dy_pixel, int32_t* x_pixel,
+                              int32_t* valid, int32_t* steps) {
+    return hulc_bf16::k_conv_wgrad_run_map(form, in_side, out_side, rows_per_band, real_rows, frames_per_band, capacity, dy_pixel, x_pixel, valid, steps);
 }
 
 int hulc_k_camera_split(int32_t grid, double work_static, double work_gripper, int32_t* wg_static, int32_t* wg_gripper) {
diff --git a/hulc_amd/csrc/conv_wgrad.h b/hulc_amd/csrc/conv_wgrad.h
--- a/hulc_amd/csrc/conv_wgrad.h
+++ b/hulc_amd/csrc/conv_wgrad.h
@@ -25,10 +25,45 @@
     static constexpr int NTW = NT / 4;
     static constexpr int CT = CO / 16;
     static_assert(NT % 4 == 0, "n-tiles must split over 4 waves");
-    static size_t lds_bytes(int R, int IW, int OW) {
-        const int OWp = (OW + 7) / 8 * 8;
+    static constexpr bool DENSE = S == 1;
+    static constexpr __host__ __device__ int owd(int OW) { return DENSE ? OW : (OW + 7) / 8 * 8; }
+    static size_t lds_bytes(int R, int IW, int OW, bool padded = false) {
         const int XR = (R - 1) * S + KH;
-        return (size_t)(XR * IW + 8 * S + KW) * XS + (size_t)(R * OWp + 8) * DYS;
+        return (size_t)(XR * IW + 8 * S + KW) * XS + (size_t)(R * (padded ? (OW + 7) / 8 * 8 : owd(OW)) + 8) * DYS;
+    }
+};
+
+struct WgradRunMap {
+    int OWd, RF, nk, S, IH, IW, xs;
+    int dc, dr, step_x, wrap_row, wrap_frame;
+    bool frames;
+    struct Pos { int c, r, x; };
+    __host__ __device__ WgradRunMap(bool dense, int S_, int IH_, int IW_, int OH, int OW, int R, int FPB, int xs_) : S(S_), IH(IH_), IW(IW_), xs(xs_) {
+        frames = dense && FPB > 1;
+        OWd = dense ? OW : (OW + 7) / 8 * 8;
+        RF = frames ? OH : (1 << 20);
+        nk = frames ? FPB * OH * OW : R * OWd;
+        int rem = 32, df = 0;
+        if (frames) { df = rem / (OH * OWd); rem -= df * OH * OWd; }
+        dr = rem / OWd; dc = rem - dr * OWd;
+        step_x = ((df * IH + dr * S) * IW + dc * S) * xs;
+        wrap_row = (S * IW - OWd * S) * xs;
+        wrap_frame = frames ? (IH - RF * S) * IW * xs : 0;
+    }
+    __host__ __device__ int steps() const { return (nk + 31) / 32; }
+    __host__ __device__ Pos at(int p) const {
+        int fi = 0;
+        if (frames) { fi = p / (RF * OWd); p -= fi * RF * OWd; }
+        Pos q;
+        q.r = p / OWd; q.c = p - q.r * OWd;
+        q.x = ((fi * IH + q.r * S) * IW + q.c * S) * xs;
+        return q;
+    }
+    template <bool FR> __host__ __device__ void advance(Pos& q) const {
+        q.x += step_x; q.c += dc;
+        if (FR) q.r += dr;
+        if (q.c >= OWd) { q.c -= OWd; q.x += wrap_row; if (FR) ++q.r; }
+        if (FR) { if (q.r >= RF) { q.r -= RF; q.x += wrap_frame; } }
     }
 };
 
@@ -166,10 +201,11 @@
     constexpr int NTH = NWV * 64, PF = 8192 / NTH, CTH = C::CT / (NWV / 4), CHY = CO / 8, CHX = CI / 8;
     extern __shared__ __attribute__((aligned(16))) char smem[];
     const int tid = threadIdx.x, lane = tid & 63, wave = tid >> 6;
-    const int OWp = (OW + 7) & ~7, U = OWp >> 3;
+    const WgradRunMap M(C::DENSE, S, IH, IW, OH, OW, R, FPB, C::XS);
+    const int OWd = M.OWd;
     const int XR = (R - 1) * S + KH;
     const int xpix = XR * IW + 8 * S + KW;
-    const int dypix = R * OWp + 8;
+    const int dypix = M.nk + 8;
     lds_char* ximg = (lds_char*)smem;
     lds_char* dyimg = ximg + xpix * C::XS;
     for (int i = tid * 16; i < xpix * C::XS + dypix * C::DYS; i += NTH * 16) *(lds_u32x4*)((lds_char*)smem + i) = u32x4_t{0u, 0u, 0u, 0u};
@@ -185,8 +221,8 @@
             const int pix = ci / CHY, c = ci % CHY;
             int r = pix / OW;
             const int ow = pix % OW;
-            if (stacked) r = (r / OH) * VP + r % OH;
-            pk[k] = ((unsigned)((xpix * C::XS + (r * OWp + ow) * C::DYS + c * 16) >> 4) << 17) | (unsigned)ci;
+            if (stacked && !C::DENSE) r = (r / OH) * VP + r % OH;
+            pk[k] = ((unsigned)((xpix * C::XS + (r * OWd + ow) * C::DYS + c * 16) >> 4) << 17) | (unsigned)ci;
         } else {
             const int cx = ci - ndy;
             const int pix = cx / CHX, c = cx % CHX;
@@ -254,30 +290,23 @@
         item = work_ctr ? s_next[iter & 1] : item + nwg;
         ++iter;
         if (item < nitems) prefetch(item);
-        const int units = R * U;
+        const int nk = M.nk;
         const int px = (g & 1) * 4 + prow;
-        const int q4 = 4 / U, r4 = 4 - q4 * U;
-        const int step4 = (q4 * S * IW + r4 * 8 * S) * C::XS, wrapd = (S * IW - U * 8 * S) * C::XS;
-        int uo[2], pbv[2];
-#pragma unroll
-        for (int hh = 0; hh < 2; ++hh) {
-            const int u = hh * 2 + (g >> 1), r = u / U;
-            uo[hh] = u - r * U;
-            pbv[hh] = ((r * S) * IW + (uo[hh] * 8 + px) * S) * C::XS + ccol;
-        }
-        const int abase = px * C::DYS + ccol + h * CTH * 32, pb_idle = (px * S) * C::XS + ccol;
+        WgradRunMap::Pos pos[2];
+#pragma unroll
+        for (int hh = 0; hh < 2; ++hh) { pos[hh] = M.at(8 * (hh * 2 + (g >> 1)) + px); pos[hh].x += ccol; }
+        const int abase = ccol + h * CTH * 32, pb_idle = (px * S) * C::XS + ccol;
 #pragma unroll 1
-        for (int u0 = 0; u0 < units; u0 += 4) {
+        for (int p0 = 0; p0 < nk; p0 += 32) {
             lds_char* ab[2];
             int pb[2];
 #pragma unroll
             for (int hh = 0; hh < 2; ++hh) {
-                const int u = u0 + hh * 2 + (g >> 1);
-                const bool valid = u < units;
-                ab[hh] = dyimg + (valid ? u * 8 : R * OWp) * C::DYS + abase;
-                pb[hh] = valid ? pbv[hh] : pb_idle;
-                pbv[hh] += step4; uo[hh] += r4;
-                if (uo[hh] >= U) { uo[hh] -= U; pbv[hh] += wrapd; }
+                const int p = p0 + 8 * (hh * 2 + (g >> 1)) + px;
+                const bool valid = p < nk;
+                ab[hh] = dyimg + (valid ? p : nk + px) * C::DYS + abase;
+                pb[hh] = valid ? pos[hh].x : pb_idle;
+                M.advance<C::DENSE>(pos[hh]);
             }
             auto bfrag = [&](int j) { return tr_read8(ximg + qoff + pb[0] + toff[j], ximg + qoff + pb[1] + toff[j]); };
             h16x8_t ring[D];
@@ -337,19 +366,21 @@
     const int Nf = J.Nf, IH = J.IH, IW = J.IW, OH = J.OH, OW = J.OW, R = J.R, nbands = J.nbands;
     int* __restrict__ const work_ctr = J.work_ctr;
     using C = WgradCfg<CI, CO, KH, KW, S>;
-    constexpr int NWV = 8, NTH = NWV * 64, CTH = C::CT / (NWV / 4), CHY = CO / 8, CHX = CI / 8, XSS = C::XS / 16, YSS = C::DYS / 16;
+    constexpr int NQ = C::NT % 8 == 0 ? 8 : 4, NTW = C::NT / NQ;
+    constexpr int NWV = 8, NTH = NWV * 64, CTH = C::CT / (NWV / NQ), CHY = CO / 8, CHX = CI / 8, XSS = C::XS / 16, YSS = C::DYS / 16;
     extern __shared__ __attribute__((aligned(16))) char smem[];
     const int tid = threadIdx.x, lane = tid & 63, wave = tid >> 6;
-    const int OWp = (OW + 7) & ~7, U = OWp >> 3;
+    const WgradRunMap M(C::DENSE, S, IH, IW, OH, OW, R, 1, C::XS);
+    const int OWd = M.OWd, nk = M.nk;
     const int XR = (R - 1) * S + KH;
     const int xpix = XR * IW + 8 * S + KW;
-    const int dypix = R * OWp + 8;
+    const int dypix = nk + 8;
     const int xslots = xpix * XSS, yslots = dypix * YSS;
     const int bbytes = ((xslots + yslots) * 16 + 1023) & ~1023;
     const int npieces = bbytes >> 10;
     lds_char* const lbase = (lds_char*)smem;
     const int nitems = Nf * nbands;
-    const float invXSS = 1.f / (float)XSS, invYSS = 1.f / (float)YSS, invIW = 1.f / (float)IW, invOWp = 1.f / (float)OWp, invOW = 1.f / (float)OW;
+    const float invXSS = 1.f / (float)XSS, invYSS = 1.f / (float)YSS, invIW = 1.f / (float)IW, invOWd = 1.f / (float)OWd, invOW = 1.f / (float)OW;
     constexpr int PFM = 10;
     unsigned pk[PFM];
 #pragma unroll
@@ -363,7 +394,7 @@
         } else {
             q -= xslots;
             const int px = wg_fdiv(q, invYSS), ch = q - px * YSS;
-            const int r = wg_fdiv(px, invOWp), c = px - r * OWp;
+            const int r = wg_fdiv(px, invOWd), c = px - r * OWd;
             if (ch < CHY && r < R && c < OW) v = 0x40000000u | ((unsigned)r << 24) | (unsigned)(((r * OW + c) * CO + ch * 8) >> 3);
         }
         pk[k] = v;
@@ -385,31 +416,29 @@
             wg_lds_dma16(src, dst + k * NWV * 1024);
         }
     };
-    const int q = wave & 3, h = wave >> 2;
-    f32x4 acc[C::NTW][CTH];
-#pragma unroll
-    for (int j = 0; j < C::NTW; ++j)
+    const int q = wave % NQ, h = wave / NQ;
+    f32x4 acc[NTW][CTH];
+#pragma unroll
+    for (int j = 0; j < NTW; ++j)
 #pragma unroll
         for (int c = 0; c < CTH; ++c) acc[j][c] = f32x4{0.f, 0.f, 0.f, 0.f};
     const int g = lane >> 4, a = lane & 15;
     const int prow = a >> 2;
     const int ccol = (a & 3) * 8;
-    constexpr int NTG = 4 / C::CGN, TPG = KH * KW / NTG;
-    static_assert(C::CGN <= 4 && 4 % C::CGN == 0 && (KH * KW) % NTG == 0 && TPG == C::NTW && (NTG == 1 || TPG % KW == 0), "n-tile assignment");
+    constexpr int NTG = NQ / C::CGN, TPG = KH * KW / NTG;
+    static_assert(C::CGN <= NQ && NQ % C::CGN == 0 && (KH * KW) % NTG == 0 && TPG == NTW && (NTG == 1 || TPG % KW == 0), "n-tile assignment");
     const int IWk = IWC ? IWC : IW;
     const int cgq = q % C::CGN, tg = q / C::CGN;
     const int qoff = ((tg * TPG / KW) * IWk) * C::XS + cgq * 32;
-    int toff[C::NTW];
-#pragma unroll
-    for (int j = 0; j < C::NTW; ++j) toff[j] = ((j / KW) * IWk + j % KW) * C::XS;
+    int toff[NTW];
+#pragma unroll
+    for (int j = 0; j < NTW; ++j) toff[j] = ((j / KW) * IWk + j % KW) * C::XS;
     float bsum[8] = {0.f, 0.f, 0.f, 0.f, 0.f, 0.f, 0.f, 0.f};
     __shared__ int s_next[2];
     int item = bid, iter = 0, nb = 0;
     if (item < nitems) dma(item, 0);
     asm volatile("s_waitcnt vmcnt(0)" ::: "memory");
     const int px = (g & 1) * 4 + prow;
-    const int q4 = 4 / U, r4 = 4 - q4 * U;
-    const int step4 = (q4 * S * IW + r4 * 8 * S) * C::XS, wrapd = (S * IW - U * 8 * S) * C::XS;
     while (item < nitems) {
         if (work_ctr && tid == 0) s_next[iter & 1] = nwg + atomicAdd(work_ctr, 1);
         __syncthreads();
@@ -422,36 +451,31 @@
         nb ^= 1;
         bool pend = item < nitems;
         if (pend && wave < 4) { dma(item, nb); pend = false; }
+        const int yrows_cur = min(R, OH - (cur % nbands) * R);
+        const int nkc = yrows_cur * OWd;
         {
-            const int f = cur / nbands, oh0 = (cur - f * nbands) * R;
-            const int nchunk = min(R, OH - oh0) * OW * CHY;
+            const int nchunk = yrows_cur * OW * CHY;
             for (int i = tid; i < nchunk; i += NTH) {
                 const int pix = i / CHY, r = wg_fdiv(pix, invOW), c = pix - r * OW;
-                const u32x4_t v = *(lds_u32x4*)(dyimg + (r * OWp + c) * C::DYS + (tid % CHY) * 16);
+                const u32x4_t v = *(lds_u32x4*)(dyimg + (r * OWd + c) * C::DYS + (tid % CHY) * 16);
 #pragma unroll
                 for (int e = 0; e < 4; ++e) { bsum[2 * e] += h2f_lo(v[e]); bsum[2 * e + 1] += h2f_hi(v[e]); }
             }
         }
-        const int units = R * U;
-        int uo[2], pbv[2];
-#pragma unroll
-        for (int hh = 0; hh < 2; ++hh) {
-            const int u = hh * 2 + (g >> 1), r = u / U;
-            uo[hh] = u - r * U;
-            pbv[hh] = ((r * S) * IW + (uo[hh] * 8 + px) * S) * C::XS + ccol;
-        }
-        const int abase = px * C::DYS + ccol + h * CTH * 32, pb_idle = (px * S) * C::XS + ccol;
-        auto mstep = [&](const int u0) {
+        WgradRunMap::Pos pos[2];
+#pragma unroll
+        for (int hh = 0; hh < 2; ++hh) { pos[hh] = M.at(8 * (hh * 2 + (g >> 1)) + px); pos[hh].x += ccol; }
+        const int abase = ccol + h * CTH * 32, pb_idle = (px * S) * C::XS + ccol;
+        auto mstep = [&](const int p0) {
             lds_char* ab[2];
             int pb[2];
 #pragma unroll
             for (int hh = 0; hh < 2; ++hh) {
-                const int u = u0 + hh * 2 + (g >> 1);
-                const bool valid = u < units;
-                ab[hh] = dyimg + (valid ? u * 8 : R * OWp) * C::DYS + abase;
-                pb[hh] = valid ? pbv[hh] : pb_idle;
-                pbv[hh] += step4; uo[hh] += r4;
-                if (uo[hh] >= U) { uo[hh] -= U; pbv[hh] += wrapd; }
+                const int p = p0 + 8 * (hh * 2 + (g >> 1)) + px;
+                const bool valid = p < nkc;
+                ab[hh] = dyimg + (valid ? p : nk + px) * C::DYS + abase;
+                pb[hh] = valid ? pos[hh].x : pb_idle;
+                M.advance<false>(pos[hh]);
             }
             auto bfrag = [&](int j) { return tr_read8(ximg + pb[0] + toff[j], ximg + pb[1] + toff[j]); };
             constexpr int D = 3;
@@ -460,28 +484,28 @@
 #pragma unroll
             for (int c = 0; c < CTH; ++c) af[c] = tr_read8(ab[0] + c * 32, ab[1] + c * 32);
 #pragma unroll
-            for (int j = 0; j < D && j < C::NTW; ++j) ring[j] = bfrag(j);
+            for (int j = 0; j < D && j < NTW; ++j) ring[j] = bfrag(j);
             __builtin_amdgcn_sched_barrier(0);
 #pragma unroll
-            for (int j = 0; j < C::NTW; ++j) {
+            for (int j = 0; j < NTW; ++j) {
                 const h16x8_t bf = ring[j % D];
 #pragma unroll
                 for (int c = 0; c < CTH; ++c) acc[j][c] = MFMA_16x16x32_H(af[c], bf, acc[j][c], 0, 0, 0);
-                if (j + D < C::NTW) ring[j % D] = bfrag(j + D);
+                if (j + D < NTW) ring[j % D] = bfrag(j + D);
                 __builtin_amdgcn_sched_barrier(0);
             }
         };
-        if (units > 0) mstep(0);
+        mstep(0);
         if (pend) { dma(item, nb); pend = false; }
 #pragma unroll 1
-        for (int u0 = 4; u0 < units; u0 += 4) mstep(u0);
+        for (int p0 = 32; p0 < nkc; p0 += 32) mstep(p0);
         if (pend) dma(item, nb);
         asm volatile("s_waitcnt vmcnt(0)" ::: "memory");
     }
     constexpr int KC = KH * KW * CI;
     float* out = part + (long long)bid * CO * KC;
 #pragma unroll
-    for (int j = 0; j < C::NTW; ++j)
+    for (int j = 0; j < NTW; ++j)
 #pragma unroll
         for (int c = 0; c < CTH; ++c)
 #pragma unroll
@@ -511,17 +535,23 @@
     else conv_wgrad_tr8_body<CI, CO, KH, KW, S, 8, 3, IWG>(B, (int)blockIdx.x - wgA, (int)gridDim.x - wgA);
 }
 template <int CI, int CO, int KH, int KW, int S>
+static inline int conv_wgrad_band_steps(int rows, int OW, int OH = 0, int fpb = 1) {
+    using C = WgradCfg<CI, CO, KH, KW, S>;
+    const int nk = (C::DENSE && fpb > 1) ? fpb * OH * OW : rows * C::owd(OW);
+    return (nk + 31) / 32;
+}
+template <int CI, int CO, int KH, int KW, int S>
 static inline int conv_wgrad_dma_rows(int IH, int IW, int OH, int OW, int* nbands_out, size_t* lds_out) {
     using C = WgradCfg<CI, CO, KH, KW, S>;
-    const int OWp = (OW + 7) / 8 * 8, U = OWp / 8;
+    auto steps = [&](int rows) { return conv_wgrad_band_steps<CI, CO, KH, KW, S>(rows, OW); };
     int bestR = 0, bestc = 1 << 30;
     for (int R = OH; R >= 1; --R) {
         const int XR = (R - 1) * S + KH;
-        const size_t band = (((size_t)(XR * IW + 8 * S + KW) * C::XS + (size_t)(R * OWp + 8) * C::DYS) + 1023) / 1024 * 1024;
+        const size_t band = (((size_t)(XR * IW + 8 * S + KW) * C::XS + (size_t)(R * C::owd(OW) + 8) * C::DYS) + 1023) / 1024 * 1024;
         const size_t lds = std::max<size_t>(2 * band, 512 * 8 * sizeof(float));
         if (lds > 160 * 1024 - 128 || band > 80 * 1024 || R > 63) continue;
         const int nb = (OH + R - 1) / R, last = OH - (nb - 1) * R;
-        const int cost = (nb - 1) * ((R * U + 3) / 4 + 1) + (last * U + 3) / 4 + 1;
+        const int cost = (nb - 1) * (steps(R) + 1) + steps(last) + 1;
         if (cost < bestc) { bestc = cost; bestR = R; *nbands_out = nb; *lds_out = lds; }
     }
     return bestR;
@@ -603,10 +633,10 @@
         }
     }
     int R = OH;
-    while (R > 1 && C::lds_bytes(R, IW, OW) > 78 * 1024) --R;
+    while (R > 1 && C::lds_bytes(R, IW, OW, true) > 78 * 1024) --R;
     const int nbands = (OH + R - 1) / R;
     R = (OH + nbands - 1) / nbands;
-    const size_t lds = C::lds_bytes(R, IW, OW);
+    const size_t lds = C::lds_bytes(R, IW, OW, true);
     static bool attr_set = false;
     if (!attr_set) {
         hipFuncSetAttribute((const void*)conv_wgrad_tr_kernel<CI, CO, KH, KW, S>, hipFuncAttributeMaxDynamicSharedMemorySize, 160 * 1024);
@@ -631,9 +661,9 @@
         A.nbands = nbA; A.FPB = 1;
         const int grid = std::min(256, max_blocks);
         if (grid < 2) return false;
-        auto steps = [](int rows, int OW) { return (rows * ((OW + 7) / 8) + 3) / 4 + 1; };
+        auto steps = [](int rows, int OW, int OH, int fpb) { return conv_wgrad_band_steps<CI, CO, KH, KW, S>(rows, OW, OH, fpb) + 1; };
         const int itemsA = A.Nf * nbA;
-        const double wA = (double)A.Nf * ((nbA - 1) * steps(A.R, A.OW) + steps(A.OH - (nbA - 1) * A.R, A.OW));
+        const double wA = (double)A.Nf * ((nbA - 1) * steps(A.R, A.OW, A.OH, 1) + steps(A.OH - (nbA - 1) * A.R, A.OW, A.OH, 1));
         size_t ldsB = 0; int itemsB = 0;
         auto planB = [&](int wgs) {
             if (!conv_wgrad_tr8_plan<CI, CO, KH, KW, S>(B.Nf, B.IH, B.IW, B.OH, B.OW, wgs, B.R, B.nbands, B.FPB, ldsB)) return false;
@@ -646,7 +676,7 @@
             if (!planB(grid)) return false;
             if (itemsA + itemsB <= grid) { nA = itemsA; nB = itemsB; }
             else {
-                camera_split(grid, wA, (double)itemsB * steps(B.R, B.OW), nA, nB);
+                camera_split(grid, wA, (double)itemsB * steps(B.R, B.OW, B.OH, B.FPB), nA, nB);
                 if (nA > itemsA) { nB = std::min(itemsB, nB + nA - itemsA); nA = itemsA; }
                 if (nB > itemsB) { nA = std::min(itemsA, nA + nB - itemsB); nB = itemsB; }
                 if (!planB(nB)) return false;
diff --git a/hulc_amd/csrc/k_entries.h b/hulc_amd/csrc/k_entries.h
--- a/hulc_amd/csrc/k_entries.h
+++ b/hulc_amd/csrc/k_entries.h
@@ -871,6 +871,26 @@
 int k_conv_plan(int form, int frames, int in_side, int out_side, int wgs, int* nbands, int* rows_per_band, int* frames_per_band, int* items) {
     static const char* who = "hulc_k_conv_plan";
     if (!nbands || !rows_per_band || !frames_per_band || !items || frames < 1 || in_side < 1 || out_side < 1 || in_side > 4096 || out_side > 4096) { hulc_set_error("%s: null argument or frames=%d, in_side=%d, out_side=%d out of range", who, frames, in_side, out_side); return 1; }
+    if (form >= 30 && form <= 33) {
+        const bool k3 = form == 30 || form == 32;
+        if (k_conv_fwd_side(in_side, k3 ? 3 : 4, k3 ? 1 : 2) != out_side) { hulc_set_error("%s: form %d: out_side %d does not belong to in_side %d", who, form, out_side, in_side); return 1; }
+        int R = 0, nb = 0, fpb = 1, st = 0; size_t lds = 0;
+        if (form <= 31) {
+            R = k3 ? conv_wgrad_dma_rows<64, 64, 3, 3, 1>(in_side, in_side, out_side, out_side, &nb, &lds) : conv_wgrad_dma_rows<32, 64, 4, 4, 2>(in_side, in_side, out_side, out_side, &nb, &lds);
+            if (R <= 0) { hulc_set_error("%s: form %d does not take in_side=%d", who, form, in_side); return 1; }
+            const int last = out_side - (nb - 1) * R;
+            st = k3 ? (nb - 1) * conv_wgrad_band_steps<64, 64, 3, 3, 1>(R, out_side) + conv_wgrad_band_steps<64, 64, 3, 3, 1>(last, out_side)
+                    : (nb - 1) * conv_wgrad_band_steps<32, 64, 4, 4, 2>(R, out_side) + conv_wgrad_band_steps<32, 64, 4, 4, 2>(last, out_side);
+        } else {
+            const int w = wgs > 0 ? wgs : 256;
+            const bool ok = k3 ? conv_wgrad_tr8_plan<64, 64, 3, 3, 1>(frames, in_side, in_side, out_side, out_side, w, R, nb, fpb, lds)
+                               : conv_wgrad_tr8_plan<32, 64, 4, 4, 2>(frames, in_side, in_side, out_side, out_side, w, R, nb, fpb, lds);
+            if (!ok) { hulc_set_error("%s: form %d does not take in_side=%d", who, form, in_side); return 1; }
+            st = k3 ? conv_wgrad_band_steps<64, 64, 3, 3, 1>(R, out_side, out_side, fpb) : conv_wgrad_band_steps<32, 64, 4, 4, 2>(R, out_side, out_side, fpb);
+        }
+        *nbands = nb; *rows_per_band = R; *frames_per_band = fpb; *items = st;
+        return 0;
+    }
     const int m10 = form % 10;
     const bool known = (form >= 10 && form <= 13) || (form >= 17 && form <= 23) || (form >= 27 && form <= 29);
     if (!known) { hulc_set_error("%s: form %d is not a weights-in-registers form", who, form); return 1; }
@@ -896,4 +916,44 @@
     return 0;
 }
 
-}
+int k_conv_slab_sum(const float* slabs, int nsplit, int O, int I, int KH, int KW, int nhwc, int yparts, float* grad, void* stream) {
+    static const char* who = "hulc_k_conv_slab_sum";
+    const long long slab = (long long)O * I * KH * KW;
+    if (!slabs || !grad || nsplit < 1 || nsplit > 4096 || O < 1 || I < 1 || KH < 1 || KW < 1 || slab > (1ll << 24) || (slab & 3) || yparts < 1 || yparts > 64) { hulc_set_error("%s: bad argument", who); return 1; }
+    UnpackBatch ub{};
+    UnpackJob& U = ub.j[0];
+    U.part = slabs; U.grad = grad; U.slab = slab; U.nsplit = nsplit; U.O = O; U.I = I; U.KH = KH; U.KW = KW; U.nhwc = nhwc ? 1 : 0; U.blk0 = 0; U.ysplit = 0;
+    ub.n = 1;
+    hipLaunchKernelGGL(unpack_conv_wgrad_batched_kernel, dim3((unsigned)((slab + 1023) / 1024), yparts), dim3(256), 0, (hipStream_t)stream, ub);
+    if (hipGetLastError() != hipSuccess) { hulc_set_error("%s: launch failed", who); return 1; }
+    return 0;
+}
+
+int k_conv_wgrad_run_map(int form, int in_side, int out_side, int rows, int real_rows, int fpb, int cap, int* dy_pixel, int* x_pixel, int* valid, int* steps) {
+    static const char* who = "hulc_k_conv_wgrad_run_map";
+    if (form < 30 || form > 33 || !dy_pixel || !x_pixel || !valid || !steps || in_side < 1 || out_side < 1 || rows < 1 || real_rows < 1 || real_rows > rows || (form >= 32 && real_rows != rows) || fpb < 1 || in_side > 4096) { hulc_set_error("%s: bad argument", who); return 1; }
+    const bool k3 = form == 30 || form == 32;
+    const int S = k3 ? 1 : 2;
+    if (k_conv_fwd_side(in_side, k3 ? 3 : 4, S) != out_side || (form <= 31 && fpb != 1)) { hulc_set_error("%s: form %d: out_side %d does not belong to in_side %d, or stacked frames on the LDS-DMA body", who, form, out_side, in_side); return 1; }
+    const WgradRunMap M(k3 ? WgradCfg<64, 64, 3, 3, 1>::DENSE : WgradCfg<32, 64, 4, 4, 2>::DENSE, S, in_side, in_side, out_side, out_side, rows, fpb, 1);
+    const int nkc = form <= 31 ? real_rows * M.OWd : M.nk;
+    *steps = (nkc + 31) / 32;
+    if (cap < 32 * *steps) { hulc_set_error("%s: %d slots, room for %d", who, 32 * *steps, cap); return 1; }
+    for (int hh = 0; hh < 2; ++hh)
+        for (int gh = 0; gh < 2; ++gh)
+            for (int px = 0; px < 8; ++px) {
+                const int lane0 = 8 * (hh * 2 + gh) + px;
+                WgradRunMap::Pos pos = M.at(lane0);
+                for (int p0 = 0, st = 0; p0 < nkc; p0 += 32, ++st) {
+                    const int p = p0 + lane0, slot = st * 32 + hh * 16 + gh * 8 + px;
+                    const bool ok = p < nkc;
+                    dy_pixel[slot] = ok ? p : M.nk + px;
+                    x_pixel[slot] = ok ? pos.x : px * S;
+                    valid[slot] = ok ? 1 : 0;
+                    if (form >= 32 && k3) M.advance<true>(pos); else M.advance<false>(pos);
+                }
+            }
+    return 0;
+}
+
+}
diff --git a/hulc_amd/lib.py b/hulc_amd/lib.py
--- a/hulc_amd/lib.py
+++ b/hulc_amd/lib.py
@@ -115,7 +115,7 @@
            "hulc_k_layernorm_fwd", "hulc_k_layernorm_bwd", "hulc_k_layernorm_mean", "hulc_k_tr_layer_fwd", "hulc_k_tr_ffn_bwd", "hulc_k_tr_attn_bwd",
            "hulc_k_window_compact", "hulc_k_rows_expand", "hulc_k_rows_reduce", "hulc_k_gemm_epi", "hulc_k_gemm_multi", "hulc_k_gemm_pick", "hulc_k_gemm_wgrad_nsplit",
            "hulc_k_det_head_loss", "hulc_k_det_head_bwd", "hulc_k_det_head_act",
-           "hulc_k_conv_wgrad_t", "hulc_k_conv1_wgrad_u8_t", "hulc_k_conv_tile_t", "hulc_k_conv_pair_t", "hulc_k_conv_plan",
+           "hulc_k_conv_wgrad_t", "hulc_k_conv1_wgrad_u8_t", "hulc_k_conv_tile_t", "hulc_k_conv_pair_t", "hulc_k_conv_plan", "hulc_k_conv_wgrad_run_map", "hulc_k_conv_slab_sum",
            "hulc_decoder_body_select"]
 
 _lib = None
@@ -278,6 +278,11 @@
         lib.hulc_k_conv_tile_t.argtypes = [I, I, P, P, P, P, P, P, I, I, I, I, I, P]
         lib.hulc_k_conv_pair_t.argtypes = [I, I, C.POINTER(HulcConvJob), C.POINTER(HulcConvJob), I, I, PI, P]
         lib.hulc_k_conv_plan.argtypes = [I, I, I, I, I, PI, PI, PI, PI]
+    if hasattr(lib, "hulc_k_conv_wgrad_run_map") or not os.environ.get("HULC_LIB_PATH"):
+        I, PI = C.c_int32, C.POINTER(C.c_int32)
+        lib.hulc_k_conv_wgrad_run_map.argtypes = [I, I, I, I, I, I, I, PI, PI, PI, PI]
+    if hasattr(lib, "hulc_k_conv_slab_sum") or not os.environ.get("HULC_LIB_PATH"):
+        lib.hulc_k_conv_slab_sum.argtypes = [C.c_void_p, C.c_int32, C.c_int32, C.c_int32, C.c_int32, C.c_int32, C.c_int32, C.c_int32, C.c_void_p, C.c_void_p]
     _lib = lib
     return lib
 
diff --git a/include/hulc_hip.h b/include/hulc_hip.h
--- a/include/hulc_hip.h
+++ b/include/hulc_hip.h
@@ -229,6 +229,9 @@
                        int32_t OUTH, int32_t relu, int32_t wgs, void* hip_stream);
 int hulc_k_conv_pair_t(int32_t dtype, int32_t stage, const hulc_conv_job* a, const hulc_conv_job* b, int32_t wg_a, int32_t wg_b, int32_t* slabs, void* hip_stream);
 int hulc_k_conv_plan(int32_t form, int32_t frames, int32_t in_side, int32_t out_side, int32_t wgs, int32_t* nbands, int32_t* rows_per_band, int32_t* frames_per_band, int32_t* items);
+int hulc_k_conv_slab_sum(const float* slabs, int32_t nsplit, int32_t O, int32_t I, int32_t KH, int32_t KW, int32_t nhwc, int32_t yparts, float* grad, void* hip_stream);
+int hulc_k_conv_wgrad_run_map(int32_t form, int32_t in_side, int32_t out_side, int32_t rows_per_band, int32_t real_rows, int32_t frames_per_band, int32_t capacity, int32_t* dy_pixel, int32_t* x_pixel,
+                              int32_t* valid, int32_t* steps);
 int hulc_k_skinny(const void* A, const void* W, void* out, int32_t M, int32_t N, int32_t K, int32_t variant, void* hip_stream);
 int hulc_k_rnn_persist(void* X, const void* W, const void* res, const void* mask, int32_t B, int32_t S, int32_t q0, int32_t dq, int32_t act,
                        uint32_t* flags, uint32_t* err, uint32_t launch_index, void* hip_stream);
```

Result: no change. 21880 windows/s, median of 6 (+0.4%).
